# SilverlightningY/dmmt-jpeg-encoder

Measured on AMD Instinct MI355X. Metric: Mpixel/s encoded (4K PPM, q=90), higher is better.
Workload: dtype f32; 1 GPU; 3840x2160 synthetic RGB u8, 4:4:4, IJG quality 90, 1 frame(s) per step per GPU, pixels in HBM -> JPEG files in HBM, inputs rotating over 12 distinct slots (285 MiB: streamed from HBM); width=3840, height=2160, subsampling=P444, quality=90, parallelism=independent frames x1, lanes=4, input_slots=12

## Files before the change

### dmmt-jpeg-encoder_amd/csrc/encoder.cpp

```cpp
#include <hip/hip_runtime.h>
#include <errno.h>
#include <stdio.h>
#include <sys/stat.h>
#include <stdlib.h>
#include <string.h>

#include <algorithm>
#include <mutex>
#include <vector>

#include "../../include/dmmt_jpeg.h"
#include "group.hpp"
#include "jpeg_common.hpp"
#include "kernels.hpp"

using namespace dmmt;

namespace {

const char* kStageNames[ST_COUNT] = {"front", "hist", "tables", "emit", "offsets", "stuffwrite"};

struct DevBuf {
    void* p = nullptr;
    size_t bytes = 0;
};

struct EventPair {
    int stage;
    hipEvent_t a, b;
};

#ifndef DMMT_FUSE_TABLES_DEFAULT
#define DMMT_FUSE_TABLES_DEFAULT 1
#endif

struct GraphEntry {
    std::vector<uint64_t> key;
    hipGraphExec_t exec = nullptr;
    uint64_t last_use = 0;
};
constexpr size_t kMaxGraphs = 16;

}

constexpr int kStatusAsync = 0, kStatusSync = 1, kStatusWords = 8;
struct Lane {
    hipStream_t stream = nullptr;
    int* status = nullptr;
    int* dstatus = nullptr;
    DevBuf coef, dcdiff, lastnz, ac_hist, dc_hist, code_tab, hdr_len, total_out, stage, chunk_bits, chunk_ff,
        chunk_ff8, chunk_edge, chunk_bit0, chunk_out, arrive;
    DevBuf ppm_rgb, ppm_counts, ppm_rowbase;
};

struct dmmt_ctx {
    dmmt::Group* group = nullptr;
    int device = 0;
    hipStream_t stream = nullptr;
    std::mutex mu;
    std::vector<Lane*> lanes;
    int nlanes = 1;
    unsigned next_lane = 0;
    DevBuf lut, qtab, qtab_u8;
    int async_bits = 0;
    hipEvent_t ev_lane0 = nullptr, ev_caller = nullptr;
    DevBuf in, out, out_len, dct;
    DevBuf ppm_text, ppm_maps, ppm_chunk_in, ppm_misc, ppm_counts;
    void* ppm_report = nullptr;
    void* ppm_batch_reports = nullptr;
    size_t ppm_batch_cap = 0;
    int ppm_batch_redone = -1;
    int lut_maxval = -1, lut_sb = -1;
    uint8_t q_cached[128];
    bool q_valid = false;
    bool profile = false;
    uint32_t profile_mask = 0;
    std::vector<EventPair> pending;
    std::vector<hipEvent_t> free_events;
    double stage_ms[ST_COUNT] = {0};
    int stage_launches[ST_COUNT] = {0};
    bool use_graphs = false;
    bool fuse_tables = DMMT_FUSE_TABLES_DEFAULT != 0;
    std::vector<GraphEntry> graphs;
    uint64_t graph_clock = 0;
    bool stripe_pending = false;
    Geom stripe_g{};
    dmmt_options stripe_opt{};
    int stripe_sb = 1;
    int16_t stripe_dc_first[3] = {0, 0, 0}, stripe_dc_last[3] = {0, 0, 0};
    bool stripe_measured = false;
    uint8_t* stripe_out = nullptr;
    size_t stripe_cap = 0;
};

namespace {

int hip_err(hipError_t e) {
    if (e == hipSuccess) return DMMT_OK;
    if (e == hipErrorOutOfMemory) return DMMT_E_OUT_OF_MEMORY;
    return DMMT_E_HIP;
}

#define HIP_TRY(expr)                      \
    do {                                   \
        hipError_t e_ = (expr);            \
        if (e_ != hipSuccess) return hip_err(e_); \
    } while (0)

int check_fresh_alloc(void* p) {
    int cur = -1;
    HIP_TRY(hipGetDevice(&cur));
    hipPointerAttribute_t a;
    HIP_TRY(hipPointerGetAttributes(&a, p));
    return a.device == cur ? DMMT_OK : DMMT_E_DEVICE_MISMATCH;
}

int ensure(DevBuf& b, size_t bytes, bool zero = false) {
    if (bytes == 0) bytes = 16;
    if (b.bytes >= bytes) return DMMT_OK;
    if (b.p) HIP_TRY(hipFree(b.p));
    b.p = nullptr;
    b.bytes = 0;
    HIP_TRY(hipMalloc(&b.p, bytes));
    if (int rc = check_fresh_alloc(b.p)) {
        (void)hipFree(b.p);
        b.p = nullptr;
        return rc;
    }
    b.bytes = bytes;
    if (zero) {
        HIP_TRY(hipMemset(b.p, 0, bytes));
        HIP_TRY(hipDeviceSynchronize());
    }
    return DMMT_OK;
}

void release(DevBuf& b) {
    if (b.p) (void)hipFree(b.p);
    b.p = nullptr;
    b.bytes = 0;
}

int validate(const dmmt_options* opt) {
    if (!opt) return DMMT_E_INVALID_ARGUMENT;
    if (opt->subsampling < 0 || opt->subsampling > 2) return DMMT_E_INVALID_ARGUMENT;
    if (opt->bits_per_channel < 0 || opt->bits_per_channel > 255) return DMMT_E_INVALID_ARGUMENT;
    for (int i = 0; i < 64; ++i)
        if (opt->luma_q[i] == 0 || opt->chroma_q[i] == 0) return DMMT_E_INVALID_ARGUMENT;
    if (opt->restart_interval < 0 || opt->restart_interval > 65535) return DMMT_E_INVALID_ARGUMENT;
    return DMMT_OK;
}

int make_checked_geom(int w, int h, int sub, int maxval, int ri, Geom* g) {
    if (w <= 0 || h <= 0) return DMMT_E_INVALID_ARGUMENT;
    *g = make_geom(w, h, sub, maxval, ri);
    if (g->wp > 65535 || g->hp > 65535) return DMMT_E_INVALID_ARGUMENT;
    return DMMT_OK;
}

int sync_lanes(dmmt_ctx* c) {
    for (Lane* L : c->lanes) HIP_TRY(hipStreamSynchronize(L->stream));
    return DMMT_OK;
}

int upload_tables(dmmt_ctx* c, const dmmt_options* opt, int maxval, int sb, hipStream_t st) {
    int rc;
    if ((rc = ensure(c->qtab, 128 * sizeof(float)))) return rc;
    if ((rc = ensure(c->qtab_u8, 256))) return rc;
    uint8_t q[256];
    memcpy(q, opt->luma_q, 64);
    memcpy(q + 64, opt->chroma_q, 64);
    for (int i = 0; i < 128; ++i) q[128 + i] = q[(i & 64) + kZigzag[i & 63]];
    if (!c->q_valid || memcmp(q, c->q_cached, 128) != 0) {
        if ((rc = sync_lanes(c))) return rc;
        float qf[128];
        for (int i = 0; i < 128; ++i) qf[i] = (float)q[i];
        HIP_TRY(hipMemcpyAsync(c->qtab.p, qf, sizeof qf, hipMemcpyHostToDevice, st));
        HIP_TRY(hipMemcpyAsync(c->qtab_u8.p, q, 256, hipMemcpyHostToDevice, st));
        HIP_TRY(hipStreamSynchronize(st));
        memcpy(c->q_cached, q, 128);
        c->q_valid = true;
    }
    if (sb == 4) {
        if (!c->lut.p && (rc = ensure(c->lut, 256 * sizeof(float)))) return rc;
        return DMMT_OK;
    }
    if (c->lut_maxval != maxval || c->lut_sb != sb) {
        if ((rc = sync_lanes(c))) return rc;
        const size_t n = sb == 1 ? 256 : 65536;
        if ((rc = ensure(c->lut, n * sizeof(float)))) return rc;
        std::vector<float> lut(n);
        for (size_t v = 0; v < n; ++v) lut[v] = (float)v / (float)maxval;
        HIP_TRY(hipMemcpyAsync(c->lut.p, lut.data(), n * sizeof(float), hipMemcpyHostToDevice, st));
        HIP_TRY(hipStreamSynchronize(st));
        c->lut_maxval = maxval;
        c->lut_sb = sb;
    }
    return DMMT_OK;
}

int ensure_work(dmmt_ctx* c, const Geom& g, int nf, Work* w, int lane, bool async) {
    int rc;
    Lane* L = c->lanes[lane];
    const size_t nb = (size_t)g.bpf * nf;
    const size_t nch = (size_t)g.nch * nf;
    if ((rc = ensure(L->coef, nb * 64 * sizeof(int16_t)))) return rc;
    if ((rc = ensure(L->dcdiff, nb * sizeof(int16_t)))) return rc;
    if ((rc = ensure(L->lastnz, nb))) return rc;
    if ((rc = ensure(L->stage, (nch * (size_t)kChunkWordsCap + 64) * sizeof(uint32_t)))) return rc;
    if ((rc = ensure(L->chunk_bits, nch * sizeof(uint32_t)))) return rc;
    if ((rc = ensure(L->chunk_ff, nch * 8 * sizeof(uint32_t)))) return rc;
    if ((rc = ensure(L->chunk_ff8, (nch + 2) * sizeof(unsigned long long)))) return rc;
    if ((rc = ensure(L->chunk_edge, nch * sizeof(uint32_t)))) return rc;
    if ((rc = ensure(L->chunk_bit0, nch * sizeof(unsigned long long)))) return rc;
    if ((rc = ensure(L->chunk_out, nch * sizeof(unsigned long long)))) return rc;
    if ((rc = ensure(L->ac_hist, (size_t)nf * kHistReps * 512 * 4, true))) return rc;
    if ((rc = ensure(L->dc_hist, (size_t)nf * kHistReps * 32 * 4, true))) return rc;
    if ((rc = ensure(L->code_tab, (size_t)nf * 1024 * 4))) return rc;
    if ((rc = ensure(L->arrive, (size_t)nf * kArriveFrameWords * 4, true))) return rc;
    if ((rc = ensure(L->hdr_len, (size_t)nf * 4))) return rc;
    if ((rc = ensure(L->total_out, (size_t)nf * 8))) return rc;
    if (!L->status) {
        void* h = nullptr;
        HIP_TRY(hipHostMalloc(&h, 2 * kStatusWords * sizeof(int), hipHostMallocMapped | hipHostMallocCoherent));
        memset(h, 0, 2 * kStatusWords * sizeof(int));
        L->status = (int*)h;
        if (hipHostGetDevicePointer((void**)&L->dstatus, h, 0) != hipSuccess) {
            (void)hipHostFree(h);
            L->status = nullptr;
            return DMMT_E_HIP;
        }
    }
    w->coef = (int16_t*)L->coef.p;
    w->dcdiff = (int16_t*)L->dcdiff.p;
    w->lastnz = (uint8_t*)L->lastnz.p;
    w->ac_hist = (uint32_t*)L->ac_hist.p;
    w->dc_hist = (uint32_t*)L->dc_hist.p;
    w->code_tab = (uint32_t*)L->code_tab.p;
    w->hdr_len = (uint32_t*)L->hdr_len.p;
    w->stage = (uint32_t*)L->stage.p;
    w->chunk_bits = (uint32_t*)L->chunk_bits.p;
    w->chunk_ff = (uint32_t*)L->chunk_ff.p;
    w->chunk_ff8 = (unsigned long long*)L->chunk_ff8.p;
    w->chunk_edge = (uint32_t*)L->chunk_edge.p;
    w->chunk_bit0 = (unsigned long long*)L->chunk_bit0.p;
    w->chunk_out = (unsigned long long*)L->chunk_out.p;
    w->total_out = (unsigned long long*)L->total_out.p;
    w->arrive = (uint32_t*)L->arrive.p;
    w->status = L->dstatus + (async ? kStatusAsync : kStatusSync) * kStatusWords;
    w->norm_lut = nullptr;
    w->qtab = nullptr;
    w->qtab_u8 = nullptr;
    return DMMT_OK;
}

int prepare(dmmt_ctx* c, const Geom& g, int nf, const dmmt_options* opt, int sb, hipStream_t st, Work* w,
            int lane = 0, bool async = false, int* status = nullptr) {
    int rc;
    if ((rc = ensure_work(c, g, nf, w, lane, async))) return rc;
    if (status) w->status = status;
    if ((rc = upload_tables(c, opt, g.maxval, sb, st))) return rc;
    w->norm_lut = (const float*)c->lut.p;
    w->qtab = (const float*)c->qtab.p;
    w->qtab_u8 = (const uint8_t*)c->qtab_u8.p;
    if (!w->norm_lut || !w->qtab || !w->qtab_u8) return DMMT_E_HIP;
    return DMMT_OK;
}

hipEvent_t take_event(dmmt_ctx* c) {
    if (!c->free_events.empty()) {
        hipEvent_t e = c->free_events.back();
        c->free_events.pop_back();
        return e;
    }
    hipEvent_t e = nullptr;
    if (hipEventCreate(&e) != hipSuccess) return nullptr;
    return e;
}

void drain_events(dmmt_ctx* c) {
    for (auto& p : c->pending) {
        (void)hipEventSynchronize(p.b);
        float ms = 0.f;
        if (hipEventElapsedTime(&ms, p.a, p.b) == hipSuccess) {
            c->stage_ms[p.stage] += ms;
            c->stage_launches[p.stage] += 1;
        }
        c->free_events.push_back(p.a);
        c->free_events.push_back(p.b);
    }
    c->pending.clear();
}

struct StageTimer {
    dmmt_ctx* c;
    int stage;
    hipStream_t st;
    hipEvent_t a = nullptr, b = nullptr;
    StageTimer(dmmt_ctx* c_, int s, hipStream_t st_) : c(c_), stage(s), st(st_) {
        if (c->profile && ((c->profile_mask >> s) & 1u)) {
            a = take_event(c);
            b = take_event(c);
            if (a) (void)hipEventRecord(a, st);
        }
    }
    ~StageTimer() {
        if (a && b) {
            (void)hipEventRecord(b, st);
            c->pending.push_back({stage, a, b});
            if (c->pending.size() > 4096) drain_events(c);
        }
    }
};

int enqueue_back_half(dmmt_ctx* c, const Geom& g, int nf, const Work& w, int bits, uint8_t* out, size_t out_stride,
                      uint32_t* out_len, hipStream_t st, int check_cat, bool hist_done = false) {
    const bool fused_tables = !hist_done && c->fuse_tables && tables_fusable(g);
    if (!hist_done) {
        StageTimer t(c, ST_HIST, st);
        HIP_TRY(launch_hist(nf, g, w, check_cat, st, fused_tables, bits, out, out_stride,
                            c->nlanes > 1 ? DMMT_HIST_WG_CAP_LANES : 0));
    }
    if (!fused_tables) {
        StageTimer t(c, ST_TABLES, st);
        HIP_TRY(launch_tables(nf, g, w, bits, out, out_stride, st));
    }
    {
        StageTimer t(c, ST_EMIT, st);
        HIP_TRY(launch_emit(nf, g, w, true, st, c->nlanes <= 1));
    }
    if (!offsets_fusable(g)) {
        StageTimer t(c, ST_OFFSETS, st);
        HIP_TRY(launch_offsets(nf, g, w, st));
    }
    {
        StageTimer t(c, ST_STUFFWRITE, st);
        HIP_TRY(launch_stuffwrite(nf, g, w, out, out_stride, out_len, st));
    }
    return DMMT_OK;
}

int enqueue_direct(dmmt_ctx* c, const void* d_rgb, size_t frame_stride, int sb, int nf, const Geom& g,
                   const Work& w, int bits, uint8_t* out, size_t out_stride, uint32_t* out_len, hipStream_t st,
                   const Surface* sf = nullptr, const YccFrames* yf = nullptr) {
    {
        StageTimer t(c, ST_FRONT, st);
        const int cap = c->nlanes > 1 ? DMMT_FRONT_PER_CU_LANES : 0;
        if (yf)
            HIP_TRY(launch_front_ycc(*yf, frame_stride, nf, g, w, st, cap));
        else if (sf)
            HIP_TRY(launch_front_surface(*sf, frame_stride, sb, nf, g, w, st, cap));
        else
            HIP_TRY(launch_front(d_rgb, frame_stride, sb, nf, g, w, st, cap));
    }
    return enqueue_back_half(c, g, nf, w, bits, out, out_stride, out_len, st, sb == 4);
}

void destroy_graphs(dmmt_ctx* c) {
    for (auto& e : c->graphs) (void)hipGraphExecDestroy(e.exec);
    c->graphs.clear();
}

int enqueue_encode(dmmt_ctx* c, const void* d_rgb, size_t frame_stride, int sb, int nf, const Geom& g,
                   const dmmt_options* opt, uint8_t* out, size_t out_stride, uint32_t* out_len, hipStream_t st,
                   int lane = 0, bool async = false, int* status = nullptr, const Surface* sf = nullptr,
                   const YccFrames* yf = nullptr) {
    Work w;
    int rc;
    if ((rc = prepare(c, g, nf, opt, sb, st, &w, lane, async, status))) return rc;
    const int bits = opt->bits_per_channel;
    if (!c->use_graphs || c->profile || status)
        return enqueue_direct(c, d_rgb, frame_stride, sb, nf, g, w, bits, out, out_stride, out_len, st, sf, yf);
    std::vector<uint64_t> key = {(uint64_t)(uintptr_t)d_rgb, (uint64_t)frame_stride, (uint64_t)sb, (uint64_t)nf,
                                 (uint64_t)g.width, (uint64_t)g.height, (uint64_t)g.hr, (uint64_t)g.vr,
                                 (uint64_t)g.maxval, (uint64_t)g.restart_interval, (uint64_t)bits,
                                 (uint64_t)(uintptr_t)out, (uint64_t)out_stride, (uint64_t)(uintptr_t)out_len,
                                 (uint64_t)(uintptr_t)st,
                                 sf ? (uint64_t)sf->format + 1 : 0, sf ? (uint64_t)sf->row_pitch : 0,
                                 sf ? (uint64_t)(uintptr_t)sf->plane[0] : 0, sf ? (uint64_t)(uintptr_t)sf->plane[1] : 0,
                                 sf ? (uint64_t)(uintptr_t)sf->plane[2] : 0};
    if (yf)
        key.insert(key.end(), {(uint64_t)yf->format + 16, (uint64_t)yf->luma_pitch, (uint64_t)yf->chroma_pitch,
                               (uint64_t)(uintptr_t)yf->plane[1], (uint64_t)(uintptr_t)yf->plane[2]});
    const void* const* wp = reinterpret_cast<const void* const*>(&w);
    static_assert(sizeof(Work) % sizeof(void*) == 0, "Work holds pointers only");
    for (size_t i = 0; i < sizeof(Work) / sizeof(void*); ++i) key.push_back((uint64_t)(uintptr_t)wp[i]);
    GraphEntry* hit = nullptr;
    for (auto& e : c->graphs)
        if (e.key == key) hit = &e;
    if (!hit) {
        hipGraph_t graph = nullptr;
        HIP_TRY(hipStreamBeginCapture(st, hipStreamCaptureModeThreadLocal));
        rc = enqueue_direct(c, d_rgb, frame_stride, sb, nf, g, w, bits, out, out_stride, out_len, st, sf, yf);
        hipError_t e = hipStreamEndCapture(st, &graph);
        if (rc) {
            if (graph) (void)hipGraphDestroy(graph);
            return rc;
        }
        HIP_TRY(e);
        hipGraphExec_t exec = nullptr;
        e = hipGraphInstantiate(&exec, graph, nullptr, nullptr, 0);
        (void)hipGraphDestroy(graph);
        HIP_TRY(e);
        if (c->graphs.size() >= kMaxGraphs) {
            size_t lru = 0;
            for (size_t i = 1; i < c->graphs.size(); ++i)
                if (c->graphs[i].last_use < c->graphs[lru].last_use) lru = i;
            (void)hipGraphExecDestroy(c->graphs[lru].exec);
            c->graphs.erase(c->graphs.begin() + lru);
        }
        c->graphs.push_back({std::move(key), exec, 0});
        hit = &c->graphs.back();
    }
    hit->last_use = ++c->graph_clock;
    HIP_TRY(hipGraphLaunch(hit->exec, st));
    return DMMT_OK;
}

int status_code(int s) {
    if (s & 1) return DMMT_E_VALUE_EXCEEDS_MAX;
    if (s & 4) return DMMT_E_CATEGORY_RANGE;
    if (s & 2) return DMMT_E_HUFFMAN_SYMBOL_MISSING;
    if (s & 16) return DMMT_E_CAPACITY;
    return DMMT_OK;
}

int read_status(Lane* L, int group, hipStream_t st, int* bits) {
    *bits = 0;
    if (!L->status) return DMMT_OK;
    if (st) HIP_TRY(hipStreamSynchronize(st));
    volatile int* p = L->status + group * kStatusWords;
    for (int k = 0; k < kStatusWords; ++k)
        if (p[k]) {
            *bits |= 1 << k;
            p[k] = 0;
        }
    return DMMT_OK;
}

int take_status(dmmt_ctx* c, hipStream_t st) {
    int s = 0, rc;
    if ((rc = read_status(c->lanes[0], kStatusSync, st, &s))) return rc;
    return status_code(s);
}

int collect_async(dmmt_ctx* c, Lane* L, bool device_synced = false) {
    int s = 0, rc;
    if ((rc = read_status(L, kStatusAsync, device_synced ? nullptr : L->stream, &s))) return rc;
    c->async_bits |= s;
    return DMMT_OK;
}

int set_device(dmmt_ctx* c) { return hip_err(hipSetDevice(c->device)); }

dmmt_ctx* primary(dmmt_ctx* c) { return c && c->group ? group_member(c->group, 0) : c; }

void destroy_lane(Lane* L, bool own_stream) {
    (void)hipStreamSynchronize(L->stream);
    if (L->status) (void)hipHostFree(L->status);
    DevBuf* bufs[] = {&L->coef,      &L->dcdiff,     &L->lastnz,     &L->ac_hist,
                      &L->dc_hist,  &L->code_tab,  &L->hdr_len,    &L->total_out,  &L->stage,
                      &L->chunk_bits, &L->chunk_ff, &L->chunk_ff8, &L->chunk_edge, &L->chunk_bit0, &L->chunk_out,
                      &L->arrive,     &L->ppm_rgb,    &L->ppm_counts, &L->ppm_rowbase};
    for (DevBuf* b : bufs) release(*b);
    if (own_stream) (void)hipStreamDestroy(L->stream);
    delete L;
}

}


extern "C" int dmmt_device_count(int* count) {
    if (!count) return DMMT_E_INVALID_ARGUMENT;
    int n = 0;
    if (hipGetDeviceCount(&n) != hipSuccess) n = 0;
    *count = n;
    return DMMT_OK;
}

extern "C" int dmmt_ctx_create(int device, dmmt_ctx** out) {
    if (!out) return DMMT_E_INVALID_ARGUMENT;
    *out = nullptr;
    int n = 0;
    if (hipGetDeviceCount(&n) != hipSuccess || n <= 0 || device < 0 || device >= n) return DMMT_E_NO_DEVICE;
    hipDeviceProp_t prop;
    if (hipGetDeviceProperties(&prop, device) != hipSuccess) return DMMT_E_NO_DEVICE;
    if (strncmp(prop.gcnArchName, "gfx950", 6) != 0) return DMMT_E_NO_DEVICE;
    if (hipSetDevice(device) != hipSuccess) return DMMT_E_NO_DEVICE;
    dmmt_ctx* c = new dmmt_ctx();
    c->device = device;
    if (const char* e = getenv("DMMT_GRAPHS")) c->use_graphs = atoi(e) != 0;
    if (const char* e = getenv("DMMT_FUSE_TABLES")) c->fuse_tables = atoi(e) != 0;
    if (hipStreamCreateWithFlags(&c->stream, hipStreamNonBlocking) != hipSuccess) {
        delete c;
        return DMMT_E_HIP;
    }
    c->lanes.push_back(new Lane());
    c->lanes[0]->stream = c->stream;
    if (hipEventCreateWithFlags(&c->ev_lane0, hipEventDisableTiming) != hipSuccess ||
        hipEventCreateWithFlags(&c->ev_caller, hipEventDisableTiming) != hipSuccess) {
        dmmt_ctx_destroy(c);
        return DMMT_E_HIP;
    }
    *out = c;
    return DMMT_OK;
}

static int check_ptr_device(const void* p, int dev) {
    if (!p) return DMMT_OK;
    hipPointerAttribute_t a;
    HIP_TRY(hipPointerGetAttributes(&a, p));
    return a.device == dev ? DMMT_OK : DMMT_E_DEVICE_MISMATCH;
}

namespace dmmt {
int ctx_check_device(dmmt_ctx* c) {
    int rc;
    if ((rc = set_device(c))) return rc;
    std::lock_guard<std::mutex> lk(c->mu);
    for (Lane* L : c->lanes) {
        const DevBuf* bufs[] = {&L->coef,       &L->dcdiff,   &L->lastnz,     &L->ac_hist,    &L->dc_hist,
                                &L->code_tab,   &L->hdr_len,  &L->total_out,  &L->stage,      &L->chunk_bits,
                                &L->chunk_ff,   &L->chunk_ff8,  &L->chunk_edge, &L->chunk_bit0, &L->chunk_out, &L->arrive,
                                &L->ppm_rgb,    &L->ppm_counts, &L->ppm_rowbase};
        for (const DevBuf* b : bufs)
            if ((rc = check_ptr_device(b->p, c->device))) return rc;
    }
    const DevBuf* bufs[] = {&c->lut, &c->qtab, &c->qtab_u8, &c->in, &c->out, &c->out_len, &c->dct, &c->ppm_text,
                            &c->ppm_maps, &c->ppm_chunk_in, &c->ppm_misc, &c->ppm_counts};
    for (const DevBuf* b : bufs)
        if ((rc = check_ptr_device(b->p, c->device))) return rc;
    return DMMT_OK;
}
int ptr_check_device(const void* p, int device) { return check_ptr_device(p, device); }
}

extern "C" int dmmt_ctx_check_device(dmmt_ctx* c, int32_t* device) {
    if (!c) return DMMT_E_INVALID_ARGUMENT;
    if (device) *device = c->device;
    if (c->group) return dmmt::group_check_devices(c->group);
    return dmmt::ctx_check_device(c);
}

extern "C" int dmmt_ctx_create_multi(const int* device_ids, int n, dmmt_ctx** out) {
    if (!out) return DMMT_E_INVALID_ARGUMENT;
    *out = nullptr;
    if (!device_ids || n < 1 || n > DMMT_MAX_GROUP) return DMMT_E_INVALID_ARGUMENT;
    dmmt::Group* g = nullptr;
    const int rc = dmmt::group_create(device_ids, n, &g);
    if (rc) return rc;
    dmmt_ctx* c = new dmmt_ctx();
    c->group = g;
    c->device = device_ids[0];
    *out = c;
    return DMMT_OK;
}

extern "C" int dmmt_ctx_num_devices(const dmmt_ctx* c) {
    if (!c) return 0;
    return c->group ? dmmt::group_size(c->group) : 1;
}

extern "C" dmmt_ctx* dmmt_ctx_member(dmmt_ctx* c, int i) {
    if (!c) return nullptr;
    if (c->group) return dmmt::group_member(c->group, i);
    return i == 0 ? c : nullptr;
}

extern "C" void dmmt_ctx_destroy(dmmt_ctx* c) {
    if (!c) return;
    if (c->group) {
        dmmt::group_destroy(c->group);
        delete c;
        return;
    }
    (void)hipSetDevice(c->device);
    (void)sync_lanes(c);
    drain_events(c);
    destroy_graphs(c);
    for (hipEvent_t e : c->free_events) (void)hipEventDestroy(e);
    for (size_t i = 0; i < c->lanes.size(); ++i) destroy_lane(c->lanes[i], i > 0);
    if (c->ev_lane0) (void)hipEventDestroy(c->ev_lane0);
    if (c->ev_caller) (void)hipEventDestroy(c->ev_caller);
    DevBuf* bufs[] = {&c->lut,      &c->qtab,         &c->qtab_u8,  &c->in,       &c->out,     &c->out_len,
                      &c->dct,      &c->ppm_text,     &c->ppm_maps, &c->ppm_chunk_in, &c->ppm_misc,
                      &c->ppm_counts};
    for (DevBuf* b : bufs) release(*b);
    if (c->ppm_report) (void)hipHostFree(c->ppm_report);
    if (c->ppm_batch_reports) (void)hipHostFree(c->ppm_batch_reports);
    (void)hipStreamDestroy(c->stream);
    delete c;
}

extern "C" int dmmt_ctx_set_lanes(dmmt_ctx* c, int n) {
    if (!c || n < 1 || n > DMMT_MAX_LANES) return DMMT_E_INVALID_ARGUMENT;
    if (c->group) return dmmt::group_set_lanes(c->group, n);
    std::lock_guard<std::mutex> lk(c->mu);
    int rc;
    if ((rc = set_device(c))) return rc;
    if ((rc = sync_lanes(c))) return rc;
    while ((int)c->lanes.size() > n) {
        if ((rc = collect_async(c, c->lanes.back()))) return rc;
        destroy_lane(c->lanes.back(), true);
        c->lanes.pop_back();
    }
    while ((int)c->lanes.size() < n) {
        Lane* L = new Lane();
        if (hipStreamCreateWithFlags(&L->stream, hipStreamNonBlocking) != hipSuccess) {
            delete L;
            return DMMT_E_HIP;
        }
        c->lanes.push_back(L);
    }
    destroy_graphs(c);
    c->nlanes = n;
    c->next_lane = 0;
    return DMMT_OK;
}

extern "C" int dmmt_ctx_synchronize(dmmt_ctx* c) {
    if (!c) return DMMT_E_INVALID_ARGUMENT;
    if (c->group) return dmmt::group_synchronize(c->group);
    std::lock_guard<std::mutex> lk(c->mu);
    int rc;
    if ((rc = set_device(c))) return rc;
    HIP_TRY(hipDeviceSynchronize());
    for (Lane* L : c->lanes)
        if ((rc = collect_async(c, L, true))) return rc;
    const int s = c->async_bits;
    c->async_bits = 0;
    return status_code(s);
}

extern "C" size_t dmmt_max_jpeg_bytes(uint16_t width, uint16_t height, int32_t subsampling) {
    if (subsampling < 0 || subsampling > 2 || width == 0 || height == 0) return 0;
    Geom g = make_geom(width, height, subsampling, 255, 0);
    return max_jpeg_bytes(g);
}

static int encode_device_frames(dmmt_ctx* c, const dmmt_device_frames* f, const dmmt_options* opt, void* stream,
                                const Geom& g, const Surface* sf, const YccFrames* yf = nullptr) {
    int rc;
    std::lock_guard<std::mutex> lk(c->mu);
    if ((rc = set_device(c))) return rc;
    if (stream) {
        hipStream_t st = (hipStream_t)stream;
        HIP_TRY(hipEventRecord(c->ev_lane0, c->stream));
        HIP_TRY(hipStreamWaitEvent(st, c->ev_lane0, 0));
        rc = enqueue_encode(c, f->d_rgb, f->frame_stride, f->sample_bytes, f->n_frames, g, opt, f->d_out,
                            f->out_stride, f->d_out_len, st, 0, true, nullptr, sf, yf);
        HIP_TRY(hipEventRecord(c->ev_caller, st));
        HIP_TRY(hipStreamWaitEvent(c->stream, c->ev_caller, 0));
        return rc;
    }
    int lane = 0;
    if (c->nlanes > 1) lane = (int)(c->next_lane++ % (unsigned)c->nlanes);
    return enqueue_encode(c, f->d_rgb, f->frame_stride, f->sample_bytes, f->n_frames, g, opt, f->d_out, f->out_stride,
                          f->d_out_len, c->lanes[lane]->stream, lane, true, nullptr, sf, yf);
}

extern "C" int dmmt_encode_device(dmmt_ctx* c, const dmmt_device_frames* f, const dmmt_options* opt, void* stream) {
    c = primary(c);
    if (!c || !f) return DMMT_E_INVALID_ARGUMENT;
    int rc;
    if ((rc = validate(opt))) return rc;
    if (f->n_frames <= 0 || !f->d_rgb || !f->d_out || !f->d_out_len) return DMMT_E_INVALID_ARGUMENT;
    if (f->sample_bytes != 1 && f->sample_bytes != 2 && f->sample_bytes != 4) return DMMT_E_INVALID_ARGUMENT;
    Geom g;
    if ((rc = make_checked_geom(f->width, f->height, opt->subsampling, f->maxval, opt->restart_interval, &g))) return rc;
    if (f->out_stride < max_jpeg_bytes(g)) return DMMT_E_CAPACITY;
    return encode_device_frames(c, f, opt, stream, g, nullptr);
}

extern "C" size_t dmmt_surface_span(const dmmt_device_surfaces* s) {
// ... 603 lines not shown
    case DMMT_E_INPUT_NOT_FOUND: return "Input file not found";
    case DMMT_E_NO_READ_PERMISSION: return "No read permission for input file";
    case DMMT_E_OPEN_INPUT: return "Unable to open input file for reading";
    case DMMT_E_OPEN_OUTPUT: return "Unable to open output file for writing";
    case DMMT_E_WRITE_IMAGE_DATA: return "Failed to write image data";
    case DMMT_E_WRITE_END_OF_FILE: return "Failed to write end of file";
    case DMMT_E_HUFFMAN_SYMBOL_MISSING: return "Huffman symbol not present in translator";
    case DMMT_E_VALUE_EXCEEDS_MAX: return "Color value must not be greater than max value";
    case DMMT_E_CATEGORY_RANGE: return "Value out of range for categorisation";
    case DMMT_E_INVALID_ARGUMENT: return "Invalid argument";
    case DMMT_E_HIP: return "HIP runtime error";
    case DMMT_E_OUT_OF_MEMORY: return "Out of device memory";
    case DMMT_E_NO_DEVICE: return "No gfx950 (MI355X) device available; this library has no CPU fallback";
    case DMMT_E_CAPACITY: return "Output buffer too small";
    case DMMT_E_DEVICE_MISMATCH: return "A context's device buffer is not on its GPU";
    default: return dmmt_error_name(code);
    }
}

extern "C" int dmmt_ctx_set_profiling(dmmt_ctx* c, int enable) {
    if (!c) return DMMT_E_INVALID_ARGUMENT;
    if (c->group) return dmmt::group_set_profiling(c->group, enable);
    std::lock_guard<std::mutex> lk(c->mu);
    drain_events(c);
    c->profile = enable != 0;
    c->profile_mask = enable == 1 ? 0xFFFFFFFFu : (uint32_t)enable;
    for (int i = 0; i < ST_COUNT; ++i) {
        c->stage_ms[i] = 0;
        c->stage_launches[i] = 0;
    }
    return DMMT_OK;
}

extern "C" int dmmt_ctx_profile(dmmt_ctx* c, double* ms, int32_t* launches, int n_stages) {
    if (!c) return DMMT_E_INVALID_ARGUMENT;
    if (c->group) return dmmt::group_profile(c->group, ms, launches, n_stages);
    std::lock_guard<std::mutex> lk(c->mu);
    (void)hipSetDevice(c->device);
    drain_events(c);
    for (int i = 0; i < n_stages && i < ST_COUNT; ++i) {
        if (ms) ms[i] = c->stage_ms[i];
        if (launches) launches[i] = c->stage_launches[i];
    }
    return DMMT_OK;
}

extern "C" int dmmt_num_stages(void) { return ST_COUNT; }
extern "C" const char* dmmt_stage_name(int s) { return s >= 0 && s < ST_COUNT ? kStageNames[s] : ""; }

extern "C" int dmmt_device_malloc(dmmt_ctx* c, size_t bytes, void** ptr) {
    c = primary(c);
    if (!c || !ptr) return DMMT_E_INVALID_ARGUMENT;
    int rc;
    if ((rc = set_device(c))) return rc;
    HIP_TRY(hipMalloc(ptr, bytes ? bytes : 16));
    if ((rc = check_fresh_alloc(*ptr))) {
        (void)hipFree(*ptr);
        *ptr = nullptr;
        return rc;
    }
    return DMMT_OK;
}

extern "C" int dmmt_device_free(dmmt_ctx* c, void* ptr) {
    c = primary(c);
    if (!c) return DMMT_E_INVALID_ARGUMENT;
    int rc;
    if ((rc = set_device(c))) return rc;
    HIP_TRY(hipFree(ptr));
    return DMMT_OK;
}

extern "C" int dmmt_memcpy_h2d(dmmt_ctx* c, void* dst, const void* src, size_t bytes) {
    c = primary(c);
    if (!c) return DMMT_E_INVALID_ARGUMENT;
    int rc;
    if ((rc = set_device(c))) return rc;
    HIP_TRY(hipMemcpy(dst, src, bytes, hipMemcpyHostToDevice));
    return DMMT_OK;
}

extern "C" int dmmt_memcpy_d2h(dmmt_ctx* c, void* dst, const void* src, size_t bytes) {
    c = primary(c);
    if (!c) return DMMT_E_INVALID_ARGUMENT;
    int rc;
    if ((rc = set_device(c))) return rc;
    HIP_TRY(hipMemcpy(dst, src, bytes, hipMemcpyDeviceToHost));
    return DMMT_OK;
}

extern "C" int dmmt_fill_synthetic(dmmt_ctx* c, void* d_rgb, uint16_t width, uint16_t height, int32_t n_frames,
                                   int32_t first_frame, uint32_t seed) {
    c = primary(c);
    if (!c || !d_rgb || n_frames <= 0) return DMMT_E_INVALID_ARGUMENT;
    int rc;
    if ((rc = set_device(c))) return rc;
    HIP_TRY(launch_synthetic((uint8_t*)d_rgb, width, height, n_frames, first_frame, seed, 0, height, c->stream));
    HIP_TRY(hipStreamSynchronize(c->stream));
    return DMMT_OK;
}

extern "C" int dmmt_fill_synthetic_rows(dmmt_ctx* c, void* d_rgb, uint16_t width, uint16_t height, int32_t row0,
                                        int32_t rows, int32_t frame, uint32_t seed) {
    c = primary(c);
    if (!c || !d_rgb || row0 < 0 || rows <= 0 || row0 + rows > height) return DMMT_E_INVALID_ARGUMENT;
    int rc;
    if ((rc = set_device(c))) return rc;
    HIP_TRY(launch_synthetic((uint8_t*)d_rgb, width, height, 1, frame, seed, row0, rows, c->stream));
    HIP_TRY(hipStreamSynchronize(c->stream));
    return DMMT_OK;
}

static int stripe_geom(const dmmt_stripe* st, const dmmt_options* opt, Geom* g) {
    if (!st || !opt || !st->d_rgb) return DMMT_E_INVALID_ARGUMENT;
    if (st->sample_bytes != 1 && st->sample_bytes != 2 && st->sample_bytes != 4) return DMMT_E_INVALID_ARGUMENT;
    const int ri = opt->restart_interval;
    if (ri < 0) return DMMT_E_INVALID_ARGUMENT;
    Geom full;
    int rc;
    if ((rc = make_checked_geom(st->width, st->height, opt->subsampling, st->maxval, ri, &full))) return rc;
    if (st->mcu_row0 < 0 || st->mcu_rows <= 0 || st->mcu_row0 + st->mcu_rows > full.mcuy) return DMMT_E_INVALID_ARGUMENT;
    const long long m0 = (long long)st->mcu_row0 * full.mcux;
    const bool last = st->mcu_row0 + st->mcu_rows == full.mcuy;
    if (ri > 0 && m0 % ri) return DMMT_E_INVALID_ARGUMENT;
    if (ri > 0 && !last && ((long long)st->mcu_rows * full.mcux) % ri) return DMMT_E_INVALID_ARGUMENT;
    const int rows_px = 8 * full.vr;
    const int y0 = st->mcu_row0 * rows_px;
    const int h = std::min(st->mcu_rows * rows_px, (int)st->height - y0);
    *g = make_geom(st->width, h, opt->subsampling, st->maxval, ri);
    g->sof_height = st->height;
    g->seg_base = ri > 0 ? (int)(m0 / ri) : 0;
    g->stripe_first = st->mcu_row0 == 0;
    g->more_after = !last;
    return DMMT_OK;
}

extern "C" size_t dmmt_stripe_max_bytes(const dmmt_stripe* st, const dmmt_options* opt) {
    Geom g;
    if (validate(opt) || stripe_geom(st, opt, &g)) return 0;
    return max_jpeg_bytes(g);
}

extern "C" int dmmt_stripe_analyze(dmmt_ctx* c, const dmmt_stripe* st, const dmmt_options* opt,
                                   uint64_t hist[DMMT_STRIPE_HIST_WORDS]) {
    c = primary(c);
    if (!c || !hist) return DMMT_E_INVALID_ARGUMENT;
    int rc;
    Geom g;
    if ((rc = validate(opt)) || (rc = stripe_geom(st, opt, &g))) return rc;
    std::lock_guard<std::mutex> lk(c->mu);
    if ((rc = set_device(c))) return rc;
    hipStream_t s = c->stream;
    Work w;
    if ((rc = prepare(c, g, 1, opt, st->sample_bytes, s, &w))) return rc;
    {
        StageTimer t(c, ST_FRONT, s);
        HIP_TRY(launch_front(st->d_rgb, (size_t)st->width * g.height * 3 * st->sample_bytes, st->sample_bytes, 1, g, w,
                             s));
    }
    {
        StageTimer t(c, ST_HIST, s);
        HIP_TRY(launch_hist(1, g, w, st->sample_bytes == 4, s));
    }
    std::vector<uint32_t> ac((size_t)kHistReps * 512), dc((size_t)kHistReps * 32);
    HIP_TRY(hipMemcpyAsync(ac.data(), w.ac_hist, ac.size() * 4, hipMemcpyDeviceToHost, s));
    HIP_TRY(hipMemcpyAsync(dc.data(), w.dc_hist, dc.size() * 4, hipMemcpyDeviceToHost, s));
    HIP_TRY(hipMemsetAsync(w.ac_hist, 0, ac.size() * 4, s));
    HIP_TRY(hipMemsetAsync(w.dc_hist, 0, dc.size() * 4, s));
    HIP_TRY(hipStreamSynchronize(s));
    if ((rc = take_status(c, s))) return rc;
    for (int i = 0; i < DMMT_STRIPE_HIST_WORDS; ++i) hist[i] = 0;
    for (int r = 0; r < kHistReps; ++r) {
        for (int k = 0; k < 16; ++k) {
            hist[k] += dc[(size_t)r * 32 + k];
            hist[272 + k] += dc[(size_t)r * 32 + 16 + k];
        }
        for (int k = 0; k < 256; ++k) {
            hist[16 + k] += ac[(size_t)r * 512 + k];
            hist[288 + k] += ac[(size_t)r * 512 + 256 + k];
        }
    }
    if (g.restart_interval == 0) {
        std::vector<int16_t> head((size_t)g.bpm * 64), tail((size_t)g.bpm * 64);
        const int nl = g.n_luma;
        HIP_TRY(hipMemcpyAsync(head.data(), w.coef, head.size() * 2, hipMemcpyDeviceToHost, s));
        HIP_TRY(hipMemcpyAsync(tail.data(), w.coef + (g.bpf - g.bpm) * 64, tail.size() * 2, hipMemcpyDeviceToHost, s));
        HIP_TRY(hipStreamSynchronize(s));
        c->stripe_dc_first[0] = head[0];
        c->stripe_dc_first[1] = head[(size_t)nl * 64];
        c->stripe_dc_first[2] = head[(size_t)(nl + 1) * 64];
        c->stripe_dc_last[0] = tail[(size_t)(nl - 1) * 64];
        c->stripe_dc_last[1] = tail[(size_t)nl * 64];
        c->stripe_dc_last[2] = tail[(size_t)(nl + 1) * 64];
    }
    c->stripe_g = g;
    c->stripe_opt = *opt;
    c->stripe_sb = st->sample_bytes;
    c->stripe_pending = true;
    c->stripe_measured = false;
    return DMMT_OK;
}

static int upload_hist_sum(const Work& w, const uint64_t* hist_sum, hipStream_t s) {
    std::vector<uint32_t> ac(512), dc(32);
    for (int k = 0; k < 16; ++k) {
        if (hist_sum[k] > 0xFFFFFFFFull || hist_sum[272 + k] > 0xFFFFFFFFull) return DMMT_E_INVALID_ARGUMENT;
        dc[k] = (uint32_t)hist_sum[k];
        dc[16 + k] = (uint32_t)hist_sum[272 + k];
    }
    for (int k = 0; k < 256; ++k) {
        if (hist_sum[16 + k] > 0xFFFFFFFFull || hist_sum[288 + k] > 0xFFFFFFFFull) return DMMT_E_INVALID_ARGUMENT;
        ac[k] = (uint32_t)hist_sum[16 + k];
        ac[256 + k] = (uint32_t)hist_sum[288 + k];
    }
    HIP_TRY(hipMemcpyAsync(w.ac_hist, ac.data(), ac.size() * 4, hipMemcpyHostToDevice, s));
    HIP_TRY(hipMemcpyAsync(w.dc_hist, dc.data(), dc.size() * 4, hipMemcpyHostToDevice, s));
    HIP_TRY(hipStreamSynchronize(s));
    return DMMT_OK;
}

static int dc_category(int v) {
    unsigned a = (unsigned)(v < 0 ? -v : v);
    int n = 0;
    while (a) {
        ++n;
        a >>= 1;
    }
    return n;
}

extern "C" int dmmt_stripe_dc_edges(dmmt_ctx* c, int16_t first_dc[3], int16_t last_dc[3]) {
    c = primary(c);
    if (!c || !first_dc || !last_dc) return DMMT_E_INVALID_ARGUMENT;
    std::lock_guard<std::mutex> lk(c->mu);
    if (!c->stripe_pending || c->stripe_g.restart_interval != 0) return DMMT_E_INVALID_ARGUMENT;
    for (int i = 0; i < 3; ++i) {
        first_dc[i] = c->stripe_dc_first[i];
        last_dc[i] = c->stripe_dc_last[i];
    }
    return DMMT_OK;
}

extern "C" void dmmt_stripe_fix_dc_hist(uint64_t hist[DMMT_STRIPE_HIST_WORDS], const int16_t first_dc[3],
                                        const int16_t prev_last_dc[3]) {
    for (int i = 0; i < 3; ++i) {
        uint64_t* h = hist + (i == 0 ? 0 : 272);
        const int was = dc_category(first_dc[i]);
        const int is = dc_category((int16_t)(first_dc[i] - prev_last_dc[i]));
        if (h[was] > 0) {
            h[was] -= 1;
            h[is] += 1;
        }
    }
}

extern "C" int dmmt_stripe_measure(dmmt_ctx* c, const uint64_t hist_sum[DMMT_STRIPE_HIST_WORDS],
                                   const int16_t prev_last_dc[3], uint8_t* d_out, size_t out_cap, uint64_t* bits,
                                   uint32_t* first16) {
    c = primary(c);
    if (!c || !hist_sum || !prev_last_dc || !d_out || !bits || !first16) return DMMT_E_INVALID_ARGUMENT;
    std::lock_guard<std::mutex> lk(c->mu);
    if (!c->stripe_pending || c->stripe_g.restart_interval != 0) return DMMT_E_INVALID_ARGUMENT;
    int rc;
    if ((rc = set_device(c))) return rc;
    const Geom g = c->stripe_g;
    if (out_cap < max_jpeg_bytes(g)) return DMMT_E_CAPACITY;
    hipStream_t s = c->stream;
    Work w;
    if ((rc = prepare(c, g, 1, &c->stripe_opt, c->stripe_sb, s, &w))) return rc;
    if ((rc = upload_hist_sum(w, hist_sum, s))) return rc;
    int16_t d[3];
    const long long at[3] = {0, g.n_luma, g.n_luma + 1};
    for (int i = 0; i < 3; ++i) {
        d[i] = (int16_t)(c->stripe_dc_first[i] - prev_last_dc[i]);
        HIP_TRY(hipMemcpyAsync(w.dcdiff + at[i], &d[i], sizeof(int16_t), hipMemcpyHostToDevice, s));
    }
    {
        StageTimer t(c, ST_TABLES, s);
        HIP_TRY(launch_tables(1, g, w, c->stripe_opt.bits_per_channel, d_out, out_cap, s));
    }
    {
        StageTimer t(c, ST_EMIT, s);
        HIP_TRY(launch_emit(1, g, w, false, s, c->nlanes <= 1));
    }
    std::vector<uint32_t> nb((size_t)g.nch), edge((size_t)g.nch);
    HIP_TRY(hipMemcpyAsync(nb.data(), w.chunk_bits, nb.size() * 4, hipMemcpyDeviceToHost, s));
    HIP_TRY(hipMemcpyAsync(edge.data(), w.chunk_edge, edge.size() * 4, hipMemcpyDeviceToHost, s));
    HIP_TRY(hipStreamSynchronize(s));
    if ((rc = take_status(c, s))) return rc;
    uint64_t total = 0;
    uint32_t f = 0;
    int have = 0;
    for (int k = 0; k < g.nch; ++k) {
        if (have < 16 && nb[k]) {
            const int t = std::min(16 - have, (int)std::min<uint32_t>(nb[k], 16u));
            f |= ((edge[k] >> 16) >> (16 - t)) << (16 - have - t);
            have += t;
        }
        total += nb[k];
    }
    *bits = total;
    *first16 = f;
    c->stripe_out = d_out;
    c->stripe_cap = out_cap;
    c->stripe_measured = true;
    return DMMT_OK;
}

extern "C" int dmmt_stripe_write(dmmt_ctx* c, uint64_t bit_offset, uint32_t next_bits, uint32_t next16,
                                 uint64_t* out_len) {
    c = primary(c);
    if (!c || !out_len || next_bits > 16) return DMMT_E_INVALID_ARGUMENT;
    std::lock_guard<std::mutex> lk(c->mu);
    if (!c->stripe_pending || !c->stripe_measured) return DMMT_E_INVALID_ARGUMENT;
    int rc;
    if ((rc = set_device(c))) return rc;
    Geom g = c->stripe_g;
    if (g.stripe_first && bit_offset) return DMMT_E_INVALID_ARGUMENT;
    g.bit_phase = (int)(bit_offset & 7);
    g.next_bits = g.more_after ? (int)next_bits : 0;
    g.next16 = g.more_after ? (next16 & 0xFFFFu) & ~(0xFFFFu >> next_bits) : 0u;
    hipStream_t s = c->stream;
    Work w;
    if ((rc = prepare(c, g, 1, &c->stripe_opt, c->stripe_sb, s, &w))) return rc;
    if ((rc = ensure(c->out_len, 4))) return rc;
    {
        StageTimer t(c, ST_OFFSETS, s);
        HIP_TRY(launch_offsets(1, g, w, s));
    }
    {
        StageTimer t(c, ST_STUFFWRITE, s);
        HIP_TRY(launch_stuffwrite(1, g, w, c->stripe_out, c->stripe_cap, (uint32_t*)c->out_len.p, s));
    }
    uint32_t len = 0;
    HIP_TRY(hipMemcpyAsync(&len, c->out_len.p, 4, hipMemcpyDeviceToHost, s));
    HIP_TRY(hipStreamSynchronize(s));
    c->stripe_pending = false;
    c->stripe_measured = false;
    if ((rc = take_status(c, s))) return rc;
    *out_len = len;
    return DMMT_OK;
}

extern "C" int dmmt_stripe_encode(dmmt_ctx* c, const uint64_t hist_sum[DMMT_STRIPE_HIST_WORDS], uint8_t* d_out,
                                  size_t out_cap, uint64_t* out_len) {
    c = primary(c);
    if (!c || !hist_sum || !d_out || !out_len) return DMMT_E_INVALID_ARGUMENT;
    std::lock_guard<std::mutex> lk(c->mu);
    if (!c->stripe_pending) return DMMT_E_INVALID_ARGUMENT;
    if (c->stripe_g.restart_interval == 0) return DMMT_E_INVALID_ARGUMENT;
    int rc;
    if ((rc = set_device(c))) return rc;
    const Geom g = c->stripe_g;
    if (out_cap < max_jpeg_bytes(g)) return DMMT_E_CAPACITY;
    hipStream_t s = c->stream;
    Work w;
    if ((rc = prepare(c, g, 1, &c->stripe_opt, c->stripe_sb, s, &w))) return rc;
    if ((rc = upload_hist_sum(w, hist_sum, s))) return rc;
    if ((rc = ensure(c->out_len, 4))) return rc;
    if ((rc = enqueue_back_half(c, g, 1, w, c->stripe_opt.bits_per_channel, d_out, out_cap, (uint32_t*)c->out_len.p,
                                s, 0, true)))
        return rc;
    uint32_t len = 0;
    HIP_TRY(hipMemcpyAsync(&len, c->out_len.p, 4, hipMemcpyDeviceToHost, s));
    HIP_TRY(hipStreamSynchronize(s));
    c->stripe_pending = false;
    if ((rc = take_status(c, s))) return rc;
    *out_len = len;
    return DMMT_OK;
}

extern "C" const char* dmmt_build_info(void) {
#if DMMT_SDWA_PEEPHOLE
#define DMMT_SDWA_NOTE "SDWA peephole on (measurement build)"
#else
#define DMMT_SDWA_NOTE "-mllvm -amdgpu-sdwa-peephole=false"
#endif
    return "dmmt-jpeg-encoder_amd: HIP kernels for gfx950, -ffp-contract=off, " DMMT_SDWA_NOTE ", ABI " "1";
}
```

### dmmt-jpeg-encoder_amd/csrc/entropy.hip

```cpp
#include <hip/hip_runtime.h>
#include <stdint.h>

#include "device_common.hpp"
#include "jpeg_common.hpp"
#include "kernels.hpp"
#include "slot_copy.hpp"

namespace dmmt {

#ifdef DMMT_PHASE_TRACE
static __device__ unsigned long long g_trace[64];
#endif

static_assert(kChunkBlocks == 256 || kChunkBlocks == 512, "one thread per block, one workgroup per chunk");
constexpr int kEmitThreads = kChunkBlocks;
constexpr int kEmitWaves = kEmitThreads / 64;
#ifndef DMMT_EMIT_OCC
#define DMMT_EMIT_OCC 8
#endif
constexpr int kEmitOcc = kChunkBlocks == 256 ? DMMT_EMIT_OCC : 3;
#ifndef DMMT_EMIT_OCC_BATCH
#define DMMT_EMIT_OCC_BATCH 7
#endif
constexpr int kEmitOccBatch = kChunkBlocks == 256 ? DMMT_EMIT_OCC_BATCH : 3;

constexpr int kEmitWords = 4 * kChunkBlocks;
constexpr int kStuffPass = 4096;
#ifndef DMMT_EMIT_BRANCHFREE
#define DMMT_EMIT_BRANCHFREE 1
#endif
#ifndef DMMT_TAIL_DMA
#define DMMT_TAIL_DMA 1
#endif
#ifndef DMMT_TAIL_NSEG1
#define DMMT_TAIL_NSEG1 1
#endif
#ifndef DMMT_WALK_COLUMN_MAJOR
#define DMMT_WALK_COLUMN_MAJOR 1
#endif
#ifndef DMMT_EMIT_PRIO_ALWAYS
#define DMMT_EMIT_PRIO_ALWAYS 0
#endif
#ifndef DMMT_EMIT_PRIO
#define DMMT_EMIT_PRIO 1
#endif

struct ChunkSpan {
    long long el0;
    int nb;
    int seg;
    bool seg_first, seg_last;
};

__device__ __forceinline__ ChunkSpan chunk_span(const Geom& g, int c) {
    ChunkSpan r;
    r.seg = min(c / g.cps, g.nseg - 1);
    const int j = c - r.seg * g.cps;
    const long long sb = (long long)r.seg * g.seg_blocks;
    const long long se = min(sb + g.seg_blocks, g.bpf);
    r.el0 = sb + (long long)j * kChunkBlocks;
    r.nb = (int)min((long long)kChunkBlocks, se - r.el0);
    r.seg_first = j == 0;
    r.seg_last = r.el0 + r.nb == se;
    return r;
}

__device__ __forceinline__ bool joined_tail(const Geom& g, int c) {
    return c == g.nch - 1 && g.more_after && g.restart_interval == 0;
}

__device__ __forceinline__ int mod_small(int x, int d, uint32_t inv16) {
    return x - (int)__umul24((uint32_t)d, __umul24((uint32_t)x, inv16) >> 16);
}

struct BlockCoef {
    uint32_t w[32];
};

__device__ __forceinline__ void load_block(const int16_t* __restrict__ p, BlockCoef& b) {
    const uint4* q = reinterpret_cast<const uint4*>(p);
#pragma unroll
    for (int i = 0; i < 8; ++i) {
        const uint4 v = q[i];
        b.w[4 * i] = v.x;
        b.w[4 * i + 1] = v.y;
        b.w[4 * i + 2] = v.z;
        b.w[4 * i + 3] = v.w;
    }
}

__device__ __forceinline__ int coef_at(const BlockCoef& b, int k) {
    return (k & 1) ? ((int)b.w[k >> 1] >> 16) : (int)(int16_t)(b.w[k >> 1] & 0xFFFFu);
}

__device__ __forceinline__ void zigzag_in_registers(BlockCoef& b) {
#if DMMT_WALK_COLUMN_MAJOR
    return;
#endif
    uint32_t z[32];
#pragma unroll
    for (int j = 0; j < 32; ++j) {
        const int i0 = coef_pos(2 * j), i1 = coef_pos(2 * j + 1);
        const uint32_t lo = (b.w[i0 >> 1] >> (16 * (i0 & 1))) & 0xFFFFu;
        const uint32_t hi = (b.w[i1 >> 1] >> (16 * (i1 & 1))) & 0xFFFFu;
        z[j] = lo | (hi << 16);
    }
#pragma unroll
    for (int j = 0; j < 32; ++j) b.w[j] = z[j];
}

template <typename Sink>
__device__ __forceinline__ void walk_block(const BlockCoef& b, int dcd, const uint2* __restrict__ dctab,
                                           const uint2* __restrict__ actab, Sink& sink, int kmax = 63) {
    {
        const int cat = category_of(dcd);
        const uint2 e = dctab[cat];
        sink(e.x | extra_bits(dcd, cat), (int)e.y);
    }
    uint32_t m_run = 0xF0u, m_low = 0xFFFFu, m_zrl = 255u;
    asm volatile("" : "+s"(m_run), "+s"(m_low), "+s"(m_zrl));
    int l16 = 16;
#pragma unroll
    for (int k0 = 0; k0 < 64; k0 += 4) {
        if (k0 != 0 && k0 > kmax) break;
#pragma unroll
        for (int k = k0 ? k0 : 1; k < k0 + 4; ++k) {
            const int kc =DMMT_WALK_COLUMN_MAJOR ? coef_pos(k) : k;
            const uint32_t w = b.w[kc >> 1];
            if ((kc & 1) ? w > m_low : (w << 16) != 0u) {
                const int v = coef_at(b, kc);
                const int r16 = 16 * k - l16;
                if (k >= 17 && __builtin_amdgcn_ballot_w64((uint32_t)r16 > m_zrl) != 0) {
                    int r = r16 >> 8;
                    asm volatile("" : "+v"(r));
                    const uint2 z = actab[0xF0];
#pragma unroll 1
                    for (; r > 0; --r) sink(z.x, (int)z.y);
                }
                const int cat = category_fast(v);
                const uint2 e = actab[(r16 & (int)m_run) | cat];
                sink(e.x | extra_bits(v, cat), (int)e.y);
                l16 = 16 * k + 16;
            }
        }
    }
    if (l16 < 16 * 64 || kmax < 63) {
        const uint2 e = actab[0];
        sink(e.x, (int)e.y);
    }
}

struct CountSink {
    uint32_t n = 0;
    __device__ __forceinline__ void operator()(uint32_t, int len) { n += (uint32_t)len; }
};

struct WindowSink {
    uint32_t* img;
    int lo, n;
    unsigned long long acc;
    int nacc;
    int w;
    bool first;
    __device__ __forceinline__ void put(uint32_t word, bool shared) {
        const int i = w - lo;
        if ((unsigned)i < (unsigned)n) {
            if (shared)
                atomicOr(&img[i], word);
            else
                img[i] = word;
        }
    }
    __device__ __forceinline__ void operator()(uint32_t val, int len) {
        acc = (acc << len) | val;
        nacc += len;
        if (nacc >= 32) {
            nacc -= 32;
            put((uint32_t)(acc >> nacc), first);
            first = false;
            ++w;
        }
    }
    __device__ __forceinline__ void finish() {
        if (nacc > 0) put((uint32_t)(acc << (32 - nacc)), true);
    }
};


struct SlotSink {
    uint32_t* slot;
    unsigned long long acc;
    int nacc;
    int wi;
#if DMMT_EMIT_BRANCHFREE
    __device__ __forceinline__ void operator()(uint32_t val, int len) {
        acc = (acc << len) | val;
        nacc += len;
        const int full = nacc >> 5;
        nacc &= 31;
        slot[min(wi, kSlotWords - 1) * kEmitThreads] = (uint32_t)(acc >> nacc);
        wi += full;
    }
#else
    __device__ __forceinline__ void operator()(uint32_t val, int len) {
        acc = (acc << len) | val;
        nacc += len;
        if (nacc >= 32) {
            nacc -= 32;
            slot[min(wi, kSlotWords - 1) * kEmitThreads] = (uint32_t)(acc >> nacc);
            ++wi;
        }
    }
#endif
    __device__ __forceinline__ uint32_t finish() {
        if (nacc > 0 && wi < kSlotWords) slot[wi * kEmitThreads] = (uint32_t)(acc << (32 - nacc));
        return (uint32_t)wi * 32u + (uint32_t)nacc;
    }
};


__device__ __forceinline__ uint32_t bits16_at(uint32_t a, uint32_t b, int p) {
    const unsigned long long x = ((unsigned long long)a << 32) | b;
    return (uint32_t)(x >> (48 - (p & 31))) & 0xFFFFu;
}

struct NoMark {
    template <typename I>
    __device__ void operator()(I) const {}
};
template <typename Mark = NoMark>
__device__ __forceinline__ void fused_offsets(const uint32_t* __restrict__ cbits, const uint32_t* __restrict__ cff,
                              const unsigned long long* __restrict__ cff8, uint8_t* sFF8,
                              const uint32_t* __restrict__ cedge, const Geom& g, unsigned long long* __restrict__ bit0,
                              unsigned long long* __restrict__ outo, unsigned long long* __restrict__ total,
                              unsigned long long* sWaveV, int* sWaveF, int tid, Mark mark = Mark());
static_assert(kArriveWords == kArriveFrameWords, "the host sizes the counters");

__device__ __forceinline__ int tid_again(int wave) {
    uint32_t zero = 0u;
    asm volatile("" : "+s"(zero));
    return (wave << 6) | (int)__builtin_amdgcn_mbcnt_hi(~0u, __builtin_amdgcn_mbcnt_lo(~0u, zero));
}

template <int OCC>
__global__ __launch_bounds__(kEmitThreads, OCC) void k_emit(const int16_t* coef, const int16_t* __restrict__ dcdiff,
                                              const uint8_t* __restrict__ lastnz,
                                              const uint32_t* __restrict__ code_tab, Geom g,
                                              uint32_t* __restrict__ stage, uint32_t* __restrict__ chunk_bits,
                                              uint32_t* __restrict__ chunk_ff, uint32_t* __restrict__ chunk_edge,
                                              uint32_t* __restrict__ ac_hist, uint32_t* __restrict__ dc_hist,
                                              int fuse, uint32_t* __restrict__ arrive,
                                              unsigned long long* __restrict__ chunk_bit0,
                                              unsigned long long* __restrict__ chunk_out,
                                              unsigned long long* __restrict__ total_out,
                                              unsigned long long* __restrict__ chunk_ff8, int prio) {
    __shared__ uint2 sTab[2 * 256 + 2 * 16];
    __shared__ __attribute__((aligned(16))) uint32_t sSlot[kSlotWords * kEmitThreads];
    static_assert(kEmitWords + 2 <= kSlotWords * kEmitThreads, "the window image lies inside the slot area");
    uint32_t* const sW = sSlot;
    __shared__ uint32_t sSort[kEmitThreads + kEmitThreads * (int)sizeof(std::conditional_t<(kEmitThreads > 256), uint16_t, uint8_t>) / 4 + kEmitThreads / 4];
    __shared__ uint32_t sWave[kEmitWaves];
    __shared__ uint32_t sFF[8];
    __shared__ uint32_t sEdge[3];
    __shared__ uint32_t sBin[65];
    __shared__ unsigned long long sOffV[kEmitWaves + 1];
    __shared__ int sOffF[kEmitWaves];
    __shared__ uint32_t sLast;
    using OrderT = std::conditional_t<(kEmitThreads > 256), uint16_t, uint8_t>;
    uint32_t* const sBits = sSort;
    OrderT* const sOrder = reinterpret_cast<OrderT*>(sSort + kEmitThreads);
    uint8_t* const sKey = reinterpret_cast<uint8_t*>(sSort + kEmitThreads + kEmitThreads * (int)sizeof(OrderT) / 4);
    DMMT_TRACE_START;
    int tid = threadIdx.x;
    const int wave = __builtin_amdgcn_readfirstlane(tid >> 6);
    const int frame = blockIdx.y;
    const unsigned chunk = blockIdx.x;
    const ChunkSpan span = chunk_span(g, (int)chunk);
    const long long el0 = span.el0;
    const int nb = span.nb;
    const size_t cid = (size_t)frame * g.nch + chunk;
    const int r0 = (int)((uint32_t)el0 % (uint32_t)g.bpm);
    const uint32_t inv16 = (65536u + (uint32_t)g.bpm - 1u) / (uint32_t)g.bpm;
    bool valid = tid < nb;
    const uint32_t* ct = code_tab + (size_t)frame * 1024;
    const int tt = tid & 255;
    const uint32_t tac0 = ct[256 + tt], tac1 = ct[768 + tt];
    const uint32_t tdc = ct[((tt & 31) < 16 ? 0 : 512 - 16) + (tt & 31)];
    const uint32_t lz = lastnz[(long long)frame * g.bpf + el0 + (valid ? tid : 0)];
    if (tid < 256) {
        const int c = tid & 15;
        sTab[tid] = make_uint2((tac0 & 0xFFFFu) << c, (tac0 >> 16) + c);
        sTab[256 + tid] = make_uint2((tac1 & 0xFFFFu) << c, (tac1 >> 16) + c);
    }
    if (tid < 32) sTab[512 + tid] = make_uint2((tdc & 0xFFFFu) << (tid & 15), (tdc >> 16) + (tid & 15));
    if (chunk == 0) {
        for (int i = tid; i < kHistReps * 512; i += kEmitThreads) ac_hist[(size_t)frame * kHistReps * 512 + i] = 0u;
        for (int i = tid; i < kHistReps * 32; i += kEmitThreads) dc_hist[(size_t)frame * kHistReps * 32 + i] = 0u;
    }
    if (tid < 8) sFF[tid] = 0u;
    if (tid < 3) sEdge[tid] = 0u;
    if (tid < 65) sBin[tid] = 0u;
    const int key = valid ? (int)lz : 64;
    __syncthreads();
    const uint32_t rank = atomicAdd(&sBin[key], 1u);
    __syncthreads();
    if (tid < 64) {
        const uint32_t c = sBin[tid];
        const uint32_t inc = wave_incl_scan_full_u32(c);
        sBin[tid] = inc - c;
    }
    __syncthreads();
    if (valid) {
        const int mine = (int)(sBin[key] + rank);
        sOrder[mine] = (OrderT)tid;
        sKey[mine] = (uint8_t)key;
    }
    __syncthreads();
    DMMT_TRACE(0);
    uint32_t wbits = 0;
    bool slot_over = false;
    {
#if DMMT_EMIT_PRIO
        if (prio) {
            if (wave == 3) __builtin_amdgcn_s_setprio(3);
            else if (wave == 2) __builtin_amdgcn_s_setprio(2);
            else if (wave == 1) __builtin_amdgcn_s_setprio(1);
        }
#endif
        if (valid) {
            const int p = sOrder[tid];
            const long long ep = (long long)frame * g.bpf + el0 + p;
            BlockCoef b;
            load_block(coef + ep * 64, b);
            zigzag_in_registers(b);
            const int dp = dcdiff[ep];
            DMMT_TRACE(4);
            const int kp = mod_small(r0 + p, g.bpm, inv16);
            const bool lum = kp < g.n_luma;
            const int kmax = __builtin_amdgcn_readfirstlane((int)sKey[min(64 * wave + 63, nb - 1)]);
            SlotSink ss{sSlot + tid, 0ull, 0, 0};
            walk_block(b, dp, sTab + 512 + (lum ? 0 : 16), sTab + (lum ? 0 : 256), ss, kmax);
            wbits = ss.finish();
            slot_over = wbits > (uint32_t)kSlotWords * 32u;
            sBits[p] = wbits | ((uint32_t)tid << 16);
            DMMT_TRACE(5);
        }
    }
#if DMMT_EMIT_PRIO
    if (prio) __builtin_amdgcn_s_setprio(0);
#endif
    const bool over = __syncthreads_or(slot_over) != 0;
    tid = tid_again(wave);
    const int lane = tid & 63;
    valid = tid < nb;
    static_assert(kMaxBlockBits < (1 << 16), "a block's bit count and its walker's column share a word");
    const uint32_t bw = valid ? sBits[tid] : (uint32_t)tid << 16;
    const uint32_t bits = bw & 0xFFFFu;
    const int mine = (int)(bw >> 16);
    const uint32_t incl = wave_incl_scan_full_u32(bits);
    if (lane == 63) sWave[wave] = incl;
    __syncthreads();
    uint32_t start = incl - bits;
    uint32_t total = 0;
#pragma unroll
    for (int q = 0; q < kEmitWaves; ++q) {
        start += q < wave ? sWave[q] : 0u;
        total += sWave[q];
    }
    DMMT_TRACE(1);

    uint32_t* slot = stage + cid * (size_t)kChunkWordsCap;
    const int nw = (int)((total + 31) >> 5);
    const int we1 = total >= 16 ? (int)((total - 16) >> 5) : 0;
    uint32_t ff[4] = {0, 0, 0, 0};
    auto window_out = [&](int tid, int w0, int wn) {
        for (int i = tid; i < wn; i += kEmitThreads) {
            const uint32_t a = sW[i], c = sW[i + 1];
            slot[w0 + i] = a;
            const int wi = w0 + i;
            if (wi == 0) sEdge[0] = a;
            if (wi == we1) {
                sEdge[1] = a;
                sEdge[2] = c;
            }
            const unsigned long long x = ((unsigned long long)a << 32) | c;
            unsigned long long z = x & (x << 1);
            z &= z << 2;
            z &= z << 4;
            const uint32_t m = (uint32_t)(z >> 32);
            if (m) {
#pragma unroll
                for (int r = 0; r < 4; ++r)
                    ff[r] += __popc(m & (0x80808080u >> (2 * r))) | (__popc(m & (0x80808080u >> (2 * r + 1))) << 16);
            }
        }
    };
    if (!over) {
        SlotWords sw;
        read_slot<kEmitThreads>(sSlot, mine, bits, sw);
        __syncthreads();
        for (int w0 = 0; w0 < nw; w0 += kEmitWords) {
            const int wn = min(kEmitWords, nw - w0);
            uint32_t st = start;
            asm volatile("" : "+v"(st));
            if (tid == 0 && w0 + wn >= nw) sW[wn] = 0u;
            copy_owned(sw, st, bits, sW, w0, wn);
            __syncthreads();
            copy_head(sw, st, bits, sW, w0, wn);
            __syncthreads();
            window_out(tid, w0, wn);
            __syncthreads();
        }
    } else {
        for (int w0 = 0; w0 < nw; w0 += kEmitWords) {
            const int wn = min(kEmitWords, nw - w0);
            uint32_t st = start;
            asm volatile("" : "+v"(st));
            for (int i = tid; i <= wn; i += kEmitThreads) sW[i] = 0u;
            __syncthreads();
            if (bits && st < (uint32_t)(w0 + wn + 1) * 32u && st + bits > (uint32_t)w0 * 32u) {
                const int te = tid_again(wave);
                const long long e = (long long)frame * g.bpf + el0 + te;
                const bool lum_t = mod_small(r0 + te, g.bpm, inv16) < g.n_luma;
                BlockCoef b;
                load_block(coef + e * 64, b);
                zigzag_in_registers(b);
                WindowSink ws{sW, w0, wn + 1, 0ull, (int)(st & 31), (int)(st >> 5), true};
                walk_block(b, dcdiff[e], sTab + 512 + (lum_t ? 0 : 16), sTab + (lum_t ? 0 : 256), ws);
                ws.finish();
            }
            tid = tid_again(wave);
            __syncthreads();
            window_out(tid, w0, wn);
            __syncthreads();
        }
    }
    DMMT_TRACE(2);
#pragma unroll
    for (int r = 0; r < 4; ++r) {
        const uint32_t v = wave_sum_full_u32(ff[r]);
        if (lane == 0 && v) {
            atomicAdd(&sFF[2 * r], v & 0xFFFFu);
            atomicAdd(&sFF[2 * r + 1], v >> 16);
        }
    }
    __syncthreads();
    if (tid == 0) {
        const uint32_t first16 = sEdge[0] >> 16;
        uint32_t last16;
        if (total >= 16)
            last16 = bits16_at(sEdge[1], sEdge[2], (int)(total - 16));
        else
            last16 = total ? sEdge[0] >> (32 - total) : 0u;
        unsigned long long f8 = 0;
#pragma unroll
        for (int r = 0; r < 8; ++r) {
            __hip_atomic_store(chunk_ff + cid * 8 + r, sFF[r], __ATOMIC_RELAXED, __HIP_MEMORY_SCOPE_AGENT);
            f8 |= (unsigned long long)min(sFF[r], 255u) << (8 * r);
        }
        __hip_atomic_store(chunk_ff8 + cid, f8, __ATOMIC_RELAXED, __HIP_MEMORY_SCOPE_AGENT);
        __hip_atomic_store(chunk_bits + cid, total, __ATOMIC_RELAXED, __HIP_MEMORY_SCOPE_AGENT);
        __hip_atomic_store(chunk_edge + cid, (first16 << 16) | last16, __ATOMIC_RELAXED, __HIP_MEMORY_SCOPE_AGENT);
    }
    if (fuse) {
        if (tid == 0) sLast = arrive_last(arrive + (size_t)frame * kArriveWords, chunk, (unsigned)g.nch);
        __syncthreads();
        DMMT_TRACE(6);
        if (sLast) {
            arrive_acquire();
            const size_t fb = (size_t)frame * g.nch;
#ifdef DMMT_PHASE_TRACE
            auto mark = [&](auto i) { DMMT_TRACE(decltype(i)::value); };
#else
            NoMark mark;
#endif
            fused_offsets(chunk_bits + fb, chunk_ff + fb * 8, chunk_ff8 + fb, reinterpret_cast<uint8_t*>(sSlot),
                          chunk_edge + fb, g, chunk_bit0 + fb, chunk_out + fb, total_out + frame, sOffV, sOffF, tid, mark);
        }
    }
    DMMT_TRACE(3);
    DMMT_TRACE_FLUSH(0, 0);
}

__device__ __forceinline__ uint32_t boundary_byte(int m1, uint32_t last16, bool has_next, uint32_t n_next,
                                                  uint32_t first16_next) {
    uint32_t v = last16 & ((1u << m1) - 1u);
    int m2 = 8 - m1;
    if (has_next) {
        const int t = (int)min((uint32_t)m2, n_next);
        v = (v << t) | (t ? first16_next >> (16 - t) : 0u);
        m2 -= t;
    }
    return ((v << m2) | ((1u << m2) - 1u)) & 0xFFu;
}

__device__ __forceinline__ unsigned long long chunk_out_bytes(const uint32_t* __restrict__ cff,
                                                              const uint32_t* __restrict__ cbits,
                                                              const uint32_t* __restrict__ cedge, const Geom& g,
                                                              int c, unsigned long long b0) {
    const ChunkSpan sp = chunk_span(g, c);
    const uint32_t n = cbits[c];
    const unsigned long long e = b0 + n;
    unsigned long long out = ((e + 7) >> 3) - ((b0 + 7) >> 3);
    out += cff[(size_t)c * 8 + ((8 - (b0 & 7)) & 7)];
    if ((e & 7) && (e & ~7ull) >= b0) {
        const bool jt = joined_tail(g, c);
        const bool has_next = !sp.seg_last || jt;
        const uint32_t nn = jt ? (uint32_t)g.next_bits : (has_next ? cbits[c + 1] : 0u);
        const uint32_t fn = jt ? g.next16 : (has_next ? cedge[c + 1] >> 16 : 0u);
        const uint32_t byte = boundary_byte((int)(e & 7), cedge[c] & 0xFFFFu, has_next, nn, fn);
        out += byte == 0xFFu ? 1u : 0u;
    }
    if (sp.seg_last && (c != g.nch - 1 || (g.more_after && g.restart_interval > 0))) out += 2;
    return out;
}

template <int NW>
__device__ __forceinline__ unsigned long long block_scan_nw(unsigned long long v, unsigned long long* sWave,
                                                            unsigned long long* tot, int tid = threadIdx.x) {
    const int lane = tid & 63, wave = __builtin_amdgcn_readfirstlane(tid >> 6);
    const unsigned long long incl = wave_incl_scan_full_u64(v);
    if (lane == 63) sWave[wave] = incl;
    __syncthreads();
    unsigned long long pre = incl - v, all = 0;
    for (int q = 0; q < NW; ++q) {
        if (q < wave) pre += sWave[q];
        all += sWave[q];
    }
    __syncthreads();
    *tot = all;
    return pre;
}

__device__ __forceinline__ void seg_combine(bool& f, unsigned long long& v, bool f2, unsigned long long v2) {
    v = f2 ? v2 : v + v2;
    f = f || f2;
}

template <int NW>
__device__ __forceinline__ unsigned long long block_segscan_nw(bool f, unsigned long long v,
                                                               unsigned long long* sWaveV, int* sWaveF,
                                                               bool* flag_out = nullptr, int tid = threadIdx.x) {
    const int lane = tid & 63, wave = __builtin_amdgcn_readfirstlane(tid >> 6);
    bool fi = f;
    unsigned long long vi = v;
    auto step = [&](unsigned long long pv, int pf) {
        bool ff = pf != 0;
        seg_combine(ff, pv, fi, vi);
        fi = ff;
        vi = pv;
    };
    step(dpp_u64<0x111, 0xF, 0xF, true>(vi), __builtin_amdgcn_update_dpp(0, (int)fi, 0x111, 0xF, 0xF, true));
    step(dpp_u64<0x112, 0xF, 0xF, true>(vi), __builtin_amdgcn_update_dpp(0, (int)fi, 0x112, 0xF, 0xF, true));
    step(dpp_u64<0x114, 0xF, 0xF, true>(vi), __builtin_amdgcn_update_dpp(0, (int)fi, 0x114, 0xF, 0xF, true));
    step(dpp_u64<0x118, 0xF, 0xF, true>(vi), __builtin_amdgcn_update_dpp(0, (int)fi, 0x118, 0xF, 0xF, true));
    step(dpp_u64<0x142, 0xA, 0xF, false>(vi), __builtin_amdgcn_update_dpp(0, (int)fi, 0x142, 0xA, 0xF, false));
    step(dpp_u64<0x143, 0xC, 0xF, false>(vi), __builtin_amdgcn_update_dpp(0, (int)fi, 0x143, 0xC, 0xF, false));
    if (lane == 63) {
        sWaveV[wave] = vi;
        sWaveF[wave] = fi;
    }
    const unsigned long long ve = dpp_u64<0x138, 0xF, 0xF, true>(vi);
    const int fe = __builtin_amdgcn_update_dpp(0, (int)fi, 0x138, 0xF, 0xF, true);
    __syncthreads();
    bool cf = false;
    unsigned long long cv = 0;
    for (int q = 0; q < wave; ++q) seg_combine(cf, cv, sWaveF[q] != 0, sWaveV[q]);
    bool rf = cf;
    unsigned long long rv = cv;
    seg_combine(rf, rv, fe != 0, ve);
    __syncthreads();
    if (flag_out) *flag_out = rf;
    return rv;
}

__device__ __forceinline__ unsigned long long block_scan_1024(unsigned long long v, unsigned long long* sWave,
                                                              unsigned long long* tot) {
    return block_scan_nw<16>(v, sWave, tot);
}
__device__ __forceinline__ unsigned long long block_segscan_1024(bool f, unsigned long long v,
                                                                 unsigned long long* sWaveV, int* sWaveF) {
    return block_segscan_nw<16>(f, v, sWaveV, sWaveF);
}

static_assert(kFusedRoundChunks % kEmitThreads == 0, "whole chunks per thread of the fused offsets");
static_assert(kFusedRoundChunks % (2 * kEmitThreads) == 0 && kFusedRoundChunks * 8 <= kSlotWords * kEmitThreads * 4,
              "a round's packed 0xFF counts: whole 16-byte pieces per thread, inside k_emit's slot area");
static_assert((unsigned long long)kFusedOffsetsMaxChunks * kChunkBlocks * kMaxBlockBits < (1ull << 32),
              "a fused frame's bit offsets fit 32 bits");
template <typename Mark>
__device__ __forceinline__ void fused_offsets(const uint32_t* __restrict__ cbits, const uint32_t* __restrict__ cff,
                              const unsigned long long* __restrict__ cff8, uint8_t* sFF8,
                              const uint32_t* __restrict__ cedge, const Geom& g, unsigned long long* __restrict__ bit0,
                              unsigned long long* __restrict__ outo, unsigned long long* __restrict__ total,
                              unsigned long long* sWaveV, int* sWaveF, int tid, Mark mark) {
    constexpr int KP = kFusedRoundChunks / kEmitThreads, NT = kEmitThreads;
    const int nch = g.nch;
    uint32_t carry_run = 0, carry_out = 0;
    for (int r0 = 0; r0 < nch; r0 += kFusedRoundChunks) {
        const int rn = min(kFusedRoundChunks, nch - r0);
        const int per = (rn + NT - 1) / NT;
        const int c0 = r0 + min(tid * per, rn), c1 = r0 + min(tid * per + per, rn);
#if DMMT_TAIL_DMA
        {
            const int npairs = (rn + 1) >> 1;
#pragma unroll
            for (int i = 0; i < kFusedRoundChunks / 2 / NT; ++i) {
                const int pc = min(i * NT + tid, npairs - 1);
                __builtin_amdgcn_global_load_lds((const void*)(cff8 + r0 + 2 * pc),
                                                 (void*)(sFF8 + 16 * (i * NT + (tid & ~63))), 16, 0, 16);
            }
        }
#endif
        uint32_t nbits[KP], edge[KP];
#pragma unroll
        for (int i = 0; i < KP; ++i) {
            const int c = min(c0 + i, nch - 1);
            nbits[i] = ld_agent(cbits + c);
            edge[i] = ld_agent(cedge + c);
        }
        const int cl = min(c1, nch - 1);
        const uint32_t nlast = ld_agent(cbits + cl), elast = ld_agent(cedge + cl);
        uint32_t firstm = 0, seglm = 0;
#pragma unroll
        for (int i = 0; i < KP; ++i) nbits[i] = c0 + i < c1 ? nbits[i] : 0u;
        if (DMMT_TAIL_NSEG1 && g.nseg == 1) {
            firstm = c0 == 0 && c0 < c1 ? 1u : 0u;
            seglm = c1 == nch && c0 < c1 ? 1u << (c1 - 1 - c0) : 0u;
        } else {
#pragma unroll
            for (int i = 0; i < KP; ++i) {
                const int c = c0 + i;
                if (c < c1) {
                    const ChunkSpan sp = chunk_span(g, c);
// ... 212 lines not shown
    const size_t cid = (size_t)frame * g.nch + c;
    const bool last = c == g.nch - 1;
    const size_t cidn = last ? cid : cid + 1;
    const uint32_t hdr = hdr_len[frame];
    const unsigned long long tot = total_out[frame];
    const unsigned long long b0 = chunk_bit0[cid];
    const uint32_t n = chunk_bits[cid], edge = chunk_edge[cid];
    const uint32_t n_next = chunk_bits[cidn], edge_next = chunk_edge[cidn];
    const unsigned long long cout = chunk_out[cid], cout_next = chunk_out[cidn];
    const uint32_t* slot = stage + cid * (size_t)kChunkWordsCap;
    uint32_t wv0[5];
    {
        const uint4 q = *reinterpret_cast<const uint4*>(slot + 4 * tid);
        wv0[0] = q.x, wv0[1] = q.y, wv0[2] = q.z, wv0[3] = q.w;
        wv0[4] = slot[4 * tid + 4];
    }
    asm volatile("" ::"s"(hdr), "s"(tot), "s"(b0), "s"(n), "s"(edge), "s"(n_next), "s"(edge_next), "s"(cout),
                 "s"(cout_next), "v"(wv0[0]), "v"(wv0[1]), "v"(wv0[2]), "v"(wv0[3]), "v"(wv0[4]));
    const unsigned long long end = (unsigned long long)hdr + tot;
    if (end + 2 > out_stride) {
        if (c == 0 && tid == 0) {
            out_len[frame] = 0;
            raise_status(status, 16);
        }
        return;
    }
    {
        const unsigned long long cend = last ? tot : cout_next;
        const unsigned long long sbytes = ((unsigned long long)n + 7) / 8 + 1;
        if (n > (uint32_t)kChunkWordsCap * 32u || cout > cend || cend > tot ||
            (unsigned long long)hdr + cout + 2 * sbytes > out_stride) {
            if (tid == 0) {
                out_len[frame] = 0;
                raise_status(status, 16);
            }
            return;
        }
    }
    const ChunkSpan sp = chunk_span(g, c);
    uint8_t* const base = out + (size_t)frame * out_stride + hdr;
    if (tid == 0) {
        if (last && !g.more_after) {
            base[tot] = 0xFF;
            base[tot + 1] = 0xD9;
            out_len[frame] = (uint32_t)(end + 2);
        } else if (sp.seg_last && g.restart_interval > 0) {
            const unsigned long long at = (last ? tot : cout_next) - 2;
            base[at] = 0xFF;
            base[at + 1] = (uint8_t)(0xD0 + ((g.seg_base + sp.seg) & 7));
            if (last) out_len[frame] = (uint32_t)end;
        } else if (last) {
            out_len[frame] = (uint32_t)end;
        }
    }
    const unsigned long long e = b0 + n;
    const unsigned long long kbeg = (b0 + 7) >> 3, kend = (e + 7) >> 3;
    if (kend <= kbeg) return;
    const unsigned long long nbytes = kend - kbeg;
    const bool shared_tail = (e & 7) != 0;
    uint32_t tail = 0;
    if (shared_tail) {
        const bool jt = joined_tail(g, c);
        const bool has_next = !sp.seg_last || jt;
        tail = boundary_byte((int)(e & 7), edge & 0xFFFFu, has_next,
                             jt ? (uint32_t)g.next_bits : (has_next ? n_next : 0u),
                             jt ? g.next16 : (has_next ? edge_next >> 16 : 0u));
    }
    const unsigned off = (unsigned)(8 * kbeg - b0);
    uint8_t* o = base + cout;
    for (unsigned long long pos = 0; pos < nbytes; pos += kStuffPass) {
        const uint32_t delta = (uint32_t)(reinterpret_cast<uintptr_t>(o) & 15u);
        const unsigned long long kb = pos + 16u * (unsigned)tid;
        const int nvalid = kb < nbytes ? (int)min(16ull, nbytes - kb) : 0;
        uint32_t x[4] = {0u, 0u, 0u, 0u};
        uint32_t ffm[4] = {0u, 0u, 0u, 0u};
        uint32_t cnt = 0;
        if (nvalid) {
            const unsigned long long p = off + 8 * kb;
            const size_t wi = (size_t)(p >> 5);
            const int sh = (int)(p & 31);
            uint32_t wv[5];
#pragma unroll
            for (int i = 0; i < 5; ++i) wv[i] = pos ? slot[wi + i] : wv0[i];
#pragma unroll
            for (int i = 0; i < 4; ++i) x[i] = sh ? (wv[i] << sh) | (wv[i + 1] >> (32 - sh)) : wv[i];
            if (shared_tail && nbytes - 1 - kb < 16) {
                const int j = (int)(nbytes - 1 - kb), sft = 24 - 8 * (j & 3);
                x[j >> 2] = (x[j >> 2] & ~(0xFFu << sft)) | (tail << sft);
            }
#pragma unroll
            for (int i = 0; i < 4; ++i) {
                const int nv = min(max(nvalid - 4 * i, 0), 4);
                const uint32_t vmask = nv ? 0x80808080u & (0xFFFFFFFFu << (32 - 8 * nv)) : 0u;
                const uint32_t t = ~x[i];
                const uint32_t nonzero = (((t & 0x7F7F7F7Fu) + 0x7F7F7F7Fu) | t) & 0x80808080u;
                ffm[i] = ~nonzero & vmask;
                cnt += (uint32_t)__popc(ffm[i]);
            }
        }
        const uint32_t incl = wave_incl_scan_full_u32(cnt);
        if (lane == 63) sWave[wave] = incl;
        __syncthreads();
        uint32_t pre = incl - cnt;
        for (int q = 0; q < wave; ++q) pre += sWave[q];
        const uint32_t ffs = sWave[0] + sWave[1] + sWave[2] + sWave[3];
        if (nvalid) {
            const uint32_t dst = delta + (uint32_t)tid * 16u + pre;
            uint32_t a = dst;
#pragma unroll
            for (int i = 0; i < 4; ++i) {
                const uint32_t w = x[i], f = ffm[i];
                sOut[a + 4 * i] = (uint8_t)(w >> 24);
                sOut[a + (uint32_t)__popc(f & 0x80000000u) + 4 * i + 1] = (uint8_t)(w >> 16);
                sOut[a + (uint32_t)__popc(f & 0x80800000u) + 4 * i + 2] = (uint8_t)(w >> 8);
                sOut[a + (uint32_t)__popc(f & 0x80808000u) + 4 * i + 3] = (uint8_t)w;
                a += (uint32_t)__popc(f);
            }
            if (cnt) {
                uint32_t m = 0;
#pragma unroll
                for (int i = 0; i < 4; ++i)
                    m |= ((((ffm[i] >> 7) * 0x08040201u) >> 24) & 0xFu) << (4 * i);
                uint32_t z = dst + 1;
                while (m) {
                    sOut[z + (uint32_t)__builtin_ctz(m)] = 0x00;
                    ++z;
                    m &= m - 1u;
                }
            }
        }
        __syncthreads();
        const unsigned long long in_pass = nbytes - pos < (unsigned long long)kStuffPass ? nbytes - pos : kStuffPass;
        const uint32_t len = (uint32_t)in_pass + ffs;
        const uint32_t send = delta + len;
        uint8_t* const oa = o - delta;
        for (uint32_t sb = 16u * (uint32_t)tid; sb + 16u <= send; sb += 16u * 256u) {
            if (sb >= delta) *reinterpret_cast<uint4*>(oa + sb) = *reinterpret_cast<const uint4*>(sOut + sb);
        }
        if (tid < 32) {
            const uint32_t sbt = send & ~15u;
            const uint32_t i = tid < 16 ? (uint32_t)tid : sbt + (uint32_t)tid - 16u;
            const bool mine = tid < 16 ? i >= delta && (delta > 0u || send < 16u) : sbt > 0u;
            if (mine && i < send) oa[i] = sOut[i];
        }
        o += len;
        __syncthreads();
    }
}

bool offsets_fusable(const Geom& g) { return g.nch <= kFusedOffsetsMaxChunks; }

hipError_t launch_emit(int n_frames, const Geom& g, const Work& w, bool fuse_offsets, hipStream_t st, bool prio) {
    const int fuse = fuse_offsets && offsets_fusable(g) ? 1 : 0;
    const auto kern = !prio && n_frames > 1 ? k_emit<kEmitOccBatch> : k_emit<kEmitOcc>;
    hipLaunchKernelGGL(kern, dim3(g.nch, n_frames), dim3(kEmitThreads), 0, st, (const int16_t*)w.coef,
                       (const int16_t*)w.dcdiff, (const uint8_t*)w.lastnz, (const uint32_t*)w.code_tab, g, w.stage, w.chunk_bits, w.chunk_ff,
                       w.chunk_edge, w.ac_hist, w.dc_hist, fuse, w.arrive, w.chunk_bit0, w.chunk_out, w.total_out,
                       w.chunk_ff8, prio || DMMT_EMIT_PRIO_ALWAYS ? 1 : 0);
    return hipGetLastError();
}

hipError_t launch_offsets(int n_frames, const Geom& g, const Work& w, hipStream_t st) {
    hipLaunchKernelGGL(k_offsets, dim3(n_frames), dim3(1024), 0, st, (const uint32_t*)w.chunk_bits,
                       (const uint32_t*)w.chunk_ff, (const uint32_t*)w.chunk_edge, g, w.chunk_bit0, w.chunk_out,
                       w.total_out);
    return hipGetLastError();
}

hipError_t launch_stuffwrite(int n_frames, const Geom& g, const Work& w, uint8_t* out, size_t out_stride,
                             uint32_t* out_len, hipStream_t st) {
    hipLaunchKernelGGL(k_stuffwrite, dim3(g.nch, n_frames), dim3(256), 0, st, (const uint32_t*)w.stage,
                       (const uint32_t*)w.chunk_bits, (const uint32_t*)w.chunk_edge,
                       (const unsigned long long*)w.chunk_bit0, (const unsigned long long*)w.chunk_out,
                       (const unsigned long long*)w.total_out, (const uint32_t*)w.hdr_len, g, out, out_stride,
                       out_len, w.status);
    return hipGetLastError();
}

}

#ifdef DMMT_PHASE_TRACE
extern "C" int dmmt_debug_trace_entropy(unsigned long long* out64) {
    if (hipMemcpyFromSymbol(out64, HIP_SYMBOL(dmmt::g_trace), 64 * 8) != hipSuccess) return -1;
    unsigned long long z[64] = {0};
    return hipMemcpyToSymbol(HIP_SYMBOL(dmmt::g_trace), z, sizeof z) == hipSuccess ? 0 : -1;
}
#endif
```

### dmmt-jpeg-encoder_amd/csrc/front_ycc.hip

```cpp

#include <hip/hip_runtime.h>
#include <stdint.h>

#include "dct_quant.hpp"
#include "device_common.hpp"
#include "front_launch.hpp"
#include "jpeg_common.hpp"
#include "kernels.hpp"
#include "ycc_load.hpp"

namespace dmmt {

struct YccArgs {
    const uint8_t *p0, *p1, *p2;
    YccDesc d;
};
struct YccMem {
    const uint8_t* base;
    __device__ __forceinline__ void load16(long long off, uint32_t (&w)[4]) const {
        const uint4 v = ld16_nt(base + off);
        w[0] = v.x, w[1] = v.y, w[2] = v.z, w[3] = v.w;
    }
    __device__ __forceinline__ uint32_t load1(long long off) const { return base[off]; }
    __device__ __forceinline__ uint32_t base_lo() const { return (uint32_t)(uintptr_t)base; }
};
struct YccMems {
    const uint8_t *p0, *p1, *p2;
    __device__ __forceinline__ YccMem plane(int p) const { return YccMem{p == 0 ? p0 : (p == 1 ? p1 : p2)}; }
};

template <int N>
__device__ __forceinline__ void lds_words(const uint8_t* s, int off, uint32_t (&o)[N]) {
    const uint32_t* a = reinterpret_cast<const uint32_t*>(s + (off & ~3));
    uint32_t t[N + 1];
#pragma unroll
    for (int i = 0; i <= N; ++i) t[i] = a[i];
#pragma unroll
    for (int i = 0; i < N; ++i) o[i] = __builtin_amdgcn_alignbyte(t[i + 1], t[i], (uint32_t)off & 3u);
}

template <int HR, int VR, int FMT, int WPE>
__global__ __launch_bounds__(256, WPE) void k_front_ycc(YccArgs ya, size_t frame_stride, Geom g,
                                                       const float* __restrict__ qtab,
                                                       int16_t* __restrict__ coef) {
    constexpr bool NV = FMT != YCC_PLANAR;
    constexpr int VU = FMT == YCC_NV_VU ? 1 : 0;
    using T = YccTile<HR, VR, NV>;
    constexpr int TM = 32 / HR;
    constexpr int ROWS = 8 * VR;
    constexpr int NLUMA = HR * VR;
    constexpr int BPM = NLUMA + 2;
    constexpr int NB = TM * BPM;
    constexpr int NYB = 32 * VR;
    constexpr int CB = TM;
    constexpr int BS = 72;
    auto blk_base = [](int b) { return b * BS + 4 * (((b >> 2) ^ (b >= NYB + CB ? 1 : 0)) & 1); };
    constexpr int SP = HR;
    static_assert(8 * CB * SP == 256, "one phase-A job per thread");
    constexpr int NCJ = NB * 8;
    constexpr int JPT = (NCJ + 255) / 256;

    __shared__ __attribute__((aligned(16))) float sT[NB * BS + 4];
    __shared__ __attribute__((aligned(16))) uint8_t sRaw[T::BYTES + 16];
    __shared__ float sQ[128];
    __shared__ float sRQ[128];

    const int tid = threadIdx.x;
    const int frame = blockIdx.y;
    const size_t foff = (size_t)frame * frame_stride;
    const YccMems ms{ya.p0 + foff, ya.p1 + foff, ya.p2 + foff};
    const YccDesc& d = ya.d;
    if (tid < 128) sQ[tid] = qtab[tid];
    if (tid < 128) sRQ[tid] = c_arai_scale[(tid >> 3) & 7] * (1.0f / qtab[tid]);
    const int col = tid & 7;

    const int tiles_per_row = (g.mcux + TM - 1) / TM;
    const int ntiles = tiles_per_row * g.mcuy;

    uint4 raw[T::NQ];
    auto load_tile = [&](int tx0, int ty0) {
        const bool interior = ycc_tile_interior<T>(d, tx0, ty0);
#pragma unroll
        for (int i = 0; i < T::NQ; ++i) {
            const int q = tid + 256 * i;
            uint32_t w[4] = {0u, 0u, 0u, 0u};
            if (q < T::NCHUNK) ycc_tile_chunk<T>(ms, d, tx0, ty0, interior, q, w);
            raw[i] = make_uint4(w[0], w[1], w[2], w[3]);
        }
    };
    if ((int)blockIdx.x < ntiles) {
        const int my = blockIdx.x / tiles_per_row;
        load_tile((blockIdx.x - my * tiles_per_row) * 256, my * ROWS);
    }
    for (int tile = blockIdx.x; tile < ntiles; tile += gridDim.x) {
        const int my = tile / tiles_per_row;
        const int mx0 = (tile - my * tiles_per_row) * TM;
        const int x0 = mx0 * 8 * HR;
        const int y0 = my * ROWS;

#pragma unroll
        for (int i = 0; i < T::NQ; ++i) {
            const int q = tid + 256 * i;
            if (q < T::NCHUNK) reinterpret_cast<uint4*>(sRaw)[q] = raw[i];
        }
        __syncthreads();
        {
            const int nt = tile + gridDim.x;
            if (nt < ntiles) {
                const int ny = nt / tiles_per_row;
                load_tile((nt - ny * tiles_per_row) * 256, ny * ROWS);
            }
        }

        {
            const int h = tid % SP, job = tid / SP;
            const int c = job % CB, r = job / CB;
            const int lx0 = c * 8 * HR + 8 * h;
#pragma unroll
            for (int dy = 0; dy < VR; ++dy) {
                const int ly = r * VR + dy;
                const int mis = surf_misalign32((uint32_t)(uintptr_t)ms.p0, (uint32_t)d.luma_pitch, 1, x0, y0 + ly);
                uint32_t w[2];
                lds_words<2>(sRaw, T::luma_row(ly) + mis + lx0, w);
                float v[8];
#pragma unroll
                for (int k = 0; k < 8; ++k) v[k] = (float)((w[k >> 2] >> (8 * (k & 3))) & 0xFFu) - 128.0f;
                arai8(v);
                float4* o = reinterpret_cast<float4*>(sT + blk_base((ly >> 3) * 32 + c * HR + h) + (ly & 7) * 8);
                o[0] = make_float4(v[0], v[1], v[2], v[3]);
                o[1] = make_float4(v[4], v[5], v[6], v[7]);
            }
            const int cx0 = x0 / HR, cy = y0 / VR + r;
#pragma unroll
            for (int pass = 0; pass < (SP == 1 ? 2 : 1); ++pass) {
                const int comp = SP == 1 ? pass : h;
                float v[8];
                if constexpr (NV) {
                    const int mis = surf_misalign32((uint32_t)(uintptr_t)ms.p1, (uint32_t)d.chroma_pitch, 2, cx0, cy);
                    uint32_t w[4];
                    lds_words<4>(sRaw, T::chroma_row(0, r) + mis + 16 * c, w);
                    const int sh = 8 * (comp ^ VU);
#pragma unroll
                    for (int k = 0; k < 8; ++k) v[k] = (float)(((w[k >> 1] >> sh) >> (16 * (k & 1))) & 0xFFu) - 128.0f;
                } else {
                    const uint8_t* pb = comp ? ms.p2 : ms.p1;
                    const int mis = surf_misalign32((uint32_t)(uintptr_t)pb, (uint32_t)d.chroma_pitch, 1, cx0, cy);
                    uint32_t w[2];
                    lds_words<2>(sRaw, T::chroma_row(comp, r) + mis + 8 * c, w);
#pragma unroll
                    for (int k = 0; k < 8; ++k) v[k] = (float)((w[k >> 2] >> (8 * (k & 3))) & 0xFFu) - 128.0f;
                }
                arai8(v);
                float4* o = reinterpret_cast<float4*>(sT + blk_base(NYB + comp * CB + c) + r * 8);
                o[0] = make_float4(v[0], v[1], v[2], v[3]);
                o[1] = make_float4(v[4], v[5], v[6], v[7]);
            }
        }
        __syncthreads();

        const int nvalid = min(TM, g.mcux - mx0) * BPM;
        const long long e0 = (long long)frame * g.bpf + ((long long)my * g.mcux + mx0) * BPM;
        int16_t* const cbase = coef + e0 * 64;
        static_assert(NCJ % 256 == 0, "JPT column jobs for every thread");
#pragma unroll
        for (int jj = 0; jj < JPT; ++jj) {
            const int blk = (tid + 256 * jj) >> 3;
            int x[8];
            {
                const float* q = sQ + (blk < NYB ? 0 : 64) + col;
                const float* rq = sRQ + (blk < NYB ? 0 : 64) + col;
                float v[8];
                const float* tb = sT + blk_base(blk) + col;
#pragma unroll
                for (int i = 0; i < 8; ++i) v[i] = tb[i * 8];
                arai8_unscaled(v);
                quantize_col8_scaled(v, q, rq, false, x);
            }
            int el;
            if (blk < NYB) {
                const int by = blk / 32, bx = blk % 32;
                el = (bx / HR) * BPM + by * HR + (bx % HR);
            } else if (blk < NYB + CB) {
                el = (blk - NYB) * BPM + NLUMA;
            } else {
                el = (blk - NYB - CB) * BPM + NLUMA + 1;
            }
            const bool valid = el < nvalid;
            if (valid) {
                uint32_t pk[4];
#pragma unroll
                for (int i = 0; i < 4; ++i) pk[i] = __builtin_amdgcn_perm((uint32_t)x[2 * i + 1], (uint32_t)x[2 * i], 0x05040100u);
                *reinterpret_cast<uint4*>(cbase + (el * 64 + 8 * col)) = make_uint4(pk[0], pk[1], pk[2], pk[3]);
            }
        }
    }
}


constexpr int front_ycc_wpe() { return 4; }

template <int HR, int VR, int FMT>
static void front_ycc_impl(const YccArgs& ya, size_t frame_stride, int n_frames, const Geom& g, const Work& w,
                           hipStream_t st, int per_cu_cap) {
    constexpr int TM = 32 / HR;
    const long long ntiles = (long long)((g.mcux + TM - 1) / TM) * g.mcuy;
    static const FrontCfg cfg = [] { return front_cfg(k_front_ycc<HR, VR, FMT, front_ycc_wpe()>); }();
    hipLaunchKernelGGL((k_front_ycc<HR, VR, FMT, front_ycc_wpe()>), front_grid(cfg, ntiles, n_frames, per_cu_cap),
                       dim3(256), 0, st, ya, frame_stride, g, w.qtab, w.coef);
}
template <int FMT>
static void front_ycc_sub(const YccArgs& ya, size_t frame_stride, int n_frames, const Geom& g, const Work& w,
                          hipStream_t st, int per_cu_cap) {
    if (g.hr == 1)
        front_ycc_impl<1, 1, FMT>(ya, frame_stride, n_frames, g, w, st, per_cu_cap);
    else if (g.vr == 1)
        front_ycc_impl<2, 1, FMT>(ya, frame_stride, n_frames, g, w, st, per_cu_cap);
    else
        front_ycc_impl<2, 2, FMT>(ya, frame_stride, n_frames, g, w, st, per_cu_cap);
}

static int ycc_chroma_width(int width, int hr) { return (width + hr - 1) / hr; }

size_t ycc_plane_span(int format, int plane, int width, int height, int hr, int vr, size_t luma_pitch,
                      size_t chroma_pitch) {
    if (format < YCC_PLANAR || format > YCC_NV_VU || width <= 0 || height <= 0) return 0;
    if (plane == 0) return (size_t)(height - 1) * luma_pitch + (size_t)width;
    if (plane != 1 && !(plane == 2 && format == YCC_PLANAR)) return 0;
    const size_t cw = (size_t)ycc_chroma_width(width, hr), ch = (size_t)((height + vr - 1) / vr);
    return (ch - 1) * chroma_pitch + cw * (format == YCC_PLANAR ? 1 : 2);
}

hipError_t launch_front_ycc(const YccFrames& yf, size_t frame_stride_bytes, int n_frames, const Geom& g, const Work& w,
                            hipStream_t st, int per_cu_cap) {
    if (yf.format < YCC_PLANAR || yf.format > YCC_NV_VU) return hipErrorInvalidValue;
    YccArgs ya{};
    ya.p0 = (const uint8_t*)yf.plane[0];
    ya.p1 = (const uint8_t*)yf.plane[1];
    ya.p2 = (const uint8_t*)yf.plane[yf.format == YCC_PLANAR ? 2 : 1];
    ya.d.luma_pitch = (long long)yf.luma_pitch;
    ya.d.chroma_pitch = (long long)yf.chroma_pitch;
    ya.d.luma_span = (long long)ycc_plane_span(yf.format, 0, g.width, g.height, g.hr, g.vr, yf.luma_pitch, yf.chroma_pitch);
    ya.d.chroma_span = (long long)ycc_plane_span(yf.format, 1, g.width, g.height, g.hr, g.vr, yf.luma_pitch, yf.chroma_pitch);
    ya.d.width = g.width, ya.d.height = g.height;
    ya.d.cw = ycc_chroma_width(g.width, g.hr), ya.d.ch = (g.height + g.vr - 1) / g.vr;
    if (yf.format == YCC_PLANAR)
        front_ycc_sub<YCC_PLANAR>(ya, frame_stride_bytes, n_frames, g, w, st, per_cu_cap);
    else if (yf.format == YCC_NV)
        front_ycc_sub<YCC_NV>(ya, frame_stride_bytes, n_frames, g, w, st, per_cu_cap);
    else
        front_ycc_sub<YCC_NV_VU>(ya, frame_stride_bytes, n_frames, g, w, st, per_cu_cap);
    return hipGetLastError();
}

}
```

### dmmt-jpeg-encoder_amd/csrc/kernels.hip

```cpp

#include <hip/hip_runtime.h>
#include <stdint.h>
#include <stdlib.h>

#include <type_traits>

#include "dct_quant.hpp"
#include "device_common.hpp"
#include "front_launch.hpp"
#include "jpeg_common.hpp"
#include "kernels.hpp"
#include "surface_load.hpp"
#include "wave_merge.hpp"

namespace dmmt {

#ifdef DMMT_PHASE_TRACE
static __device__ unsigned long long g_trace[64];
#endif

__constant__ uint8_t c_zigzag[64] = {0,  1,  8,  16, 9,  2,  3,  10, 17, 24, 32, 25, 18, 11, 4,  5,
                                     12, 19, 26, 33, 40, 48, 41, 34, 27, 20, 13, 6,  7,  14, 21, 28,
                                     35, 42, 49, 56, 57, 50, 43, 36, 29, 22, 15, 23, 30, 37, 44, 51,
                                     58, 59, 52, 45, 38, 31, 39, 46, 53, 60, 61, 54, 47, 55, 62, 63};
// ... 24 lines not shown
    static constexpr int NCHUNK = ROWS * RC;
    static constexpr int NQ = (NCHUNK + 255) / 256;
    static constexpr int BYTES = NCHUNK * 16;

    __device__ static __forceinline__ long long row_start(const Geom& g, int x0, int py) {
        return ((long long)py * g.width + x0) * 3 * (long long)sizeof(Sample);
    }
    __device__ static __forceinline__ int misalign(const uint8_t* fbase, long long start) {
        return (int)(((uintptr_t)fbase + (uintptr_t)start) & 15u);
    }

    __device__ static __forceinline__ int misalign32(const uint8_t* fbase, const Geom& g, int x0, int py) {
        return (int)(((uint32_t)(uintptr_t)fbase + (uint32_t)(py * g.width + x0) * (uint32_t)(3 * sizeof(Sample))) & 15u);
    }

    __device__ static __forceinline__ void load(const uint8_t* __restrict__ fbase, long long fbytes, const Geom& g,
                                                int x0, int y0, int tid, uint4 (&v)[NQ]) {
        const long long last = row_start(g, x0, y0 + ROWS - 1);
        if (x0 + 256 <= g.width && y0 + ROWS <= g.height && row_start(g, x0, y0) >= 16 && last + RB + 16 <= fbytes) {
            const uint8_t* tb = fbase + row_start(g, x0, y0);
            const uint32_t rowpitch = (uint32_t)g.width * (uint32_t)(3 * sizeof(Sample));
#pragma unroll
            for (int i = 0; i < NQ; ++i) {
                const int q = tid + 256 * i;
                const int row = q / RC, j = q - (q / RC) * RC;
                const uint8_t* r = tb + (size_t)((uint32_t)row * rowpitch);
                const uint8_t* a = r - ((uint32_t)(uintptr_t)r & 15u) + 16u * (uint32_t)j;
                v[i] = q < NCHUNK ? ld16_nt(a) : make_uint4(0u, 0u, 0u, 0u);
            }
            return;
        }
        const long long rowbytes = (long long)min(256, g.width - x0) * 3 * (long long)sizeof(Sample);
#pragma unroll
        for (int i = 0; i < NQ; ++i) {
            v[i] = make_uint4(0u, 0u, 0u, 0u);
            const int q = tid + 256 * i;
            const int row = q / RC, j = q - (q / RC) * RC;
            const int py = y0 + row;
            if (q >= NCHUNK || py >= g.height) continue;
            const long long start = row_start(g, x0, py);
            const long long c = start - misalign(fbase, start) + 16LL * j;
            if (c >= start + rowbytes) continue;
            if (c >= 0 && c + 16 <= fbytes) {
                v[i] = ld16_nt(fbase + c);
            } else {
                uint32_t w[4] = {0u, 0u, 0u, 0u};
                for (int k = 0; k < 16; ++k)
                    if (c + k >= 0 && c + k < fbytes) w[k >> 2] |= (uint32_t)fbase[c + k] << (8 * (k & 3));
                v[i] = make_uint4(w[0], w[1], w[2], w[3]);
            }
            const long long keep = start + rowbytes - c;
            if (keep < 16) {
                uint32_t w[4] = {v[i].x, v[i].y, v[i].z, v[i].w};
#pragma unroll
                for (int k = 0; k < 4; ++k) {
                    const long long n = keep - 4 * k;
                    w[k] &= n >= 4 ? 0xFFFFFFFFu : (n <= 0 ? 0u : (1u << (8 * n)) - 1u);
                }
                v[i] = make_uint4(w[0], w[1], w[2], w[3]);
            }
        }
    }

    __device__ static __forceinline__ void stage(uint8_t* sRaw, int tid, const uint4 (&v)[NQ]) {
#pragma unroll
        for (int i = 0; i < NQ; ++i) {
            const int q = tid + 256 * i;
            if (q < NCHUNK) reinterpret_cast<uint4*>(sRaw)[q] = v[i];
        }
    }
};

enum { LAY_TIGHT = 0, LAY_RGB = 1, LAY_RGBX = 2, LAY_PLANAR = 3 };
template <int LAY>
struct SurfLayout {
    static constexpr int NPL = LAY == LAY_PLANAR ? 3 : 1;
    static constexpr int SPP = LAY == LAY_RGBX ? 4 : (LAY == LAY_PLANAR ? 1 : 3);
};
struct SurfMem {
    const uint8_t* base;
    __device__ __forceinline__ void load16(long long off, uint32_t (&w)[4]) const {
        const uint4 v = ld16_nt(base + off);
        w[0] = v.x, w[1] = v.y, w[2] = v.z, w[3] = v.w;
    }
    __device__ __forceinline__ uint32_t load1(long long off) const { return base[off]; }
};
template <typename Sample, int ROWS, int LAY>
struct SurfTile {
    static constexpr int NPL = SurfLayout<LAY>::NPL;
    static constexpr int BPP = SurfLayout<LAY>::SPP * (int)sizeof(Sample);
    static constexpr int RB = 256 * BPP;
    static constexpr int RC = RB / 16 + 1;
    static constexpr int RS = RC * 16;
    static constexpr int NCHUNK = ROWS * NPL * RC;
    static constexpr int NQ = (NCHUNK + 255) / 256;
    static constexpr int BYTES = NCHUNK * 16;

    struct Planes {
        const uint8_t *p0, *p1, *p2;
    };
    __device__ static __forceinline__ Planes planes(const SurfArgs& sa, size_t foff) {
        return Planes{sa.plane[0] + foff, sa.plane[NPL == 1 ? 0 : 1] + foff, sa.plane[NPL == 1 ? 0 : 2] + foff};
    }
    __device__ static __forceinline__ const uint8_t* plane(const Planes& pl, int p) {
        return NPL == 1 || p == 0 ? pl.p0 : (p == 1 ? pl.p1 : pl.p2);
    }
    __device__ static __forceinline__ int misalign32(const uint8_t* pbase, const SurfArgs& sa, int x0, int py) {
        return surf_misalign32((uint32_t)(uintptr_t)pbase, (uint32_t)sa.pitch, BPP, x0, py);
    }

    __device__ static __forceinline__ void load(const SurfArgs& sa, size_t foff, const Geom& g, int x0, int y0, int tid,
                                                uint4 (&v)[NQ]) {
        const Planes pl = planes(sa, foff);
        const long long first = surf_row_start(sa.pitch, BPP, x0, y0);
        if (x0 + 256 <= g.width && y0 + ROWS <= g.height &&
            surf_interior(first, surf_row_start(sa.pitch, BPP, x0, y0 + ROWS - 1), RB, sa.span)) {
#pragma unroll
            for (int i = 0; i < NQ; ++i) {
                const int q = tid + 256 * i;
                const int tr = q / RC, j = q - (q / RC) * RC;
                const int row = tr / NPL, p = tr - (tr / NPL) * NPL;
                const uint8_t* pb = plane(pl, p);
                const long long c = surf_interior_chunk((uint32_t)(uintptr_t)pb, first + (long long)row * sa.pitch, j);
                v[i] = q < NCHUNK ? ld16_nt(pb + c) : make_uint4(0u, 0u, 0u, 0u);
            }
            return;
        }
        const long long rowbytes = surf_row_bytes(g.width, BPP, x0);
#pragma unroll
        for (int i = 0; i < NQ; ++i) {
            v[i] = make_uint4(0u, 0u, 0u, 0u);
            const int q = tid + 256 * i;
            const int tr = q / RC, j = q - (q / RC) * RC;
            const int row = tr / NPL, p = tr - (tr / NPL) * NPL;
            const int py = y0 + row;
            if (q >= NCHUNK || py >= g.height) continue;
            const SurfMem m{plane(pl, p)};
            uint32_t w[4];
            surf_load_chunk(m, surf_row_start(sa.pitch, BPP, x0, py), misalign32(m.base, sa, x0, py), rowbytes, sa.span,
                            j, w);
            v[i] = make_uint4(w[0], w[1], w[2], w[3]);
        }
    }

    __device__ static __forceinline__ void stage(uint8_t* sRaw, int tid, const uint4 (&v)[NQ]) {
#pragma unroll
        for (int i = 0; i < NQ; ++i) {
            const int q = tid + 256 * i;
            if (q < NCHUNK) reinterpret_cast<uint4*>(sRaw)[q] = v[i];
        }
    }
};

template <int HR, int VR, typename Sample, int LAY>
__device__ __forceinline__ void front_body(const Sample* __restrict__ rgb, size_t frame_stride, const SurfArgs& sa,
                                           Geom g, const float* __restrict__ norm_lut,
                                           const float* __restrict__ qtab,
                                           int16_t* __restrict__ coef, int* __restrict__ status) {
    constexpr int TM = 32 / HR;
    constexpr int ROWS = 8 * VR;
    constexpr int NLUMA = HR * VR;
    constexpr int BPM = NLUMA + 2;
    constexpr int NB = TM * BPM;
    constexpr int NYB = 32 * VR;
    constexpr int CB = TM;
    constexpr int BS = 72;
    auto blk_base = [](int b) { return b * BS + 4 * (((b >> 2) ^ (b >= NYB + CB ? 1 : 0)) & 1); };
    constexpr int SP = HR;
    constexpr int NJ = 8 * CB * SP;
    constexpr int NCS = 8 / SP;
    constexpr int SB = (int)sizeof(Sample);
    constexpr int NPL = SurfLayout<LAY>::NPL;
    constexpr int SPP = SurfLayout<LAY>::SPP;
    constexpr int PXB = 8 * SPP * SB;
    constexpr int PXW = PXB / 4;
    constexpr int NCJ = NB * 8;
    constexpr int JPT = (NCJ + 255) / 256;
    using Raw = std::conditional_t<LAY == LAY_TIGHT, RawTile<Sample, ROWS>, SurfTile<Sample, ROWS, LAY>>;

    __shared__ __attribute__((aligned(16))) float sT[NB * BS + 4];
    __shared__ __attribute__((aligned(16))) uint8_t sRaw[Raw::BYTES];
    __shared__ float sLut[256];
    __shared__ float sQ[128];
    __shared__ float sRQ[128];

    DMMT_TRACE_START;
    const int tid = threadIdx.x;
    const int frame = blockIdx.y;
    const uint8_t* fbase = nullptr;
    long long fbytes = 0;
    size_t foff = 0;
    if constexpr (LAY == LAY_TIGHT) {
        fbase = reinterpret_cast<const uint8_t*>(rgb + (size_t)frame * frame_stride);
        fbytes = (long long)g.width * g.height * 3 * SB;
    } else {
        foff = (size_t)frame * frame_stride;
    }
    if (tid < 128) sQ[tid] = qtab[tid];
    if (tid < 128) sRQ[tid] = SB == 4 ? 1.0f / qtab[tid] : c_arai_scale[(tid >> 3) & 7] * (1.0f / qtab[tid]);
    if (SB == 1) sLut[tid] = norm_lut[tid];
    const int col = tid & 7;

    const int tiles_per_row = (g.mcux + TM - 1) / TM;
    const int ntiles = tiles_per_row * g.mcuy;
    int bad = 0;
    const bool check_range = SB != 4 && g.maxval < (SB == 1 ? 255 : 65535);

    uint4 raw[Raw::NQ];
    auto load_tile = [&](int tx0, int ty0) {
        if constexpr (LAY == LAY_TIGHT)
            Raw::load(fbase, fbytes, g, tx0, ty0, tid, raw);
        else
            Raw::load(sa, foff, g, tx0, ty0, tid, raw);
    };
    if ((int)blockIdx.x < ntiles) {
        const int my = blockIdx.x / tiles_per_row;
        load_tile((blockIdx.x - my * tiles_per_row) * TM * 8 * HR, my * ROWS);
    }
    for (int tile = blockIdx.x; tile < ntiles; tile += gridDim.x) {
        const int my = tile / tiles_per_row;
        const int mx0 = (tile - my * tiles_per_row) * TM;
        const int x0 = mx0 * 8 * HR;
        const int y0 = my * ROWS;

        Raw::stage(sRaw, tid, raw);
        __syncthreads();
        {
            const int nt = tile + gridDim.x;
            if (nt < ntiles) {
                const int ny = nt / tiles_per_row;
                load_tile((nt - ny * tiles_per_row) * TM * 8 * HR, ny * ROWS);
            }
        }

        auto phase_a = [&](auto range_check) {
            constexpr bool CHECK = decltype(range_check)::value;
            const int h = tid % SP, job = tid / SP;
            const int c = job % CB, r = job / CB;
            const int lx0 = c * 8 * HR + 8 * h;
            uint32_t pw[VR * NPL][SB == 4 ? 1 : PXW];
            const float* fsrc[VR * NPL];
#pragma unroll
            for (int dy = 0; dy < VR; ++dy) {
#pragma unroll
                for (int p = 0; p < NPL; ++p) {
                    const int ly = r * VR + dy;
                    int mis;
                    if constexpr (LAY == LAY_TIGHT)
                        mis = Raw::misalign32(fbase, g, x0, y0 + ly);
                    else
                        mis = Raw::misalign32(sa.plane[p] + foff, sa, x0, y0 + ly);
                    const uint8_t* src = sRaw + (ly * NPL + p) * Raw::RS + mis + lx0 * SPP * SB;
                    fsrc[dy * NPL + p] = reinterpret_cast<const float*>(src);
                    if constexpr (SB == 4) {
                        pw[dy * NPL + p][0] = 0u;
                    } else if ((mis & 7) == 0) {
#pragma unroll
                        for (int k = 0; k < PXW / 2; ++k) {
                            const uint2 u = reinterpret_cast<const uint2*>(src)[k];
                            pw[dy * NPL + p][2 * k] = u.x;
                            pw[dy * NPL + p][2 * k + 1] = u.y;
                        }
                    } else {
#pragma unroll
                        for (int k = 0; k < PXW; ++k)
                            pw[dy * NPL + p][k] = (uint32_t)src[4 * k] | ((uint32_t)src[4 * k + 1] << 8) |
                                                  ((uint32_t)src[4 * k + 2] << 16) | ((uint32_t)src[4 * k + 3] << 24);
                    }
                }
            }
            float yv[VR][8];
            float cbv[8], crv[8];
            uint32_t smax = 0;
#pragma unroll
            for (int k = 0; k < NCS; ++k) {
                float cbs = 0.0f, crs = 0.0f;
#pragma unroll
                for (int dx = 0; dx < HR; ++dx) {
#pragma unroll
                    for (int dy = 0; dy < VR; ++dy) {
                        const int jx = k * HR + dx;
                        float rr, gg, bb;
                        if constexpr (SB == 4) {
                            if constexpr (LAY == LAY_PLANAR) {
                                rr = fsrc[dy * NPL][jx];
                                gg = fsrc[dy * NPL + 1][jx];
                                bb = fsrc[dy * NPL + 2][jx];
                            } else {
                                rr = fsrc[dy][jx * SPP];
                                gg = fsrc[dy][jx * SPP + 1];
                                bb = fsrc[dy][jx * SPP + 2];
                                if constexpr (LAY != LAY_TIGHT) {
                                    const float s0 = rr;
                                    rr = sa.bgr ? bb : rr;
                                    bb = sa.bgr ? s0 : bb;
                                }
                            }
                        } else {
                            uint32_t sv[3];
#pragma unroll
                            for (int ch = 0; ch < 3; ++ch) {
                                const int si = LAY == LAY_PLANAR ? jx : jx * SPP + ch;
                                const uint32_t* rw = pw[LAY == LAY_PLANAR ? dy * NPL + ch : dy];
                                sv[ch] = SB == 1 ? (rw[si >> 2] >> (8 * (si & 3))) & 0xFFu
                                                 : (rw[si >> 1] >> (16 * (si & 1))) & 0xFFFFu;
                            }
                            if constexpr (LAY == LAY_RGB || LAY == LAY_RGBX) {
                                const uint32_t s0 = sv[0];
                                sv[0] = sa.bgr ? sv[2] : sv[0];
                                sv[2] = sa.bgr ? s0 : sv[2];
                            }
                            if constexpr (CHECK) smax = max(smax, max(sv[0], max(sv[1], sv[2])));
                            if (SB == 1) {
                                rr = sLut[sv[0]];
                                gg = sLut[sv[1]];
                                bb = sLut[sv[2]];
                            } else {
                                rr = norm_lut[sv[0]];
                                gg = norm_lut[sv[1]];
                                bb = norm_lut[sv[2]];
                            }
                        }
                        float y, cb, cr;
                        rgb_to_ycbcr<SB != 4>(rr, gg, bb, y, cb, cr);
                        yv[dy][jx] = y;
                        if (dx == 0 && dy == 0) {
                            cbs = cb;
                            crs = cr;
                        } else {
                            cbs = cbs + cb;
                            crs = crs + cr;
                        }
                    }
                }
                if (HR * VR > 1) {
                    cbs = cbs / (float)(HR * VR);
                    crs = crs / (float)(HR * VR);
                }
                cbv[k] = cbs;
                crv[k] = crs;
            }
            if constexpr (CHECK) bad |= (int)(smax > (uint32_t)g.maxval);
#pragma unroll
            for (int dy = 0; dy < VR; ++dy) {
                const int ly = r * VR + dy;
                arai8(yv[dy]);
                float4* o = reinterpret_cast<float4*>(sT + blk_base((ly >> 3) * 32 + c * HR + h) + (ly & 7) * 8);
                o[0] = make_float4(yv[dy][0], yv[dy][1], yv[dy][2], yv[dy][3]);
                o[1] = make_float4(yv[dy][4], yv[dy][5], yv[dy][6], yv[dy][7]);
            }
            if constexpr (SP == 1) {
                arai8(cbv);
                arai8(crv);
                float4* ob = reinterpret_cast<float4*>(sT + blk_base(NYB + c) + r * 8);
                ob[0] = make_float4(cbv[0], cbv[1], cbv[2], cbv[3]);
                ob[1] = make_float4(cbv[4], cbv[5], cbv[6], cbv[7]);
                float4* orr = reinterpret_cast<float4*>(sT + blk_base(NYB + CB + c) + r * 8);
                orr[0] = make_float4(crv[0], crv[1], crv[2], crv[3]);
                orr[1] = make_float4(crv[4], crv[5], crv[6], crv[7]);
            } else {
                float fr[8];
#pragma unroll
                for (int k = 0; k < 4; ++k) {
                    const float send = h ? cbv[k] : crv[k];
                    const float recv = __int_as_float(
                        __builtin_amdgcn_update_dpp(0, __float_as_int(send), 0xB1, 0xF, 0xF, false));
                    fr[k] = h ? recv : cbv[k];
                    fr[4 + k] = h ? crv[k] : recv;
                }
                arai8(fr);
                float4* oc = reinterpret_cast<float4*>(sT + blk_base(NYB + (h ? CB : 0) + c) + r * 8);
                oc[0] = make_float4(fr[0], fr[1], fr[2], fr[3]);
                oc[1] = make_float4(fr[4], fr[5], fr[6], fr[7]);
            }
        };
        if (tid < NJ) {
            if (check_range)
                phase_a(std::integral_constant<bool, true>{});
            else
                phase_a(std::integral_constant<bool, false>{});
        }
        __syncthreads();
        DMMT_TRACE(0);

        const int nvalid = min(TM, g.mcux - mx0) * BPM;
        const long long e0 = (long long)frame * g.bpf + ((long long)my * g.mcux + mx0) * BPM;
        int16_t* const cbase = coef + e0 * 64;
        static_assert(NCJ % 256 == 0, "JPT column jobs for every thread");
#pragma unroll
        for (int jj = 0; jj < JPT; ++jj) {
            const int blk = (tid + 256 * jj) >> 3;
            int x[8];
            {
                const float* q = sQ + (blk < NYB ? 0 : 64) + col;
                const float* rq = sRQ + (blk < NYB ? 0 : 64) + col;
                float v[8];
                const float* tb = sT + blk_base(blk) + col;
#pragma unroll
                for (int i = 0; i < 8; ++i) v[i] = tb[i * 8];
                if constexpr (SB == 4) {
                    arai8(v);
                    quantize_col8(v, q, rq, x);
                } else {
                    arai8_unscaled(v);
                    quantize_col8_scaled(v, q, rq, g.maxval == 0, x);
                }
            }
            int el;
            if (blk < NYB) {
                const int by = blk / 32, bx = blk % 32;
                el = (bx / HR) * BPM + by * HR + (bx % HR);
            } else if (blk < NYB + CB) {
                el = (blk - NYB) * BPM + NLUMA;
            } else {
                el = (blk - NYB - CB) * BPM + NLUMA + 1;
            }
            const bool valid = el < nvalid;
            if (valid) {
                uint32_t pk[4];
#pragma unroll
                for (int i = 0; i < 4; ++i) pk[i] = __builtin_amdgcn_perm((uint32_t)x[2 * i + 1], (uint32_t)x[2 * i], 0x05040100u);
                *reinterpret_cast<uint4*>(cbase + (el * 64 + 8 * col)) = make_uint4(pk[0], pk[1], pk[2], pk[3]);
            }
        }
        DMMT_TRACE(2);
    }

    if (bad) raise_status(status, bad);
    DMMT_TRACE(5);
    DMMT_TRACE_FLUSH(0, 0);
}

template <int HR, int VR, typename Sample, int WPE>
__global__ __launch_bounds__(256, WPE) void k_front(const Sample* __restrict__ rgb, size_t frame_stride, Geom g,
                                               const float* __restrict__ norm_lut,
                                               const float* __restrict__ qtab,
                                               int16_t* __restrict__ coef, int* __restrict__ status) {
    front_body<HR, VR, Sample, LAY_TIGHT>(rgb, frame_stride, SurfArgs{}, g, norm_lut, qtab, coef, status);
}

template <int HR, int VR, typename Sample, int LAY, int WPE>
__global__ __launch_bounds__(256, WPE) void k_front_surf(SurfArgs sa, size_t frame_stride, Geom g,
                                                    const float* __restrict__ norm_lut,
                                                    const float* __restrict__ qtab, int16_t* __restrict__ coef,
                                                    int* __restrict__ status) {
    front_body<HR, VR, Sample, LAY>(nullptr, frame_stride, sa, g, norm_lut, qtab, coef, status);
}

struct HistCoef {
    uint32_t w[32];
};

constexpr int kTailSmallWords = 4 + 4 * 16;
__device__ __forceinline__ void tables_tail(uint8_t* lds, const uint32_t* ac_hist, const uint32_t* dc_hist, int frame,
                                            const Geom& g, uint32_t* __restrict__ code_tab, uint8_t* __restrict__ out,
                                            size_t out_stride, uint32_t* __restrict__ hdr_len,
                                            const uint8_t* __restrict__ qtab_u8, int bits_per_channel,
                                            int* __restrict__ status, int* sCnt, int* sBits);
constexpr int kHistCopies = 4, kHistCopyWords = 545;
constexpr int kTailLdsBytes = 7072;

#ifndef DMMT_HIST_NEWEST_FIRST
#define DMMT_HIST_NEWEST_FIRST 0
#endif
template <bool CHECK, bool FUSE>
__global__ __launch_bounds__(256) __attribute__((amdgpu_waves_per_eu(8, 8))) void k_hist(const int16_t* __restrict__ coef, int16_t* __restrict__ dcdiff,
                                              uint8_t* __restrict__ lastnz, Geom g,
                                              uint32_t* __restrict__ ac_hist ,
                                              uint32_t* __restrict__ dc_hist ,
                                              int* __restrict__ status, uint32_t* __restrict__ arrive,
                                              uint32_t* __restrict__ code_tab, uint8_t* __restrict__ out,
                                              size_t out_stride, uint32_t* __restrict__ hdr_len,
                                              const uint8_t* __restrict__ qtab_u8, int bits_per_channel) {
    constexpr int NC = kHistCopies, HS = kHistCopyWords;
    constexpr int kWords = FUSE && kTailLdsBytes / 4 > NC * HS ? kTailLdsBytes / 4 : NC * HS;
    __shared__ __attribute__((aligned(16))) uint32_t sH[kWords];
    __shared__ int sSmall[FUSE ? kTailSmallWords : 1];
    __shared__ uint32_t sLastWg;
    const int tid = threadIdx.x;
    const int frame = blockIdx.y;
    for (int i = tid; i < NC * HS; i += 256) sH[i] = 0;
    __syncthreads();
    uint32_t* const H = sH + HS * (tid & 3);
    const long long base = (long long)frame * g.bpf;
    const int lane = lane_id();
    int bad = 0;
    const uint32_t bpf = (uint32_t)g.bpf, bpm = (uint32_t)g.bpm, ri = (uint32_t)max(g.restart_interval, 1);
    const uint32_t stride = gridDim.x * 256u, sm = stride / bpm, sk = stride - sm * bpm;
    uint32_t el = blockIdx.x * 256u + (uint32_t)tid;
#if DMMT_HIST_NEWEST_FIRST
    const uint32_t passes = (bpf + stride - 1u) / stride;
    el += (passes - 1u) * stride;
    const uint32_t el1 = el < bpf ? el : el - stride;
    uint32_t m = el1 / bpm, k = el1 - m * bpm, mr = m % ri;
#else
    uint32_t m = el / bpm, k = el - m * bpm, mr = m % ri;
#endif
    const uint32_t smr = sm % ri;
#if DMMT_HIST_NEWEST_FIRST
    for (uint32_t left = passes; left > 0; --left, el -= stride) {
        if (el >= bpf) continue;
#else
    for (; el < bpf; el += stride) {
#endif
        const long long e = base + el;
        const uint4* q = reinterpret_cast<const uint4*>(coef + e * 64);
        uint32_t cw[32];
#pragma unroll
        for (int i = 0; i < 8; ++i) {
            const uint4 v = q[i];
            cw[4 * i] = v.x, cw[4 * i + 1] = v.y, cw[4 * i + 2] = v.z, cw[4 * i + 3] = v.w;
        }
        const int t = k < (uint32_t)g.n_luma ? 0 : 1;
        const bool restart = g.restart_interval > 0 && mr == 0;
        int back = 0;
        if (k > 0 && k < (uint32_t)g.n_luma)
            back = 1;
        else if (m > 0 && !restart)
            back = (k == 0) ? (int)bpm - g.n_luma + 1 : (int)bpm;
        const int cur = (int)(int16_t)(cw[0] & 0xFFFFu);
        const int nb = __shfl_up(cur, (unsigned)back, 64);
        int pv = 0;
        if (back) pv = lane >= back ? nb : (int)coef[(e - back) * 64];
        HistCoef b;
#pragma unroll
        for (int j = 0; j < 32; ++j) {
            const int i0 = coef_pos(2 * j), i1 = coef_pos(2 * j + 1);
            const uint32_t lo = (cw[i0 >> 1] >> (16 * (i0 & 1))) & 0xFFFFu;
            const uint32_t hi = (cw[i1 >> 1] >> (16 * (i1 & 1))) & 0xFFFFu;
            b.w[j] = lo | (hi << 16);
        }
        uint32_t* h = H + 256 * t;
        int l16 = 16;
        uint32_t zrl = 0;
#pragma unroll
        for (int kk = 1; kk < 64; ++kk) {
            const int v = (kk & 1) ? ((int)b.w[kk >> 1] >> 16) : (int)(int16_t)(b.w[kk >> 1] & 0xFFFFu);
            if (v != 0) {
                if (CHECK && v == -32768) bad |= 4;
                const int r16 = 16 * kk - l16;
                zrl += (uint32_t)(r16 >> 8);
                atomicAdd(&h[(r16 & 0xF0) | category_fast(v)], 1u);
                l16 = 16 * kk + 16;
            }
        }
        if (zrl) atomicAdd(&h[0xF0], zrl);
        if (l16 < 16 * 64) atomicAdd(&h[0], 1u);
        lastnz[e] = (uint8_t)((l16 >> 4) - 1);
        {
            const int16_t d = (int16_t)(cur - pv);
            bad |= d == -32768 ? 4 : 0;
            dcdiff[e] = d;
            atomicAdd(&H[512 + 16 * t + category_of(d)], 1u);
        }
#if DMMT_HIST_NEWEST_FIRST
        m -= sm, k -= sk, mr -= smr;
        if (k >= bpm) k += bpm, --m, --mr;
        if (mr >= ri) mr += ri;
#else
        m += sm, k += sk, mr += smr;
        if (k >= bpm) k -= bpm, ++m, ++mr;
        if (mr >= ri) mr -= ri;
#endif
    }
    if (bad) raise_status(status, bad);
    __syncthreads();
    const size_t rep = (size_t)frame * kHistReps + blockIdx.x % kHistReps;
    for (int i = tid; i < 544; i += 256) {
        uint32_t v = 0;
#pragma unroll
        for (int c = 0; c < NC; ++c) v += sH[HS * c + i];
        if (!v) continue;
        if (i < 512)
            atomicAdd(&ac_hist[rep * 512 + i], v);
        else
            atomicAdd(&dc_hist[rep * 32 + (i - 512)], v);
    }
    if (FUSE) {
#if !DMMT_ARRIVE_FORMAL
        asm volatile("s_waitcnt vmcnt(0)" ::: "memory");
#endif
        __syncthreads();
        if (tid == 0) sLastWg = arrive_last(arrive + (size_t)frame * kArriveWords, blockIdx.x, gridDim.x);
        __syncthreads();
        if (sLastWg) {
            arrive_acquire();
            tables_tail(reinterpret_cast<uint8_t*>(sH), ac_hist, dc_hist, frame, g, code_tab, out, out_stride, hdr_len,
                        qtab_u8, bits_per_channel, status, sSmall, sSmall + 4);
        }
    }
}


#define PM_LEVELS 15

__device__ __forceinline__ void put_be16(uint8_t* p, int v) {
    p[0] = (uint8_t)(v >> 8);
    p[1] = (uint8_t)v;
}

__device__ void write_table_header(uint8_t* o, int tab, int t0, int step, int n, const int nt[4],
                                   const uint8_t* symrank, const int* bits16, const Geom& g,
                                   const uint8_t* __restrict__ qtab_u8, int bits_per_channel, uint32_t* hdr_len,
                                   int dq = -1) {
    if (!g.stripe_first) {
        if (tab == 0 && t0 == 0) *hdr_len = 0;
        return;
    }
    const int pos_dht0 = 2 + 18 + 69 + 69 + 19;
    const int off_lac = pos_dht0;
    const int off_ldc = off_lac + 21 + nt[1];
    const int off_cac = off_ldc + 21 + nt[0];
    const int off_cdc = off_cac + 21 + nt[3];
    const int dht = tab == 0 ? off_ldc : tab == 1 ? off_lac : tab == 2 ? off_cdc : off_cac;
    for (int s = t0; s < n; s += step) o[dht + 21 + s] = symrank[n - 1 - s];
    for (int s = t0; s < 16; s += step) o[dht + 5 + s] = (uint8_t)bits16[s];
    if (t0 == 0) {
        uint8_t* d = o + dht;
        d[0] = 0xFF;
        d[1] = 0xC4;
        put_be16(d + 2, 2 + 17 + n);
        const uint8_t kind[4] = {0x00, 0x11, 0x02, 0x13};
        d[4] = kind[tab];
    }
    if (tab != 0) return;
    const int pos_after_dht = pos_dht0 + 4 * 21 + nt[0] + nt[1] + nt[2] + nt[3];
    const int pos_sos = pos_after_dht + (g.restart_interval > 0 ? 6 : 0);
    if (t0 == 0) {
        o[0] = 0xFF;
        o[1] = 0xD8;
        const uint8_t app0[18] = {0xFF, 0xE0, 0x00, 0x10, 'J', 'F', 'I', 'F', 0, 0x01, 0x02, 0x00, 0x00, 0x48, 0x00, 0x48, 0, 0};
        for (int i = 0; i < 18; ++i) o[2 + i] = app0[i];
        for (int q = 0; q < 2; ++q) {
            uint8_t* d = o + 20 + 69 * q;
            d[0] = 0xFF;
            d[1] = 0xDB;
            put_be16(d + 2, 67);
            d[4] = (uint8_t)q;
        }
        uint8_t* sof = o + 158;
        sof[0] = 0xFF;
        sof[1] = 0xC0;
        put_be16(sof + 2, 17);
        sof[4] = (uint8_t)bits_per_channel;
        put_be16(sof + 5, g.sof_height);
        put_be16(sof + 7, g.width);
        sof[9] = 3;
        sof[10] = 1;
        sof[11] = (uint8_t)((g.hr << 4) | g.vr);
        sof[12] = 0;
        sof[13] = 2;
        sof[14] = 0x11;
        sof[15] = 1;
        sof[16] = 3;
        sof[17] = 0x11;
        sof[18] = 1;
        if (g.restart_interval > 0) {
            uint8_t* d = o + pos_after_dht;
            d[0] = 0xFF;
            d[1] = 0xDD;
            put_be16(d + 2, 4);
            put_be16(d + 4, g.restart_interval);
        }
        const uint8_t sos[14] = {0xFF, 0xDA, 0x00, 0x0C, 0x03, 0x01, 0x01, 0x02, 0x23, 0x03, 0x23, 0x00, 0x3F, 0x00};
        for (int i = 0; i < 14; ++i) o[pos_sos + i] = sos[i];
        *hdr_len = (uint32_t)(pos_sos + 14);
    }
    if (dq >= 0) {
        o[25 + t0] = (uint8_t)dq;
        o[94 + t0] = (uint8_t)(dq >> 8);
        return;
    }
    for (int s = t0; s < 128; s += step) {
        const int q = s >> 6, i = s & 63;
        o[20 + 69 * q + 5 + i] = qtab_u8[q * 64 + c_zigzag[i]];
    }
}

__device__ __forceinline__ int packages_below(const unsigned long long* prev, int m, unsigned long long x, int lb) {
    const ulonglong2* pr = reinterpret_cast<const ulonglong2*>(prev);
    int lo = lb, hi = m, step = 1;
    while (lo < hi) {
        const int probe = min(lo + step - 1, hi - 1);
        const ulonglong2 p = pr[probe];
        if (p.x + p.y < x) {
            lo = probe + 1;
            step <<= 1;
        } else {
            hi = probe;
            break;
        }
    }
    while (lo < hi) {
        const int mid = (lo + hi) >> 1;
        const ulonglong2 p = pr[mid];
        if (p.x + p.y < x)
            lo = mid + 1;
        else
            hi = mid;
    }
    return lo;
}

__device__ __forceinline__ int leaves_not_above(const unsigned long long* f, int m, unsigned long long x, int ub) {
    int lo = 0, hi = min(ub, m), step = 1;
    while (lo < hi) {
        const int probe = max(hi - step, lo);
        if (f[probe] <= x) {
            lo = probe + 1;
            break;
        }
        hi = probe;
        step <<= 1;
    }
    while (lo < hi) {
        const int mid = (lo + hi) >> 1;
        if (f[mid] <= x)
            lo = mid + 1;
        else
            hi = mid;
    }
    return lo;
}

__global__ __launch_bounds__(512) void k_tables(const uint32_t* __restrict__ ac_hist,
                                                const uint32_t* __restrict__ dc_hist,
                                                uint32_t* __restrict__ code_tab,
                                                uint8_t* __restrict__ out, size_t out_stride,
                                                uint32_t* __restrict__ hdr_len, Geom g,
                                                const uint8_t* __restrict__ qtab_u8,
                                                int bits_per_channel, int* __restrict__ status) {
    __shared__ __attribute__((aligned(16))) unsigned long long sKey[256];
    __shared__ __attribute__((aligned(16))) unsigned long long sF[256];
    __shared__ __attribute__((aligned(16))) unsigned long long sLev[2][512];
    __shared__ unsigned long long sPk[PM_LEVELS][8];
    __shared__ int sPkCum[PM_LEVELS][8];
    __shared__ uint8_t sSym[256];
    __shared__ int sLen[256];
    __shared__ int sCnt[4][4];
    __shared__ int sLeaf[PM_LEVELS];
    __shared__ uint32_t sWave[4];
    __shared__ int sBits[16];

// ... 364 lines not shown
                    F[lane + 64 * q] = x[q] >> 8;
                    Sym[lane + 64 * q] = (uint8_t)x[q];
                }
        } else {
            uint32_t x[1] = {f[0] ? (f[0] << 8) | (uint32_t)lane : kMergeInf};
            sort_bitonic<1>(x);
            if (lane < n) {
                F[lane] = x[0] >> 8;
                Sym[lane] = (uint8_t)x[0];
            }
        }
    } else {
        int at = 0;
#pragma unroll
        for (int q = 0; q < 4; ++q) {
            if (f[q]) Key[at + __popcll(pres[q] & ((1ull << lane) - 1ull))] = ((unsigned long long)f[q] << 8) | (unsigned)(lane + 64 * q);
            at += __popcll(pres[q]);
        }
        wave_lds_sync();
        tail_rank_any(Key, n, F, Sym);
    }
    wave_lds_sync();

    int leaf[kTailLevels];
    if (n <= 32)
        tail_levels<1>(F, n, leaf);
    else if (n <= 64)
        tail_levels<2>(F, n, leaf);
    else if (n <= 128)
        tail_levels<4>(F, n, leaf);
    else
        tail_levels<8>(F, n, leaf);

    uint32_t len[4];
#pragma unroll
    for (int r = 0; r < 4; ++r) {
        const int i = lane + 64 * r;
        len[r] = 0;
        if (i < n) {
            uint32_t L = i == 0 ? 1u : 0u;
#pragma unroll
            for (int k = 0; k < kTailLevels; ++k) L += i < leaf[k] ? 1u : 0u;
            len[r] = L;
            atomicAdd(&bits16[L - 1], 1);
        }
    }

    {
        uint32_t carry = 0;
        uint32_t inc[4];
#pragma unroll
        for (int r = 0; r < 4; ++r) {
            const uint32_t wgt = len[r] ? 1u << (16 - len[r]) : 0u;
            inc[r] = carry + wave_incl_scan_full_u32(wgt);
            carry = (uint32_t)__builtin_amdgcn_readlane((int)inc[r], 63);
        }
#pragma unroll
        for (int r = 0; r < 4; ++r) {
            const int i = lane + 64 * r;
            if (i < n) {
                const uint32_t pat = (carry - inc[r]) & 0xFFFFu;
                ct[Sym[i]] = (len[r] << 16) | (pat >> (16 - len[r]));
            }
        }
    }
    __syncthreads();

    const int nt[4] = {sCnt[0], sCnt[1], sCnt[2], sCnt[3]};
    write_table_header(out + (size_t)frame * out_stride, tab, lane, 64, n, nt, Sym, bits16, g, qtab_u8,
                       bits_per_channel, hdr_len + frame, dq);
}

__global__ __launch_bounds__(256) void k_dct_blocks(float* __restrict__ data, long long nblocks) {
    __shared__ float s[32 * 65];
    const int tid = threadIdx.x;
    for (long long b0 = (long long)blockIdx.x * 32; b0 < nblocks; b0 += (long long)gridDim.x * 32) {
        const int nbk = (int)min(32LL, nblocks - b0);
        for (int i = tid; i < nbk * 64; i += 256) s[(i >> 6) * 65 + (i & 63)] = data[b0 * 64 + i];
        __syncthreads();
        {
            const int blk = tid >> 3, row = tid & 7;
            if (blk < nbk) {
                float v[8];
                for (int i = 0; i < 8; ++i) v[i] = s[blk * 65 + row * 8 + i];
                arai8(v);
                for (int i = 0; i < 8; ++i) s[blk * 65 + row * 8 + i] = v[i];
            }
        }
        __syncthreads();
        {
            const int blk = tid >> 3, col = tid & 7;
            if (blk < nbk) {
                float v[8];
                for (int i = 0; i < 8; ++i) v[i] = s[blk * 65 + i * 8 + col];
                arai8(v);
                for (int i = 0; i < 8; ++i) s[blk * 65 + i * 8 + col] = v[i];
            }
        }
        __syncthreads();
        for (int i = tid; i < nbk * 64; i += 256) data[b0 * 64 + i] = s[(i >> 6) * 65 + (i & 63)];
        __syncthreads();
    }
}

__device__ __forceinline__ uint32_t xorshift32(uint32_t x) {
    x ^= x << 13;
    x ^= x >> 17;
    x ^= x << 5;
    return x;
}

__global__ __launch_bounds__(256) void k_synthetic(uint8_t* __restrict__ rgb, int w, int h, int n_frames,
                                                   int first_frame, uint32_t seed, int row0, int rows) {
    const long long npx = (long long)w * h;
    const long long nout = (long long)w * rows;
    for (long long i = (long long)blockIdx.x * 256 + threadIdx.x; i < nout * n_frames;
         i += (long long)gridDim.x * 256) {
        const int fl = (int)(i / nout);
        const long long pi = i - (long long)fl * nout + (long long)row0 * w;
        const int y = (int)(pi / w), x = (int)(pi - (long long)y * w);
        const uint32_t f = (uint32_t)(first_frame + fl);
        const uint32_t base = (uint32_t)(x + 8 * y) & 255u;
        const uint32_t n = xorshift32(seed ^ (uint32_t)(f * (uint32_t)npx + (uint32_t)pi));
        const uint32_t r = base + (n & 15u);
        const uint32_t g = ((base + 85u * f + ((uint32_t)y >> 3)) & 255u) + ((n >> 4) & 15u);
        const uint32_t b = ((255u - base + ((uint32_t)x >> 4)) & 255u) + ((n >> 8) & 15u);
        uint8_t* p = rgb + i * 3;
        p[0] = (uint8_t)min(r, 255u);
        p[1] = (uint8_t)min(g, 255u);
        p[2] = (uint8_t)min(b, 255u);
    }
}


}

namespace dmmt {

#ifndef FRONT_WPE_420
#define FRONT_WPE_420 3
#endif

template <int HR, int VR, typename S>
constexpr int front_wpe() {
    return sizeof(S) == 1 ? (HR * VR == 4 ? FRONT_WPE_420 : 4) : 1;
}


template <int HR, int VR, typename S>
static void front_impl(const void* rgb, size_t stride_elems, int n_frames, const Geom& g, const Work& w,
                       hipStream_t st, int per_cu_cap) {
    constexpr int TM = 32 / HR;
    const long long ntiles = (long long)((g.mcux + TM - 1) / TM) * g.mcuy;
    static const FrontCfg cfg = [] { return front_cfg(k_front<HR, VR, S, front_wpe<HR, VR, S>()>); }();
    hipLaunchKernelGGL((k_front<HR, VR, S, front_wpe<HR, VR, S>()>), front_grid(cfg, ntiles, n_frames, per_cu_cap),
                       dim3(256), 0, st, (const S*)rgb, stride_elems, g, w.norm_lut, w.qtab, w.coef, w.status);
}

template <int HR, int VR, typename S, int LAY>
static void front_surf_impl(const SurfArgs& sa, size_t frame_stride, int n_frames, const Geom& g, const Work& w,
                            hipStream_t st, int per_cu_cap) {
    constexpr int TM = 32 / HR;
    const long long ntiles = (long long)((g.mcux + TM - 1) / TM) * g.mcuy;
    static const FrontCfg cfg = [] { return front_cfg(k_front_surf<HR, VR, S, LAY, front_wpe<HR, VR, S>()>); }();
    hipLaunchKernelGGL((k_front_surf<HR, VR, S, LAY, front_wpe<HR, VR, S>()>),
                       front_grid(cfg, ntiles, n_frames, per_cu_cap), dim3(256), 0, st, sa, frame_stride, g, w.norm_lut,
                       w.qtab, w.coef, w.status);
}
template <typename S, int LAY>
static void front_surf_sub(const SurfArgs& sa, size_t frame_stride, int n_frames, const Geom& g, const Work& w,
                           hipStream_t st, int per_cu_cap) {
    if (g.hr == 1)
        front_surf_impl<1, 1, S, LAY>(sa, frame_stride, n_frames, g, w, st, per_cu_cap);
    else if (g.vr == 1)
        front_surf_impl<2, 1, S, LAY>(sa, frame_stride, n_frames, g, w, st, per_cu_cap);
    else
        front_surf_impl<2, 2, S, LAY>(sa, frame_stride, n_frames, g, w, st, per_cu_cap);
}

int surface_samples_per_pixel(int format, int sample_bytes) {
    const bool sb_ok = sample_bytes == 1 || sample_bytes == 2 || sample_bytes == 4;
    if (format == SURF_RGB || format == SURF_BGR) return sb_ok ? 3 : 0;
    if (format == SURF_RGBX || format == SURF_BGRX) return sample_bytes == 1 ? 4 : 0;
    if (format == SURF_PLANAR) return sample_bytes == 1 || sample_bytes == 4 ? 1 : 0;
    return 0;
}

hipError_t launch_front_surface(const Surface& sf, size_t frame_stride_bytes, int sample_bytes, int n_frames,
                                const Geom& g, const Work& w, hipStream_t st, int per_cu_cap) {
    const int spp = surface_samples_per_pixel(sf.format, sample_bytes);
    if (!spp) return hipErrorInvalidValue;
    SurfArgs sa{};
    for (int p = 0; p < 3; ++p) sa.plane[p] = (const uint8_t*)sf.plane[p];
    sa.pitch = (long long)sf.row_pitch;
    sa.span = (long long)(g.height - 1) * sa.pitch + (long long)g.width * spp * sample_bytes;
    sa.bgr = sf.format == SURF_BGR || sf.format == SURF_BGRX;
    if (sf.format == SURF_PLANAR) {
        if (sample_bytes == 1)
            front_surf_sub<uint8_t, LAY_PLANAR>(sa, frame_stride_bytes, n_frames, g, w, st, per_cu_cap);
        else
            front_surf_sub<float, LAY_PLANAR>(sa, frame_stride_bytes, n_frames, g, w, st, per_cu_cap);
    } else if (spp == 4) {
        front_surf_sub<uint8_t, LAY_RGBX>(sa, frame_stride_bytes, n_frames, g, w, st, per_cu_cap);
    } else if (sample_bytes == 1) {
        front_surf_sub<uint8_t, LAY_RGB>(sa, frame_stride_bytes, n_frames, g, w, st, per_cu_cap);
    } else if (sample_bytes == 2) {
        front_surf_sub<uint16_t, LAY_RGB>(sa, frame_stride_bytes, n_frames, g, w, st, per_cu_cap);
    } else {
        front_surf_sub<float, LAY_RGB>(sa, frame_stride_bytes, n_frames, g, w, st, per_cu_cap);
    }
    return hipGetLastError();
}

hipError_t launch_front(const void* rgb, size_t frame_stride_bytes, int sample_bytes, int n_frames, const Geom& g,
                        const Work& w, hipStream_t st, int per_cu_cap) {
    const size_t se = frame_stride_bytes / (size_t)sample_bytes;
    if (sample_bytes == 4) {
        if (g.hr == 1)
            front_impl<1, 1, float>(rgb, se, n_frames, g, w, st, per_cu_cap);
        else if (g.vr == 1)
            front_impl<2, 1, float>(rgb, se, n_frames, g, w, st, per_cu_cap);
        else
            front_impl<2, 2, float>(rgb, se, n_frames, g, w, st, per_cu_cap);
    } else if (sample_bytes == 1) {
        if (g.hr == 1)
            front_impl<1, 1, uint8_t>(rgb, se, n_frames, g, w, st, per_cu_cap);
        else if (g.vr == 1)
            front_impl<2, 1, uint8_t>(rgb, se, n_frames, g, w, st, per_cu_cap);
        else
            front_impl<2, 2, uint8_t>(rgb, se, n_frames, g, w, st, per_cu_cap);
    } else {
        if (g.hr == 1)
            front_impl<1, 1, uint16_t>(rgb, se, n_frames, g, w, st, per_cu_cap);
        else if (g.vr == 1)
            front_impl<2, 1, uint16_t>(rgb, se, n_frames, g, w, st, per_cu_cap);
        else
            front_impl<2, 2, uint16_t>(rgb, se, n_frames, g, w, st, per_cu_cap);
    }
    return hipGetLastError();
}

#ifndef DMMT_HIST_WG_CAP
#define DMMT_HIST_WG_CAP 1024
#endif
bool tables_fusable(const Geom& g) { return g.stripe_first && !g.more_after && g.bpf * 64 * 16 < (1ll << 30); }

hipError_t launch_hist(int n_frames, const Geom& g, const Work& w, int check_cat, hipStream_t st, bool fuse_tables,
                       int bits_per_channel, uint8_t* out, size_t out_stride, int wg_cap) {
    const int cap = wg_cap > 0 ? wg_cap : DMMT_HIST_WG_CAP;
    const int per_frame = cap / n_frames > 0 ? cap / n_frames : 1;
    dim3 grid(clampi((g.bpf + 255) / 256, 1, per_frame), n_frames);
    const bool fuse = fuse_tables && tables_fusable(g);
    auto go = [&](auto kern) {
        hipLaunchKernelGGL(kern, grid, dim3(256), 0, st, (const int16_t*)w.coef, w.dcdiff, w.lastnz, g, w.ac_hist,
                           w.dc_hist, w.status, w.arrive, w.code_tab, out, out_stride, w.hdr_len, w.qtab_u8,
                           bits_per_channel);
    };
    if (check_cat)
        fuse ? go(k_hist<true, true>) : go(k_hist<true, false>);
    else
        fuse ? go(k_hist<false, true>) : go(k_hist<false, false>);
    return hipGetLastError();
}

hipError_t launch_tables(int n_frames, const Geom& g, const Work& w, int bits_per_channel, uint8_t* out,
                         size_t out_stride, hipStream_t st) {
    hipLaunchKernelGGL(k_tables, dim3(4, n_frames), dim3(512), 0, st, (const uint32_t*)w.ac_hist,
                       (const uint32_t*)w.dc_hist, w.code_tab, out, out_stride,
                       w.hdr_len, g, w.qtab_u8, bits_per_channel, w.status);
    return hipGetLastError();
}

hipError_t launch_dct_blocks(float* data, long long nblocks, hipStream_t st) {
    hipLaunchKernelGGL(k_dct_blocks, dim3(clampi((nblocks + 31) / 32, 1, 2048)), dim3(256), 0, st, data, nblocks);
    return hipGetLastError();
}

hipError_t launch_synthetic(uint8_t* rgb, int w, int h, int n_frames, int first_frame, uint32_t seed, int row0,
                            int rows, hipStream_t st) {
    const long long n = (long long)w * rows * n_frames;
    hipLaunchKernelGGL(k_synthetic, dim3(clampi((n + 255) / 256, 1, 8192)), dim3(256), 0, st, rgb, w, h, n_frames,
                       first_frame, seed, row0, rows);
    return hipGetLastError();
}

}

#ifdef DMMT_PHASE_TRACE
extern "C" int dmmt_debug_trace_kernels(unsigned long long* out64) {
    if (hipMemcpyFromSymbol(out64, HIP_SYMBOL(dmmt::g_trace), 64 * 8) != hipSuccess) return -1;
    unsigned long long z[64] = {0};
    return hipMemcpyToSymbol(HIP_SYMBOL(dmmt::g_trace), z, sizeof z) == hipSuccess ? 0 : -1;
}
#endif
```

### dmmt-jpeg-encoder_amd/csrc/kernels.hpp

```cpp
#pragma once
#include <hip/hip_runtime.h>
#include <stdint.h>

#include "jpeg_common.hpp"

namespace dmmt {

struct Work {
    int16_t* coef;
    int16_t* dcdiff;
    uint8_t* lastnz;
    uint32_t* ac_hist;
    uint32_t* dc_hist;
    uint32_t* code_tab;
    uint32_t* hdr_len;
    uint32_t* stage;
    uint32_t* chunk_bits;
    uint32_t* chunk_ff;
    unsigned long long* chunk_ff8;
    uint32_t* chunk_edge;
    unsigned long long* chunk_bit0;
    unsigned long long* chunk_out;
    unsigned long long* total_out;
    uint32_t* arrive;
    int* status;
    const float* norm_lut;
    const float* qtab;
    const uint8_t* qtab_u8;
};

enum Stage { ST_FRONT = 0, ST_HIST, ST_TABLES, ST_EMIT, ST_OFFSETS, ST_STUFFWRITE, ST_COUNT };

enum { SURF_RGB = 0, SURF_BGR = 1, SURF_RGBX = 2, SURF_BGRX = 3, SURF_PLANAR = 4 };
struct Surface {
    const void* plane[3];
    size_t row_pitch;
    int format;
};
struct SurfArgs {
    const uint8_t* plane[3];
    long long pitch;
    long long span;
    int bgr;
};
int surface_samples_per_pixel(int format, int sample_bytes);
hipError_t launch_front_surface(const Surface& sf, size_t frame_stride_bytes, int sample_bytes, int n_frames,
                                const Geom& g, const Work& w, hipStream_t st, int per_cu_cap = 0);

enum { YCC_PLANAR = 0, YCC_NV = 1, YCC_NV_VU = 2 };
struct YccFrames {
    const void* plane[3];
    size_t luma_pitch, chroma_pitch;
    int format;
};
size_t ycc_plane_span(int format, int plane, int width, int height, int hr, int vr, size_t luma_pitch,
                      size_t chroma_pitch);
hipError_t launch_front_ycc(const YccFrames& yf, size_t frame_stride_bytes, int n_frames, const Geom& g, const Work& w,
                            hipStream_t st, int per_cu_cap = 0);

hipError_t launch_front(const void* rgb, size_t frame_stride_bytes, int sample_bytes, int n_frames, const Geom& g,
                        const Work& w, hipStream_t st, int per_cu_cap = 0);
#ifndef DMMT_FRONT_PER_CU_LANES
#define DMMT_FRONT_PER_CU_LANES 2
#endif
bool tables_fusable(const Geom& g);
hipError_t launch_hist(int n_frames, const Geom& g, const Work& w, int check_cat, hipStream_t st,
                       bool fuse_tables = false, int bits_per_channel = 8, uint8_t* out = nullptr,
                       size_t out_stride = 0, int wg_cap = 0);
#ifndef DMMT_HIST_WG_CAP_LANES
#define DMMT_HIST_WG_CAP_LANES 512
#endif
hipError_t launch_tables(int n_frames, const Geom& g, const Work& w, int bits_per_channel, uint8_t* out,
                         size_t out_stride, hipStream_t st);
constexpr int kFusedRoundChunks = 1536;
constexpr int kFusedOffsetsMaxChunks = 4 * kFusedRoundChunks;
constexpr int kArriveFrameWords = 65 * 32;
bool offsets_fusable(const Geom& g);
hipError_t launch_emit(int n_frames, const Geom& g, const Work& w, bool fuse_offsets, hipStream_t st, bool prio);
hipError_t launch_offsets(int n_frames, const Geom& g, const Work& w, hipStream_t st);
hipError_t launch_stuffwrite(int n_frames, const Geom& g, const Work& w, uint8_t* out, size_t out_stride,
                             uint32_t* out_len, hipStream_t st);
size_t ppm_chunk_count(const uint8_t* text, size_t body_offset, size_t len);
size_t ppm_counts_capacity(long long nch);
constexpr size_t kPpmReportBytes = 32;
bool ppm_fast_path(const uint8_t* text, size_t body_offset, size_t len);
hipError_t launch_ppm_p3_fast(const uint8_t* text, size_t body_offset, size_t len, uint32_t* counts,
                              unsigned long long* row_base, void* report, void* out, int sample_bytes,
                              unsigned long long nsamples, uint32_t maxval, hipStream_t st);
hipError_t launch_ppm_p3_general(const uint8_t* text, size_t body_offset, size_t len, unsigned long long* maps,
                                 unsigned long long* chunk_in, void* misc, void* out, int sample_bytes,
                                 unsigned long long nsamples, uint32_t maxval, hipStream_t st);
hipError_t launch_ppm_p6(const uint8_t* samples, void* out, int sample_bytes, unsigned long long nsamples,
                         uint32_t maxval, uint32_t* status, hipStream_t st);
hipError_t launch_dct_blocks(float* data, long long nblocks, hipStream_t st);
hipError_t launch_synthetic(uint8_t* rgb, int w, int h, int n_frames, int first_frame, uint32_t seed, int row0,
                            int rows, hipStream_t st);

}
```

Before: 198,800 Mpixel/s.

## Add narrow int8 coefficient format with escape path to cut coefficient traffic

Adds a compact coefficient layout: the first 8 zigzag coefficients stay int16, the rest are stored as int8 with an escape marker, and full int16 values are written to the wide buffer only for columns that overflow. The front kernel writes this format, and the hist and emit kernels read it, falling back to the wide buffer when a block is flagged. The aim is to shrink the coefficient bytes written and read between stages, from 128 to 80 per block. In exchange the code takes on extra per-block branches, ballots, escape handling and more kernel variants. The format is chosen automatically when the quantisation tables allow it, which they do at quality 90.

```diff
diff --git a/dmmt-jpeg-encoder_amd/csrc/coef_format.hpp b/dmmt-jpeg-encoder_amd/csrc/coef_format.hpp
--- /dev/null
+++ b/dmmt-jpeg-encoder_amd/csrc/coef_format.hpp
@@ -0,0 +1,116 @@
+#pragma once
+#include <stdint.h>
+
+#include "jpeg_common.hpp"
+
+namespace dmmt {
+
+constexpr int kCoefLoCount = 8;
+constexpr int kCoefLoBytes = 2 * kCoefLoCount, kCoefHiBytes = 64;
+constexpr int kCoefEscape = -128;
+
+constexpr bool coef_in_lo(int k) { return k < kCoefLoCount; }
+constexpr int coef_hi_byte(int v) { return v < -127 || v > 127 ? kCoefEscape : v; }
+constexpr int coef_hi_word(int k) { return coef_pos(k) >> 2; }
+constexpr int coef_hi_shift(int k) { return 8 * (coef_pos(k) & 3); }
+constexpr int coef_lo_rows(int c) { return c == 0 ? 3 : c < 3 ? 2 : c == 3 ? 1 : 0; }
+
+inline void coef_pack_block(const int16_t* zz, int16_t* lo, int8_t* hi, int16_t* wide) {
+    for (int k = 0; k < kCoefLoCount; ++k) lo[k] = zz[k];
+    bool esc[8] = {false};
+    bool any = false;
+    for (int k = 0; k < 64; ++k) {
+        const int p = coef_pos(k);
+        const int b = coef_in_lo(k) ? 0 : coef_hi_byte(zz[k]);
+        hi[p] = (int8_t)b;
+        if (!coef_in_lo(k) && b == kCoefEscape) esc[p >> 3] = any = true;
+    }
+    hi[coef_pos(0)] = any ? 1 : 0;
+    for (int k = 0; k < 64; ++k)
+        if (esc[coef_pos(k) >> 3]) wide[coef_pos(k)] = zz[k];
+}
+inline bool coef_block_flag(const int8_t* hi) { return hi[coef_pos(0)] != 0; }
+inline int coef_read(int k, const int16_t* lo, const int8_t* hi, const int16_t* wide) {
+    if (coef_in_lo(k)) return lo[k];
+    const int b = hi[coef_pos(k)];
+    return coef_block_flag(hi) && b == kCoefEscape ? wide[coef_pos(k)] : b;
+}
+
+enum { COEF_FORMAT_AUTO = 0, COEF_FORMAT_WIDE = 1, COEF_FORMAT_NARROW = 2 };
+constexpr int kCoefNarrowMinQ = 2;
+inline bool coef_narrow_for(int mode, int sample_bytes, const uint8_t* luma_q, const uint8_t* chroma_q) {
+    if (sample_bytes == 4 || mode == COEF_FORMAT_WIDE) return false;
+    if (mode == COEF_FORMAT_NARROW) return true;
+    for (int k = kCoefLoCount; k < 64; ++k)
+        if (luma_q[kZigzag[k]] < kCoefNarrowMinQ || chroma_q[kZigzag[k]] < kCoefNarrowMinQ) return false;
+    return true;
+}
+
+#ifdef __HIPCC__
+__device__ __forceinline__ bool coef_word_escapes(uint32_t w) {
+    const uint32_t t = w ^ 0x80808080u;
+    return ((t - 0x01010101u) & ~t & 0x80808080u) != 0u;
+}
+
+__device__ __forceinline__ void coef_store_column_narrow(const int (&x)[8], int col, int el, bool valid,
+                                                         int16_t* __restrict__ wide, int16_t* __restrict__ lo,
+                                                         int8_t* __restrict__ hi) {
+    uint32_t c[8];
+#pragma unroll
+    for (int i = 0; i < 8; ++i) c[i] = (uint32_t)min(max(x[i], -128), 128);
+    uint32_t w0 = __builtin_amdgcn_perm(c[1], c[0], 0x0c0c0400u) | __builtin_amdgcn_perm(c[3], c[2], 0x04000c0cu);
+    const uint32_t w1 = __builtin_amdgcn_perm(c[5], c[4], 0x0c0c0400u) | __builtin_amdgcn_perm(c[7], c[6], 0x04000c0cu);
+    w0 &= 0xFFFFFFFFu << (8 * (col == 0 ? 3 : col < 3 ? 2 : col == 3 ? 1 : 0));
+    const uint32_t p = __builtin_amdgcn_perm((uint32_t)x[1], (uint32_t)x[0], 0x05040100u);
+    const uint32_t s1 = (uint32_t)__builtin_amdgcn_update_dpp(0, (int)p, 0x101, 0xF, 0xF, true);
+    const uint32_t s2 = (uint32_t)__builtin_amdgcn_update_dpp(0, (int)p, 0x102, 0xF, 0xF, true);
+    const uint32_t s3 = (uint32_t)__builtin_amdgcn_update_dpp(0, (int)p, 0x103, 0xF, 0xF, true);
+    const bool esc = coef_word_escapes(w0) || coef_word_escapes(w1);
+    const unsigned long long em = __builtin_amdgcn_ballot_w64(esc);
+    if (em != 0) {
+        const uint32_t lane = __builtin_amdgcn_mbcnt_hi(~0u, __builtin_amdgcn_mbcnt_lo(~0u, 0u));
+        const uint32_t group = (uint32_t)(em >> (lane & 56u)) & 0xFFu;
+        w0 |= col == 0 && group != 0u ? 1u : 0u;
+    }
+    if (valid) {
+        *reinterpret_cast<uint2*>(hi + (el * 64 + 8 * col)) = make_uint2(w0, w1);
+        if (col == 0) {
+            const uint32_t l0 = __builtin_amdgcn_perm(s1, p, 0x05040100u);
+            const uint32_t l1 = __builtin_amdgcn_perm((uint32_t)x[2], p, 0x05040302u);
+            const uint32_t l2 = __builtin_amdgcn_perm(s2, s1, 0x05040302u);
+            const uint32_t l3 = __builtin_amdgcn_perm(s2, s3, 0x07060100u);
+            *reinterpret_cast<uint4*>(lo + el * 8) = make_uint4(l0, l1, l2, l3);
+        }
+        if (esc) {
+            uint32_t pk[4];
+            pk[0] = p;
+#pragma unroll
+            for (int i = 1; i < 4; ++i) pk[i] = __builtin_amdgcn_perm((uint32_t)x[2 * i + 1], (uint32_t)x[2 * i], 0x05040100u);
+            *reinterpret_cast<uint4*>(wide + (el * 64 + 8 * col)) = make_uint4(pk[0], pk[1], pk[2], pk[3]);
+        }
+    }
+}
+
+struct NarrowCoef {
+    uint32_t lo[4];
+    uint32_t hi[16];
+};
+__device__ __forceinline__ void load_narrow(const int16_t* __restrict__ lo, const int8_t* __restrict__ hi, long long e,
+                                            NarrowCoef& b) {
+    const uint4 l = *reinterpret_cast<const uint4*>(lo + e * 8);
+    b.lo[0] = l.x, b.lo[1] = l.y, b.lo[2] = l.z, b.lo[3] = l.w;
+    const uint4* q = reinterpret_cast<const uint4*>(hi + e * 64);
+#pragma unroll
+    for (int i = 0; i < 4; ++i) {
+        const uint4 v = q[i];
+        b.hi[4 * i] = v.x, b.hi[4 * i + 1] = v.y, b.hi[4 * i + 2] = v.z, b.hi[4 * i + 3] = v.w;
+    }
+}
+__device__ __forceinline__ bool narrow_flag(const NarrowCoef& b) { return (b.hi[0] & 0xFFu) != 0u; }
+__device__ __forceinline__ int narrow_at(const NarrowCoef& b, int k) {
+    if (coef_in_lo(k)) return (k & 1) ? ((int)b.lo[k >> 1] >> 16) : (int)(int16_t)(b.lo[k >> 1] & 0xFFFFu);
+    return (int)(b.hi[coef_hi_word(k)] << (24 - coef_hi_shift(k))) >> 24;
+}
+#endif
+
+}
diff --git a/dmmt-jpeg-encoder_amd/csrc/encoder.cpp b/dmmt-jpeg-encoder_amd/csrc/encoder.cpp
--- a/dmmt-jpeg-encoder_amd/csrc/encoder.cpp
+++ b/dmmt-jpeg-encoder_amd/csrc/encoder.cpp
@@ -48,7 +48,7 @@
     hipStream_t stream = nullptr;
     int* status = nullptr;
     int* dstatus = nullptr;
-    DevBuf coef, dcdiff, lastnz, ac_hist, dc_hist, code_tab, hdr_len, total_out, stage, chunk_bits, chunk_ff,
+    DevBuf coef, coef_lo, coef_hi, dcdiff, lastnz, ac_hist, dc_hist, code_tab, hdr_len, total_out, stage, chunk_bits, chunk_ff,
         chunk_ff8, chunk_edge, chunk_bit0, chunk_out, arrive;
     DevBuf ppm_rgb, ppm_counts, ppm_rowbase;
 };
@@ -81,6 +81,7 @@
     int stage_launches[ST_COUNT] = {0};
     bool use_graphs = false;
     bool fuse_tables = DMMT_FUSE_TABLES_DEFAULT != 0;
+    int coef_format = COEF_FORMAT_AUTO;
     std::vector<GraphEntry> graphs;
     uint64_t graph_clock = 0;
     bool stripe_pending = false;
@@ -199,12 +200,16 @@
     return DMMT_OK;
 }
 
-int ensure_work(dmmt_ctx* c, const Geom& g, int nf, Work* w, int lane, bool async) {
+int ensure_work(dmmt_ctx* c, const Geom& g, int nf, Work* w, int lane, bool async, bool narrow = false) {
     int rc;
     Lane* L = c->lanes[lane];
     const size_t nb = (size_t)g.bpf * nf;
     const size_t nch = (size_t)g.nch * nf;
     if ((rc = ensure(L->coef, nb * 64 * sizeof(int16_t)))) return rc;
+    if (narrow) {
+        if ((rc = ensure(L->coef_lo, nb * kCoefLoBytes))) return rc;
+        if ((rc = ensure(L->coef_hi, nb * kCoefHiBytes))) return rc;
+    }
     if ((rc = ensure(L->dcdiff, nb * sizeof(int16_t)))) return rc;
     if ((rc = ensure(L->lastnz, nb))) return rc;
     if ((rc = ensure(L->stage, (nch * (size_t)kChunkWordsCap + 64) * sizeof(uint32_t)))) return rc;
@@ -232,6 +237,8 @@
         }
     }
     w->coef = (int16_t*)L->coef.p;
+    w->coef_lo = narrow ? (int16_t*)L->coef_lo.p : nullptr;
+    w->coef_hi = narrow ? (int8_t*)L->coef_hi.p : nullptr;
     w->dcdiff = (int16_t*)L->dcdiff.p;
     w->lastnz = (uint8_t*)L->lastnz.p;
     w->ac_hist = (uint32_t*)L->ac_hist.p;
@@ -255,9 +262,10 @@
 }
 
 int prepare(dmmt_ctx* c, const Geom& g, int nf, const dmmt_options* opt, int sb, hipStream_t st, Work* w,
-            int lane = 0, bool async = false, int* status = nullptr) {
-    int rc;
-    if ((rc = ensure_work(c, g, nf, w, lane, async))) return rc;
+            int lane = 0, bool async = false, int* status = nullptr, bool allow_narrow = false) {
+    int rc;
+    const bool narrow = allow_narrow && coef_narrow_for(c->coef_format, sb, opt->luma_q, opt->chroma_q);
+    if ((rc = ensure_work(c, g, nf, w, lane, async, narrow))) return rc;
     if (status) w->status = status;
     if ((rc = upload_tables(c, opt, g.maxval, sb, st))) return rc;
     w->norm_lut = (const float*)c->lut.p;
@@ -367,7 +375,7 @@
                    const YccFrames* yf = nullptr) {
     Work w;
     int rc;
-    if ((rc = prepare(c, g, nf, opt, sb, st, &w, lane, async, status))) return rc;
+    if ((rc = prepare(c, g, nf, opt, sb, st, &w, lane, async, status, true))) return rc;
     const int bits = opt->bits_per_channel;
     if (!c->use_graphs || c->profile || status)
         return enqueue_direct(c, d_rgb, frame_stride, sb, nf, g, w, bits, out, out_stride, out_len, st, sf, yf);
@@ -458,7 +466,7 @@
 void destroy_lane(Lane* L, bool own_stream) {
     (void)hipStreamSynchronize(L->stream);
     if (L->status) (void)hipHostFree(L->status);
-    DevBuf* bufs[] = {&L->coef,      &L->dcdiff,     &L->lastnz,     &L->ac_hist,
+    DevBuf* bufs[] = {&L->coef,      &L->coef_lo,    &L->coef_hi,    &L->dcdiff,     &L->lastnz,     &L->ac_hist,
                       &L->dc_hist,  &L->code_tab,  &L->hdr_len,    &L->total_out,  &L->stage,
                       &L->chunk_bits, &L->chunk_ff, &L->chunk_ff8, &L->chunk_edge, &L->chunk_bit0, &L->chunk_out,
                       &L->arrive,     &L->ppm_rgb,    &L->ppm_counts, &L->ppm_rowbase};
@@ -491,6 +499,8 @@
     c->device = device;
     if (const char* e = getenv("DMMT_GRAPHS")) c->use_graphs = atoi(e) != 0;
     if (const char* e = getenv("DMMT_FUSE_TABLES")) c->fuse_tables = atoi(e) != 0;
+    if (const char* e = getenv("DMMT_COEF_FORMAT"))
+        c->coef_format = !strcmp(e, "wide") ? COEF_FORMAT_WIDE : !strcmp(e, "narrow") ? COEF_FORMAT_NARROW : COEF_FORMAT_AUTO;
     if (hipStreamCreateWithFlags(&c->stream, hipStreamNonBlocking) != hipSuccess) {
         delete c;
         return DMMT_E_HIP;
@@ -519,7 +529,7 @@
     if ((rc = set_device(c))) return rc;
     std::lock_guard<std::mutex> lk(c->mu);
     for (Lane* L : c->lanes) {
-        const DevBuf* bufs[] = {&L->coef,       &L->dcdiff,   &L->lastnz,     &L->ac_hist,    &L->dc_hist,
+        const DevBuf* bufs[] = {&L->coef,       &L->coef_lo,  &L->coef_hi,    &L->dcdiff,   &L->lastnz,     &L->ac_hist,    &L->dc_hist,
                                 &L->code_tab,   &L->hdr_len,  &L->total_out,  &L->stage,      &L->chunk_bits,
                                 &L->chunk_ff,   &L->chunk_ff8,  &L->chunk_edge, &L->chunk_bit0, &L->chunk_out, &L->arrive,
                                 &L->ppm_rgb,    &L->ppm_counts, &L->ppm_rowbase};
@@ -1429,7 +1439,7 @@
     if ((rc = set_device(c))) return rc;
     hipStream_t s = c->stream;
     Work w;
-    if ((rc = prepare(c, g, 1, opt, st->sample_bytes, s, &w))) return rc;
+    if ((rc = prepare(c, g, 1, opt, st->sample_bytes, s, &w, 0, false, nullptr, true))) return rc;
     {
         StageTimer t(c, ST_FRONT, s);
         HIP_TRY(launch_front(st->d_rgb, (size_t)st->width * g.height * 3 * st->sample_bytes, st->sample_bytes, 1, g, w,
@@ -1458,17 +1468,19 @@
         }
     }
     if (g.restart_interval == 0) {
-        std::vector<int16_t> head((size_t)g.bpm * 64), tail((size_t)g.bpm * 64);
+        const int16_t* const blocks = w.coef_lo ? w.coef_lo : w.coef;
+        const size_t bs = w.coef_lo ? kCoefLoCount : 64;
+        std::vector<int16_t> head((size_t)g.bpm * bs), tail((size_t)g.bpm * bs);
         const int nl = g.n_luma;
-        HIP_TRY(hipMemcpyAsync(head.data(), w.coef, head.size() * 2, hipMemcpyDeviceToHost, s));
-        HIP_TRY(hipMemcpyAsync(tail.data(), w.coef + (g.bpf - g.bpm) * 64, tail.size() * 2, hipMemcpyDeviceToHost, s));
+        HIP_TRY(hipMemcpyAsync(head.data(), blocks, head.size() * 2, hipMemcpyDeviceToHost, s));
+        HIP_TRY(hipMemcpyAsync(tail.data(), blocks + (g.bpf - g.bpm) * bs, tail.size() * 2, hipMemcpyDeviceToHost, s));
         HIP_TRY(hipStreamSynchronize(s));
         c->stripe_dc_first[0] = head[0];
-        c->stripe_dc_first[1] = head[(size_t)nl * 64];
-        c->stripe_dc_first[2] = head[(size_t)(nl + 1) * 64];
-        c->stripe_dc_last[0] = tail[(size_t)(nl - 1) * 64];
-        c->stripe_dc_last[1] = tail[(size_t)nl * 64];
-        c->stripe_dc_last[2] = tail[(size_t)(nl + 1) * 64];
+        c->stripe_dc_first[1] = head[(size_t)nl * bs];
+        c->stripe_dc_first[2] = head[(size_t)(nl + 1) * bs];
+        c->stripe_dc_last[0] = tail[(size_t)(nl - 1) * bs];
+        c->stripe_dc_last[1] = tail[(size_t)nl * bs];
+        c->stripe_dc_last[2] = tail[(size_t)(nl + 1) * bs];
     }
     c->stripe_g = g;
     c->stripe_opt = *opt;
@@ -1544,7 +1556,7 @@
     if (out_cap < max_jpeg_bytes(g)) return DMMT_E_CAPACITY;
     hipStream_t s = c->stream;
     Work w;
-    if ((rc = prepare(c, g, 1, &c->stripe_opt, c->stripe_sb, s, &w))) return rc;
+    if ((rc = prepare(c, g, 1, &c->stripe_opt, c->stripe_sb, s, &w, 0, false, nullptr, true))) return rc;
     if ((rc = upload_hist_sum(w, hist_sum, s))) return rc;
     int16_t d[3];
     const long long at[3] = {0, g.n_luma, g.n_luma + 1};
@@ -1599,7 +1611,7 @@
     g.next16 = g.more_after ? (next16 & 0xFFFFu) & ~(0xFFFFu >> next_bits) : 0u;
     hipStream_t s = c->stream;
     Work w;
-    if ((rc = prepare(c, g, 1, &c->stripe_opt, c->stripe_sb, s, &w))) return rc;
+    if ((rc = prepare(c, g, 1, &c->stripe_opt, c->stripe_sb, s, &w, 0, false, nullptr, true))) return rc;
     if ((rc = ensure(c->out_len, 4))) return rc;
     {
         StageTimer t(c, ST_OFFSETS, s);
@@ -1632,7 +1644,7 @@
     if (out_cap < max_jpeg_bytes(g)) return DMMT_E_CAPACITY;
     hipStream_t s = c->stream;
     Work w;
-    if ((rc = prepare(c, g, 1, &c->stripe_opt, c->stripe_sb, s, &w))) return rc;
+    if ((rc = prepare(c, g, 1, &c->stripe_opt, c->stripe_sb, s, &w, 0, false, nullptr, true))) return rc;
     if ((rc = upload_hist_sum(w, hist_sum, s))) return rc;
     if ((rc = ensure(c->out_len, 4))) return rc;
     if ((rc = enqueue_back_half(c, g, 1, w, c->stripe_opt.bits_per_channel, d_out, out_cap, (uint32_t*)c->out_len.p,
diff --git a/dmmt-jpeg-encoder_amd/csrc/entropy.hip b/dmmt-jpeg-encoder_amd/csrc/entropy.hip
--- a/dmmt-jpeg-encoder_amd/csrc/entropy.hip
+++ b/dmmt-jpeg-encoder_amd/csrc/entropy.hip
@@ -109,9 +109,30 @@
     for (int j = 0; j < 32; ++j) b.w[j] = z[j];
 }
 
-template <typename Sink>
-__device__ __forceinline__ void walk_block(const BlockCoef& b, int dcd, const uint2* __restrict__ dctab,
-                                           const uint2* __restrict__ actab, Sink& sink, int kmax = 63) {
+__device__ __forceinline__ bool walk_nonzero(const BlockCoef& b, int k, uint32_t m_low) {
+    const int kc = DMMT_WALK_COLUMN_MAJOR ? coef_pos(k) : k;
+    const uint32_t w = b.w[kc >> 1];
+    return (kc & 1) ? w > m_low : (w << 16) != 0u;
+}
+__device__ __forceinline__ int walk_value(const BlockCoef& b, int k) {
+    return coef_at(b, DMMT_WALK_COLUMN_MAJOR ? coef_pos(k) : k);
+}
+__device__ __forceinline__ bool walk_nonzero(const NarrowCoef& b, int k, uint32_t m_low) {
+    if (coef_in_lo(k)) {
+        const uint32_t w = b.lo[k >> 1];
+        return (k & 1) ? w > m_low : (w << 16) != 0u;
+    }
+    const uint32_t w = b.hi[coef_hi_word(k)];
+    const int s = coef_hi_shift(k);
+    return s == 24 ? w > 0x00FFFFFFu : s == 0 ? (w << 24) != 0u : (w & (0xFFu << s)) != 0u;
+}
+__device__ __forceinline__ int walk_value(const NarrowCoef& b, int k) { return narrow_at(b, k); }
+
+template <bool ESC = true, typename Sink, typename Block>
+__device__ __forceinline__ void walk_block(const Block& b, int dcd, const uint2* __restrict__ dctab,
+                                           const uint2* __restrict__ actab, Sink& sink, int kmax = 63,
+                                           const int16_t* esc = nullptr) {
+    constexpr bool kNarrow = std::is_same<Block, NarrowCoef>::value;
     {
         const int cat = category_of(dcd);
         const uint2 e = dctab[cat];
@@ -125,10 +146,13 @@
         if (k0 != 0 && k0 > kmax) break;
 #pragma unroll
         for (int k = k0 ? k0 : 1; k < k0 + 4; ++k) {
-            const int kc =DMMT_WALK_COLUMN_MAJOR ? coef_pos(k) : k;
-            const uint32_t w = b.w[kc >> 1];
-            if ((kc & 1) ? w > m_low : (w << 16) != 0u) {
-                const int v = coef_at(b, kc);
+            if (walk_nonzero(b, k, m_low)) {
+                int v = walk_value(b, k);
+                if (kNarrow && ESC && !coef_in_lo(k)) {
+                    if (__builtin_amdgcn_ballot_w64(v == kCoefEscape) != 0) {
+                        if (v == kCoefEscape) v = (int)esc[coef_pos(k)];
+                    }
+                }
                 const int r16 = 16 * k - l16;
                 if (k >= 17 && __builtin_amdgcn_ballot_w64((uint32_t)r16 > m_zrl) != 0) {
                     int r = r16 >> 8;
@@ -242,10 +266,11 @@
     return (wave << 6) | (int)__builtin_amdgcn_mbcnt_hi(~0u, __builtin_amdgcn_mbcnt_lo(~0u, zero));
 }
 
-template <int OCC>
-__global__ __launch_bounds__(kEmitThreads, OCC) void k_emit(const int16_t* coef, const int16_t* __restrict__ dcdiff,
+template <bool NARROW>
+__device__ __forceinline__ void emit_body(const int16_t* coef, const int16_t* __restrict__ coef_lo,
+                                              const int8_t* __restrict__ coef_hi, const int16_t* __restrict__ dcdiff,
                                               const uint8_t* __restrict__ lastnz,
-                                              const uint32_t* __restrict__ code_tab, Geom g,
+                                              const uint32_t* __restrict__ code_tab, const Geom& g,
                                               uint32_t* __restrict__ stage, uint32_t* __restrict__ chunk_bits,
                                               uint32_t* __restrict__ chunk_ff, uint32_t* __restrict__ chunk_edge,
                                               uint32_t* __restrict__ ac_hist, uint32_t* __restrict__ dc_hist,
@@ -330,16 +355,27 @@
         if (valid) {
             const int p = sOrder[tid];
             const long long ep = (long long)frame * g.bpf + el0 + p;
-            BlockCoef b;
-            load_block(coef + ep * 64, b);
-            zigzag_in_registers(b);
+            std::conditional_t<NARROW, NarrowCoef, BlockCoef> b;
+            if constexpr (NARROW) {
+                load_narrow(coef_lo, coef_hi, ep, b);
+            } else {
+                load_block(coef + ep * 64, b);
+                zigzag_in_registers(b);
+            }
             const int dp = dcdiff[ep];
             DMMT_TRACE(4);
             const int kp = mod_small(r0 + p, g.bpm, inv16);
             const bool lum = kp < g.n_luma;
             const int kmax = __builtin_amdgcn_readfirstlane((int)sKey[min(64 * wave + 63, nb - 1)]);
             SlotSink ss{sSlot + tid, 0ull, 0, 0};
-            walk_block(b, dp, sTab + 512 + (lum ? 0 : 16), sTab + (lum ? 0 : 256), ss, kmax);
+            if constexpr (NARROW) {
+                if (__builtin_amdgcn_ballot_w64(narrow_flag(b)) != 0)
+                    walk_block<true>(b, dp, sTab + 512 + (lum ? 0 : 16), sTab + (lum ? 0 : 256), ss, kmax, coef + ep * 64);
+                else
+                    walk_block<false>(b, dp, sTab + 512 + (lum ? 0 : 16), sTab + (lum ? 0 : 256), ss, kmax);
+            } else {
+                walk_block(b, dp, sTab + 512 + (lum ? 0 : 16), sTab + (lum ? 0 : 256), ss, kmax);
+            }
             wbits = ss.finish();
             slot_over = wbits > (uint32_t)kSlotWords * 32u;
             sBits[p] = wbits | ((uint32_t)tid << 16);
@@ -422,11 +458,15 @@
                 const int te = tid_again(wave);
                 const long long e = (long long)frame * g.bpf + el0 + te;
                 const bool lum_t = mod_small(r0 + te, g.bpm, inv16) < g.n_luma;
-                BlockCoef b;
-                load_block(coef + e * 64, b);
-                zigzag_in_registers(b);
+                std::conditional_t<NARROW, NarrowCoef, BlockCoef> b;
+                if constexpr (NARROW) {
+                    load_narrow(coef_lo, coef_hi, e, b);
+                } else {
+                    load_block(coef + e * 64, b);
+                    zigzag_in_registers(b);
+                }
                 WindowSink ws{sW, w0, wn + 1, 0ull, (int)(st & 31), (int)(st >> 5), true};
-                walk_block(b, dcdiff[e], sTab + 512 + (lum_t ? 0 : 16), sTab + (lum_t ? 0 : 256), ws);
+                walk_block(b, dcdiff[e], sTab + 512 + (lum_t ? 0 : 16), sTab + (lum_t ? 0 : 256), ws, 63, coef + e * 64);
                 ws.finish();
             }
             tid = tid_again(wave);
@@ -480,6 +520,38 @@
     }
     DMMT_TRACE(3);
     DMMT_TRACE_FLUSH(0, 0);
+}
+
+template <int OCC>
+__global__ __launch_bounds__(kEmitThreads, OCC) void k_emit(const int16_t* coef, const int16_t* __restrict__ dcdiff,
+                                              const uint8_t* __restrict__ lastnz,
+                                              const uint32_t* __restrict__ code_tab, Geom g,
+                                              uint32_t* __restrict__ stage, uint32_t* __restrict__ chunk_bits,
+                                              uint32_t* __restrict__ chunk_ff, uint32_t* __restrict__ chunk_edge,
+                                              uint32_t* __restrict__ ac_hist, uint32_t* __restrict__ dc_hist,
+                                              int fuse, uint32_t* __restrict__ arrive,
+                                              unsigned long long* __restrict__ chunk_bit0,
+                                              unsigned long long* __restrict__ chunk_out,
+                                              unsigned long long* __restrict__ total_out,
+                                              unsigned long long* __restrict__ chunk_ff8, int prio) {
+    emit_body<false>(coef, nullptr, nullptr, dcdiff, lastnz, code_tab, g, stage, chunk_bits, chunk_ff, chunk_edge, ac_hist,
+                     dc_hist, fuse, arrive, chunk_bit0, chunk_out, total_out, chunk_ff8, prio);
+}
+template <int OCC>
+__global__ __launch_bounds__(kEmitThreads, OCC) void k_emit_n(const int16_t* coef, const int16_t* __restrict__ coef_lo,
+                                                const int8_t* __restrict__ coef_hi, const int16_t* __restrict__ dcdiff,
+                                                const uint8_t* __restrict__ lastnz,
+                                                const uint32_t* __restrict__ code_tab, Geom g,
+                                                uint32_t* __restrict__ stage, uint32_t* __restrict__ chunk_bits,
+                                                uint32_t* __restrict__ chunk_ff, uint32_t* __restrict__ chunk_edge,
+                                                uint32_t* __restrict__ ac_hist, uint32_t* __restrict__ dc_hist,
+                                                int fuse, uint32_t* __restrict__ arrive,
+                                                unsigned long long* __restrict__ chunk_bit0,
+                                                unsigned long long* __restrict__ chunk_out,
+                                                unsigned long long* __restrict__ total_out,
+                                                unsigned long long* __restrict__ chunk_ff8, int prio) {
+    emit_body<true>(coef, coef_lo, coef_hi, dcdiff, lastnz, code_tab, g, stage, chunk_bits, chunk_ff, chunk_edge, ac_hist,
+                    dc_hist, fuse, arrive, chunk_bit0, chunk_out, total_out, chunk_ff8, prio);
 }
 
 __device__ __forceinline__ uint32_t boundary_byte(int m1, uint32_t last16, bool has_next, uint32_t n_next,
@@ -998,6 +1070,15 @@
 
 hipError_t launch_emit(int n_frames, const Geom& g, const Work& w, bool fuse_offsets, hipStream_t st, bool prio) {
     const int fuse = fuse_offsets && offsets_fusable(g) ? 1 : 0;
+    if (w.coef_lo) {
+        const auto kn = !prio && n_frames > 1 ? k_emit_n<kEmitOccBatch> : k_emit_n<kEmitOcc>;
+        hipLaunchKernelGGL(kn, dim3(g.nch, n_frames), dim3(kEmitThreads), 0, st, (const int16_t*)w.coef,
+                           (const int16_t*)w.coef_lo, (const int8_t*)w.coef_hi, (const int16_t*)w.dcdiff,
+                           (const uint8_t*)w.lastnz, (const uint32_t*)w.code_tab, g, w.stage, w.chunk_bits, w.chunk_ff,
+                           w.chunk_edge, w.ac_hist, w.dc_hist, fuse, w.arrive, w.chunk_bit0, w.chunk_out, w.total_out,
+                           w.chunk_ff8, prio || DMMT_EMIT_PRIO_ALWAYS ? 1 : 0);
+        return hipGetLastError();
+    }
     const auto kern = !prio && n_frames > 1 ? k_emit<kEmitOccBatch> : k_emit<kEmitOcc>;
     hipLaunchKernelGGL(kern, dim3(g.nch, n_frames), dim3(kEmitThreads), 0, st, (const int16_t*)w.coef,
                        (const int16_t*)w.dcdiff, (const uint8_t*)w.lastnz, (const uint32_t*)w.code_tab, g, w.stage, w.chunk_bits, w.chunk_ff,
diff --git a/dmmt-jpeg-encoder_amd/csrc/front_ycc.hip b/dmmt-jpeg-encoder_amd/csrc/front_ycc.hip
--- a/dmmt-jpeg-encoder_amd/csrc/front_ycc.hip
+++ b/dmmt-jpeg-encoder_amd/csrc/front_ycc.hip
@@ -39,10 +39,11 @@
     for (int i = 0; i < N; ++i) o[i] = __builtin_amdgcn_alignbyte(t[i + 1], t[i], (uint32_t)off & 3u);
 }
 
-template <int HR, int VR, int FMT, int WPE>
-__global__ __launch_bounds__(256, WPE) void k_front_ycc(YccArgs ya, size_t frame_stride, Geom g,
-                                                       const float* __restrict__ qtab,
-                                                       int16_t* __restrict__ coef) {
+template <int HR, int VR, int FMT, bool NARROW>
+__device__ __forceinline__ void front_ycc_body(const YccArgs& ya, size_t frame_stride, const Geom& g,
+                                               const float* __restrict__ qtab,
+                                               int16_t* __restrict__ coef, int16_t* __restrict__ coef_lo,
+                                               int8_t* __restrict__ coef_hi) {
     constexpr bool NV = FMT != YCC_PLANAR;
     constexpr int VU = FMT == YCC_NV_VU ? 1 : 0;
     using T = YccTile<HR, VR, NV>;
@@ -186,7 +187,9 @@
                 el = (blk - NYB - CB) * BPM + NLUMA + 1;
             }
             const bool valid = el < nvalid;
-            if (valid) {
+            if constexpr (NARROW) {
+                coef_store_column_narrow(x, col, el, valid, cbase, coef_lo + e0 * 8, coef_hi + e0 * 64);
+            } else if (valid) {
                 uint32_t pk[4];
 #pragma unroll
                 for (int i = 0; i < 4; ++i) pk[i] = __builtin_amdgcn_perm((uint32_t)x[2 * i + 1], (uint32_t)x[2 * i], 0x05040100u);
@@ -194,6 +197,18 @@
             }
         }
     }
+}
+
+template <int HR, int VR, int FMT, int WPE>
+__global__ __launch_bounds__(256, WPE) void k_front_ycc(YccArgs ya, size_t frame_stride, Geom g,
+                                                       const float* __restrict__ qtab, int16_t* __restrict__ coef) {
+    front_ycc_body<HR, VR, FMT, false>(ya, frame_stride, g, qtab, coef, nullptr, nullptr);
+}
+template <int HR, int VR, int FMT, int WPE>
+__global__ __launch_bounds__(256, WPE) void k_front_ycc_n(YccArgs ya, size_t frame_stride, Geom g,
+                                                         const float* __restrict__ qtab, int16_t* __restrict__ coef,
+                                                         int16_t* __restrict__ coef_lo, int8_t* __restrict__ coef_hi) {
+    front_ycc_body<HR, VR, FMT, true>(ya, frame_stride, g, qtab, coef, coef_lo, coef_hi);
 }
 
 
@@ -204,6 +219,12 @@
                            hipStream_t st, int per_cu_cap) {
     constexpr int TM = 32 / HR;
     const long long ntiles = (long long)((g.mcux + TM - 1) / TM) * g.mcuy;
+    if (w.coef_lo) {
+        static const FrontCfg cfgn = [] { return front_cfg(k_front_ycc_n<HR, VR, FMT, front_ycc_wpe()>); }();
+        hipLaunchKernelGGL((k_front_ycc_n<HR, VR, FMT, front_ycc_wpe()>), front_grid(cfgn, ntiles, n_frames, per_cu_cap),
+                           dim3(256), 0, st, ya, frame_stride, g, w.qtab, w.coef, w.coef_lo, w.coef_hi);
+        return;
+    }
     static const FrontCfg cfg = [] { return front_cfg(k_front_ycc<HR, VR, FMT, front_ycc_wpe()>); }();
     hipLaunchKernelGGL((k_front_ycc<HR, VR, FMT, front_ycc_wpe()>), front_grid(cfg, ntiles, n_frames, per_cu_cap),
                        dim3(256), 0, st, ya, frame_stride, g, w.qtab, w.coef);
diff --git a/dmmt-jpeg-encoder_amd/csrc/kernels.hip b/dmmt-jpeg-encoder_amd/csrc/kernels.hip
--- a/dmmt-jpeg-encoder_amd/csrc/kernels.hip
+++ b/dmmt-jpeg-encoder_amd/csrc/kernels.hip
@@ -200,11 +200,14 @@
     }
 };
 
-template <int HR, int VR, typename Sample, int LAY>
+template <int HR, int VR, typename Sample, int LAY, bool NARROW = false>
 __device__ __forceinline__ void front_body(const Sample* __restrict__ rgb, size_t frame_stride, const SurfArgs& sa,
                                            Geom g, const float* __restrict__ norm_lut,
                                            const float* __restrict__ qtab,
-                                           int16_t* __restrict__ coef, int* __restrict__ status) {
+                                           int16_t* __restrict__ coef, int* __restrict__ status,
+                                           int16_t* __restrict__ coef_lo = nullptr,
+                                           int8_t* __restrict__ coef_hi = nullptr) {
+    static_assert(!NARROW || sizeof(Sample) != 4, "Image<f32> dots are unbounded: wide blocks");
     constexpr int TM = 32 / HR;
     constexpr int ROWS = 8 * VR;
     constexpr int NLUMA = HR * VR;
@@ -464,7 +467,9 @@
                 el = (blk - NYB - CB) * BPM + NLUMA + 1;
             }
             const bool valid = el < nvalid;
-            if (valid) {
+            if constexpr (NARROW) {
+                coef_store_column_narrow(x, col, el, valid, cbase, coef_lo + e0 * 8, coef_hi + e0 * 64);
+            } else if (valid) {
                 uint32_t pk[4];
 #pragma unroll
                 for (int i = 0; i < 4; ++i) pk[i] = __builtin_amdgcn_perm((uint32_t)x[2 * i + 1], (uint32_t)x[2 * i], 0x05040100u);
@@ -493,6 +498,23 @@
                                                     const float* __restrict__ qtab, int16_t* __restrict__ coef,
                                                     int* __restrict__ status) {
     front_body<HR, VR, Sample, LAY>(nullptr, frame_stride, sa, g, norm_lut, qtab, coef, status);
+}
+
+template <int HR, int VR, typename Sample, int WPE>
+__global__ __launch_bounds__(256, WPE) void k_front_n(const Sample* __restrict__ rgb, size_t frame_stride, Geom g,
+                                                 const float* __restrict__ norm_lut, const float* __restrict__ qtab,
+                                                 int16_t* __restrict__ coef, int* __restrict__ status,
+                                                 int16_t* __restrict__ coef_lo, int8_t* __restrict__ coef_hi) {
+    front_body<HR, VR, Sample, LAY_TIGHT, true>(rgb, frame_stride, SurfArgs{}, g, norm_lut, qtab, coef, status, coef_lo,
+                                                coef_hi);
+}
+template <int HR, int VR, typename Sample, int LAY, int WPE>
+__global__ __launch_bounds__(256, WPE) void k_front_surf_n(SurfArgs sa, size_t frame_stride, Geom g,
+                                                      const float* __restrict__ norm_lut,
+                                                      const float* __restrict__ qtab, int16_t* __restrict__ coef,
+                                                      int* __restrict__ status, int16_t* __restrict__ coef_lo,
+                                                      int8_t* __restrict__ coef_hi) {
+    front_body<HR, VR, Sample, LAY, true>(nullptr, frame_stride, sa, g, norm_lut, qtab, coef, status, coef_lo, coef_hi);
 }
 
 struct HistCoef {
@@ -511,15 +533,16 @@
 #ifndef DMMT_HIST_NEWEST_FIRST
 #define DMMT_HIST_NEWEST_FIRST 0
 #endif
-template <bool CHECK, bool FUSE>
-__global__ __launch_bounds__(256) __attribute__((amdgpu_waves_per_eu(8, 8))) void k_hist(const int16_t* __restrict__ coef, int16_t* __restrict__ dcdiff,
-                                              uint8_t* __restrict__ lastnz, Geom g,
-                                              uint32_t* __restrict__ ac_hist ,
-                                              uint32_t* __restrict__ dc_hist ,
-                                              int* __restrict__ status, uint32_t* __restrict__ arrive,
-                                              uint32_t* __restrict__ code_tab, uint8_t* __restrict__ out,
-                                              size_t out_stride, uint32_t* __restrict__ hdr_len,
-                                              const uint8_t* __restrict__ qtab_u8, int bits_per_channel) {
+template <bool CHECK, bool FUSE, bool NARROW>
+__device__ __forceinline__ void hist_body(const int16_t* __restrict__ coef, const int16_t* __restrict__ coef_lo,
+                                          const int8_t* __restrict__ coef_hi, int16_t* __restrict__ dcdiff,
+                                          uint8_t* __restrict__ lastnz, const Geom& g,
+                                          uint32_t* __restrict__ ac_hist ,
+                                          uint32_t* __restrict__ dc_hist ,
+                                          int* __restrict__ status, uint32_t* __restrict__ arrive,
+                                          uint32_t* __restrict__ code_tab, uint8_t* __restrict__ out,
+                                          size_t out_stride, uint32_t* __restrict__ hdr_len,
+                                          const uint8_t* __restrict__ qtab_u8, int bits_per_channel) {
     constexpr int NC = kHistCopies, HS = kHistCopyWords;
     constexpr int kWords = FUSE && kTailLdsBytes / 4 > NC * HS ? kTailLdsBytes / 4 : NC * HS;
     __shared__ __attribute__((aligned(16))) uint32_t sH[kWords];
@@ -552,12 +575,18 @@
     for (; el < bpf; el += stride) {
 #endif
         const long long e = base + el;
-        const uint4* q = reinterpret_cast<const uint4*>(coef + e * 64);
-        uint32_t cw[32];
-#pragma unroll
-        for (int i = 0; i < 8; ++i) {
-            const uint4 v = q[i];
-            cw[4 * i] = v.x, cw[4 * i + 1] = v.y, cw[4 * i + 2] = v.z, cw[4 * i + 3] = v.w;
+        uint32_t cw[NARROW ? 1 : 32];
+        NarrowCoef nc;
+        if constexpr (NARROW) {
+            load_narrow(coef_lo, coef_hi, e, nc);
+            cw[0] = nc.lo[0];
+        } else {
+            const uint4* q = reinterpret_cast<const uint4*>(coef + e * 64);
+#pragma unroll
+            for (int i = 0; i < 8; ++i) {
+                const uint4 v = q[i];
+                cw[4 * i] = v.x, cw[4 * i + 1] = v.y, cw[4 * i + 2] = v.z, cw[4 * i + 3] = v.w;
+            }
         }
         const int t = k < (uint32_t)g.n_luma ? 0 : 1;
         const bool restart = g.restart_interval > 0 && mr == 0;
@@ -569,28 +598,52 @@
         const int cur = (int)(int16_t)(cw[0] & 0xFFFFu);
         const int nb = __shfl_up(cur, (unsigned)back, 64);
         int pv = 0;
-        if (back) pv = lane >= back ? nb : (int)coef[(e - back) * 64];
+        if (back) pv = lane >= back ? nb : NARROW ? (int)coef_lo[(e - back) * 8] : (int)coef[(e - back) * 64];
         HistCoef b;
-#pragma unroll
-        for (int j = 0; j < 32; ++j) {
-            const int i0 = coef_pos(2 * j), i1 = coef_pos(2 * j + 1);
-            const uint32_t lo = (cw[i0 >> 1] >> (16 * (i0 & 1))) & 0xFFFFu;
-            const uint32_t hi = (cw[i1 >> 1] >> (16 * (i1 & 1))) & 0xFFFFu;
-            b.w[j] = lo | (hi << 16);
+        if constexpr (!NARROW) {
+#pragma unroll
+            for (int j = 0; j < 32; ++j) {
+                const int i0 = coef_pos(2 * j), i1 = coef_pos(2 * j + 1);
+                const uint32_t lo = (cw[i0 >> 1] >> (16 * (i0 & 1))) & 0xFFFFu;
+                const uint32_t hi = (cw[i1 >> 1] >> (16 * (i1 & 1))) & 0xFFFFu;
+                b.w[j] = lo | (hi << 16);
+            }
         }
         uint32_t* h = H + 256 * t;
         int l16 = 16;
         uint32_t zrl = 0;
-#pragma unroll
-        for (int kk = 1; kk < 64; ++kk) {
-            const int v = (kk & 1) ? ((int)b.w[kk >> 1] >> 16) : (int)(int16_t)(b.w[kk >> 1] & 0xFFFFu);
-            if (v != 0) {
-                if (CHECK && v == -32768) bad |= 4;
-                const int r16 = 16 * kk - l16;
-                zrl += (uint32_t)(r16 >> 8);
-                atomicAdd(&h[(r16 & 0xF0) | category_fast(v)], 1u);
-                l16 = 16 * kk + 16;
-            }
+        auto walk = [&](auto with_escapes) {
+            constexpr bool ESC = decltype(with_escapes)::value;
+#pragma unroll
+            for (int kk = 1; kk < 64; ++kk) {
+                int v;
+                if constexpr (NARROW)
+                    v = narrow_at(nc, kk);
+                else
+                    v = (kk & 1) ? ((int)b.w[kk >> 1] >> 16) : (int)(int16_t)(b.w[kk >> 1] & 0xFFFFu);
+                if (v != 0) {
+                    if (NARROW && ESC && !coef_in_lo(kk)) {
+                        if (__builtin_amdgcn_ballot_w64(v == kCoefEscape) != 0) {
+                            if (v == kCoefEscape) v = (int)coef[e * 64 + coef_pos(kk)];
+                            if (CHECK && v == -32768) bad |= 4;
+                        }
+                    } else if (CHECK) {
+                        bad |= v == -32768 ? 4 : 0;
+                    }
+                    const int r16 = 16 * kk - l16;
+                    zrl += (uint32_t)(r16 >> 8);
+                    atomicAdd(&h[(r16 & 0xF0) | category_fast(v)], 1u);
+                    l16 = 16 * kk + 16;
+                }
+            }
+        };
+        if constexpr (NARROW) {
+            if (__builtin_amdgcn_ballot_w64(narrow_flag(nc)) != 0)
+                walk(std::integral_constant<bool, true>{});
+            else
+                walk(std::integral_constant<bool, false>{});
+        } else {
+            walk(std::integral_constant<bool, false>{});
         }
         if (zrl) atomicAdd(&h[0xF0], zrl);
         if (l16 < 16 * 64) atomicAdd(&h[0], 1u);
@@ -637,6 +690,30 @@
                         qtab_u8, bits_per_channel, status, sSmall, sSmall + 4);
         }
     }
+}
+
+template <bool CHECK, bool FUSE>
+__global__ __launch_bounds__(256) __attribute__((amdgpu_waves_per_eu(8, 8))) void k_hist(const int16_t* __restrict__ coef, int16_t* __restrict__ dcdiff,
+                                              uint8_t* __restrict__ lastnz, Geom g,
+                                              uint32_t* __restrict__ ac_hist, uint32_t* __restrict__ dc_hist,
+                                              int* __restrict__ status, uint32_t* __restrict__ arrive,
+                                              uint32_t* __restrict__ code_tab, uint8_t* __restrict__ out,
+                                              size_t out_stride, uint32_t* __restrict__ hdr_len,
+                                              const uint8_t* __restrict__ qtab_u8, int bits_per_channel) {
+    hist_body<CHECK, FUSE, false>(coef, nullptr, nullptr, dcdiff, lastnz, g, ac_hist, dc_hist, status, arrive, code_tab,
+                                  out, out_stride, hdr_len, qtab_u8, bits_per_channel);
+}
+template <bool CHECK, bool FUSE>
+__global__ __launch_bounds__(256) __attribute__((amdgpu_waves_per_eu(8, 8))) void k_hist_n(const int16_t* __restrict__ coef, const int16_t* __restrict__ coef_lo,
+                                                const int8_t* __restrict__ coef_hi, int16_t* __restrict__ dcdiff,
+                                                uint8_t* __restrict__ lastnz, Geom g,
+                                                uint32_t* __restrict__ ac_hist, uint32_t* __restrict__ dc_hist,
+                                                int* __restrict__ status, uint32_t* __restrict__ arrive,
+                                                uint32_t* __restrict__ code_tab, uint8_t* __restrict__ out,
+                                                size_t out_stride, uint32_t* __restrict__ hdr_len,
+                                                const uint8_t* __restrict__ qtab_u8, int bits_per_channel) {
+    hist_body<CHECK, FUSE, true>(coef, coef_lo, coef_hi, dcdiff, lastnz, g, ac_hist, dc_hist, status, arrive, code_tab,
+                                 out, out_stride, hdr_len, qtab_u8, bits_per_channel);
 }
 
 
@@ -1307,6 +1384,15 @@
                        hipStream_t st, int per_cu_cap) {
     constexpr int TM = 32 / HR;
     const long long ntiles = (long long)((g.mcux + TM - 1) / TM) * g.mcuy;
+    if constexpr (sizeof(S) != 4) {
+        if (w.coef_lo) {
+            static const FrontCfg cfgn = [] { return front_cfg(k_front_n<HR, VR, S, front_wpe<HR, VR, S>()>); }();
+            hipLaunchKernelGGL((k_front_n<HR, VR, S, front_wpe<HR, VR, S>()>),
+                               front_grid(cfgn, ntiles, n_frames, per_cu_cap), dim3(256), 0, st, (const S*)rgb,
+                               stride_elems, g, w.norm_lut, w.qtab, w.coef, w.status, w.coef_lo, w.coef_hi);
+            return;
+        }
+    }
     static const FrontCfg cfg = [] { return front_cfg(k_front<HR, VR, S, front_wpe<HR, VR, S>()>); }();
     hipLaunchKernelGGL((k_front<HR, VR, S, front_wpe<HR, VR, S>()>), front_grid(cfg, ntiles, n_frames, per_cu_cap),
                        dim3(256), 0, st, (const S*)rgb, stride_elems, g, w.norm_lut, w.qtab, w.coef, w.status);
@@ -1317,6 +1403,15 @@
                             hipStream_t st, int per_cu_cap) {
     constexpr int TM = 32 / HR;
     const long long ntiles = (long long)((g.mcux + TM - 1) / TM) * g.mcuy;
+    if constexpr (sizeof(S) != 4) {
+        if (w.coef_lo) {
+            static const FrontCfg cfgn = [] { return front_cfg(k_front_surf_n<HR, VR, S, LAY, front_wpe<HR, VR, S>()>); }();
+            hipLaunchKernelGGL((k_front_surf_n<HR, VR, S, LAY, front_wpe<HR, VR, S>()>),
+                               front_grid(cfgn, ntiles, n_frames, per_cu_cap), dim3(256), 0, st, sa, frame_stride, g,
+                               w.norm_lut, w.qtab, w.coef, w.status, w.coef_lo, w.coef_hi);
+            return;
+        }
+    }
     static const FrontCfg cfg = [] { return front_cfg(k_front_surf<HR, VR, S, LAY, front_wpe<HR, VR, S>()>); }();
     hipLaunchKernelGGL((k_front_surf<HR, VR, S, LAY, front_wpe<HR, VR, S>()>),
                        front_grid(cfg, ntiles, n_frames, per_cu_cap), dim3(256), 0, st, sa, frame_stride, g, w.norm_lut,
@@ -1411,7 +1506,14 @@
                            w.dc_hist, w.status, w.arrive, w.code_tab, out, out_stride, w.hdr_len, w.qtab_u8,
                            bits_per_channel);
     };
-    if (check_cat)
+    auto gon = [&](auto kern) {
+        hipLaunchKernelGGL(kern, grid, dim3(256), 0, st, (const int16_t*)w.coef, (const int16_t*)w.coef_lo,
+                           (const int8_t*)w.coef_hi, w.dcdiff, w.lastnz, g, w.ac_hist, w.dc_hist, w.status, w.arrive,
+                           w.code_tab, out, out_stride, w.hdr_len, w.qtab_u8, bits_per_channel);
+    };
+    if (w.coef_lo)
+        fuse ? gon(k_hist_n<false, true>) : gon(k_hist_n<false, false>);
+    else if (check_cat)
         fuse ? go(k_hist<true, true>) : go(k_hist<true, false>);
     else
         fuse ? go(k_hist<false, true>) : go(k_hist<false, false>);
diff --git a/dmmt-jpeg-encoder_amd/csrc/kernels.hpp b/dmmt-jpeg-encoder_amd/csrc/kernels.hpp
--- a/dmmt-jpeg-encoder_amd/csrc/kernels.hpp
+++ b/dmmt-jpeg-encoder_amd/csrc/kernels.hpp
@@ -2,12 +2,15 @@
 #include <hip/hip_runtime.h>
 #include <stdint.h>
 
+#include "coef_format.hpp"
 #include "jpeg_common.hpp"
 
 namespace dmmt {
 
 struct Work {
     int16_t* coef;
+    int16_t* coef_lo;
+    int8_t* coef_hi;
     int16_t* dcdiff;
     uint8_t* lastnz;
     uint32_t* ac_hist;
```

Result: faster. 206,700 Mpixel/s (median of 6 runs) (+4.0%).
